# epfl-lts2/pygsp

Measured on AMD Instinct MI355X. Metric: filtered-vertices/sec (N·Nsig·K/s) + achieved HBM GB/s vs roofline, 1M-vertex K=30, higher is better.
Workload: dtype f64

## Files before the change

include/gspx_ext.h:

```cpp
#ifndef GSPX_EXT_H
#define GSPX_EXT_H

#include "gspx.h"

#ifdef __cplusplus
extern "C" {
#endif

int gspx_newton_filter_dev(gspx_graph* g, double lmax, int K, const double* nodes,
                           const double* dcoef, int64_t Nsig, const void* x_dev, void* y_dev,
                           double* kernel_ms);
int gspx_newton_filter(gspx_graph* g, double lmax, int K, const double* nodes, const double* dcoef,
                       int64_t Nsig, const void* x_host, void* y_host, double* kernel_ms);

int gspx_poly_program_dev(gspx_graph* g, double lmax, int S, const double* scale, const double* beta, const double* gamma,
                          int old_is_x, int64_t Nsig, const void* x_dev, void* y_dev, double* kernel_ms);
int gspx_poly_program(gspx_graph* g, double lmax, int S, const double* scale, const double* beta, const double* gamma,
                      int old_is_x, int64_t Nsig, const void* x_host, void* y_host, double* kernel_ms);

int gspx_graph_download_internal(gspx_graph* g, int32_t* rowptr, int32_t* col);

int gspx_graph_set_gather_tiles(gspx_graph* g, int block_rows, int nb, const int32_t* s1ptr,
                                const int32_t* s1rows, const uint16_t* lidx, int64_t* stats);

int gspx_laplacian_apply_dev(gspx_graph* g, int64_t Nsig, const void* x_dev, void* y_dev,
                             double* kernel_ms);
int gspx_dirichlet_energy_dev(gspx_graph* g, int64_t Nsig, const void* x_dev, double* gram_host,
                              double* kernel_ms);
int gspx_panel_gram_dev(gspx_ctx* ctx, int64_t N, const double* A, int64_t lda, int na, const double* B, int64_t ldb,
                        int nb, double* C_host, double* kernel_ms);
int gspx_panel_combine_dev(gspx_ctx* ctx, int64_t N, const double* X, int64_t ldx, int p, const double* Q_host, int q,
                           double* Y, int64_t ldy, double* kernel_ms);
int gspx_panel_gram_to_dev(gspx_ctx* ctx, int64_t N, const double* A, int64_t lda, int na, const double* B, int64_t ldb,
                           int nb, const double* rowscale, double alpha, double* C, int64_t ldc, double* kernel_ms);
int gspx_spectral_apply_dev(gspx_ctx* ctx, int64_t N, const double* U, int64_t ldu, int n, const double* S, int64_t lds,
                            int w, int mode, int nf, const double* H, double* Y, int64_t ldy, double* kernel_ms);
int gspx_panel_residual_norms_dev(gspx_ctx* ctx, int64_t N, const double* X, const double* LX, int64_t ld, int p,
                                  const double* theta_host, double* out_host, double* kernel_ms);
int gspx_panel_copy_dev(gspx_ctx* ctx, int64_t N, const double* X, int64_t ldx, int w, double* Y, int64_t ldy,
                        double* kernel_ms);
int gspx_lanczos_krylov_dev(gspx_graph* g, int order, int64_t Nsig, const void* x_dev, int64_t ldx, double breakdown,
                            void* V_dev, double* alpha_host, double* beta_host, double* proj_host, int32_t* steps_host,
                            double* phase_ms, double* kernel_ms);
int gspx_lanczos_combine_dev(gspx_graph* g, int order, int64_t Nsig, const void* V_dev, int Nf,
                             const double* weights_host, void* y_dev, int64_t ldy, double* kernel_ms);
int gspx_tikhonov_cg_dev(gspx_graph* g, double tau, const void* mask_dev, int64_t Nsig,
                         const void* y_dev, void* x_dev, double rtol, double atol, int64_t maxiter,
                         int32_t* iterations, double* kernel_ms);
int gspx_dirichlet_cg_dev(gspx_graph* g, const void* mask_dev, int64_t Nsig, const void* y_dev, void* x_dev,
                          double rtol, double atol, int64_t maxiter, int32_t* iterations, double* kernel_ms);
int gspx_tikhonov_simplex_dev(gspx_graph* g, double tau, double step, const int32_t* labels_dev, int n_classes,
                              double rtol, double atol, double dtol, double xtol, int64_t maxit, void* x_dev,
                              int64_t* niter, int32_t* crit, double* objective_host, double* kernel_ms);
int gspx_prox_tv_dev(gspx_graph* g, double gamma, double step, int64_t Nsig, const void* x_dev, void* z_dev,
                     double rtol, double atol, double dtol, double xtol, int64_t maxit, int64_t* niter, int32_t* crit,
                     double* objective_host, double* kernel_ms);
int gspx_graph_n_edges(gspx_graph* g, int64_t* n_edges);
int gspx_graph_download_edges(gspx_graph* g, int32_t* sources, int32_t* targets, void* weights,
                              void* d_source, void* d_target);
int gspx_graph_set_edge_list(gspx_graph* g, int64_t n_edges, const int32_t* sources, const int32_t* targets,
                             const double* weights, int directed);

int gspx_grad_dev(gspx_graph* g, int64_t Nsig, const void* x_dev, void* y_dev, double* kernel_ms);
int gspx_div_dev(gspx_graph* g, int64_t Nsig, const void* y_dev, void* z_dev, double* kernel_ms);

typedef struct gspx_knn gspx_knn;
int gspx_knn_build(gspx_ctx* ctx, int64_t N, int d, const double* coords, int k, double sigma,
                   int metric, int symmetrize, gspx_knn** out);
int gspx_knn_destroy(gspx_knn* h);
int gspx_knn_info(gspx_knn* h, int64_t* nnz, double* sigma, double* build_ms);
int gspx_knn_search_stats(gspx_knn* h, double out[4]);
int gspx_knn_download_w(gspx_knn* h, int32_t* indptr, int32_t* indices, double* data);
int gspx_knn_download_neighbors(gspx_knn* h, int32_t* nn, double* dist);

int gspx_radius_build(gspx_ctx* ctx, int64_t N, int d, const double* coords, double epsilon,
                      double sigma, int metric, gspx_knn** out);

int gspx_sbm_build(gspx_ctx* ctx, int64_t N, int k, const int32_t* order, const int64_t* bounds,
                   const double* M, uint64_t seed, gspx_knn** out);
int gspx_sbm_build_ex(gspx_ctx* ctx, int64_t N, int k, const int32_t* order, const int64_t* bounds,
                      const double* M, uint64_t seed, int flags, gspx_knn** out);

int gspx_linegraph_size(gspx_graph* g, int64_t* n_vertices, int64_t* nnz);
int gspx_linegraph_build(gspx_graph* g, gspx_knn** out, double* kernel_ms);

int gspx_schur_cg_dev(gspx_graph* g, double shift, const void* mask_dev, int64_t Nsig, const void* f_dev, void* x_dev,
                      void* alpha_dev, double rtol, double atol, int64_t maxiter, int32_t* iterations,
                      double* kernel_ms);
int gspx_kron_build(gspx_graph* g, double shift, const int32_t* ind_host, int64_t nk, double rtol, int64_t maxiter,
                    double* lnew_dev, gspx_knn** w_out, int32_t* iterations, double* kernel_ms);

int gspx_curve_keys(gspx_ctx* ctx, int64_t N, int d, const double* coords, int curve, uint64_t* keys);

int gspx_curve_order(gspx_ctx* ctx, int64_t N, int d, const double* coords, int curve, int32_t* perm);

int gspx_graph_setup(gspx_ctx* ctx, int64_t N, int64_t nnz, const int32_t* indptr, const int32_t* indices,
                     const void* data, int data_dtype, int lap_type, int compute_dtype, const double* coords,
                     int d, int order_mode, const int32_t* perm_in, int64_t report[12], gspx_graph** out);
int gspx_graph_setup_from_knn(gspx_knn* h, int lap_type, int compute_dtype, const double* coords, int d,
                              int order_mode, const int32_t* perm_in, int64_t report[12], gspx_graph** out);
int gspx_graph_lmax_bounds(gspx_graph* g, double out[4]);
int gspx_graph_download_perm(gspx_graph* g, int32_t* perm);

int gspx_graph_components_dev(gspx_graph* g, int32_t* labels_dev, int64_t* n_components, int* rounds,
                              double* kernel_ms);
int gspx_graph_components(gspx_graph* g, int32_t* labels_host, int64_t* n_components, int* rounds, double* kernel_ms);
int gspx_components_round_cap(int64_t N, int* cap);

int gspx_layout_spring_dev(gspx_graph* g, int dim, double k, const void* fixed_dev, int64_t iterations, double t0,
                           double dt, void* pos_dev, double* kernel_ms);
int gspx_layout_splits(gspx_graph* g, int64_t* splits);

#define GSPX_ERR_NOCONV 7
int gspx_sym_eig_dev(gspx_ctx* ctx, int n, const double* A, int64_t lda, double* V, int64_t ldv, double* e_host,
                     double tol, int max_sweeps, double* info, int64_t* skipped_per_sweep);
int gspx_sym_eig_schedule_describe(int n_blocks, int* pairs_out, int* n_rounds);
int gspx_panel_scale_cols_dev(gspx_ctx* ctx, int64_t N, double* X, int64_t ldx, int w, const double* s_host);

int gspx_identity_panel_dev(gspx_ctx* ctx, int dtype, int64_t N, int64_t j0, int64_t w, void* out_dev);
int gspx_cheby_sqnorms_dev(gspx_graph* g, double lmax, int Nf, int M, const double* coeffs, int64_t Nsig,
                           const void* x_dev, double* out, double* kernel_ms);
int gspx_cheby_moments_dev(gspx_graph* g, double lmax, int M, int64_t Nsig, const void* x_dev,
                           double* out, double* kernel_ms);

int gspx_device_pci_bus_id(int device, char* out, int capacity);

int gspx_planes_pack_dev(gspx_ctx* ctx, int dtype, int64_t N, int64_t S, int64_t F, const void* src_dev,
                         void* dst_dev, int to_planes);

int gspx_plan_describe(gspx_ctx* ctx, int Nf, int M, const double* coeffs, double* plan);
int gspx_host_pipeline_describe(int mode, int64_t host_batch, int64_t host_edge, int64_t host_threads, int dtype,
                                int64_t N, int64_t Nsig, int planes_total, int64_t* widths, int capacity,
                                int* n_batches, int* threads);

int gspx_last_host_timing(gspx_ctx* ctx, double out[9]);
int gspx_last_step_kinds(gspx_ctx* ctx, int64_t out[2]);
int gspx_last_host_timeline(gspx_ctx* ctx, double* out, int capacity, int* batches);

int gspx_bench_copy(gspx_ctx* ctx, int64_t bytes, int iters, double* gbps);

int gspx_bench_read(gspx_ctx* ctx, int64_t bytes, int passes, double* gbps);

int gspx_ctx_tune_placement(gspx_graph* g, double lmax, int M, const double* coeffs, int64_t Nsig, const void* x_dev,
                            void* y_dev, int candidates, int64_t stride_mb, double* out);

int gspx_bench_streams(gspx_ctx* ctx, int64_t bytes_per_stream, int n_read, int n_write, int nt, int workgroups_per_cu,
                       int iters, double* gbps);

int gspx_bench_step_mix(gspx_graph* g, double lmax, int M, const double* coeffs, int64_t Nsig, const void* x_dev,
                        void* y_dev, int mode);

int gspx_bench_gather(gspx_ctx* ctx, int64_t panel_rows, int row_bytes, int64_t n_gathers, int in_flight,
                      int blocks, double p_intra, int workgroups_per_cu, int iters, double* ms, double* gbps);

int gspx_comm_info(gspx_comm* comm, int64_t out[3]);

#ifdef __cplusplus
}
#endif
#endif
```

pygsp_amd/_capi.py:

```python
import ctypes
import os

import numpy as np

_HERE = os.path.dirname(os.path.abspath(__file__))
LIB_PATH = os.environ.get("GSPX_LIB_PATH") or os.path.join(_HERE, "_lib", "libgspx.so")

F32, F64 = 0, 1
LAP_COMBINATORIAL, LAP_NORMALIZED = 0, 1
ANALYSIS, SYNTHESIS = 0, 1

OK, ERR_INVALID, ERR_COEFF, ERR_HIP, ERR_NODEVICE, ERR_OOM, ERR_INTERNAL, ERR_NOCONV = 0, 1, 2, 3, 4, 5, 6, 7

_lib = None


class GspxError(RuntimeError):
    """HIP / runtime failure inside libgspx."""


def dtype_code(dt):
    dt = np.dtype(dt)
    if dt == np.float32:
        return F32
    if dt == np.float64:
        return F64
    raise ValueError("libgspx computes in float32 or float64, got {}".format(dt))


def np_dtype(code):
    return np.float32 if code == F32 else np.float64


_c = ctypes
_P = _c.c_void_p
SIGNATURES = {
    "gspx_last_error": (_c.c_char_p, []),
    "gspx_version": (_c.c_char_p, []),
    "gspx_device_count": (_c.c_int, [_c.POINTER(_c.c_int)]),
    "gspx_ctx_create": (_c.c_int, [_c.c_int, _c.POINTER(_P)]),
    "gspx_ctx_destroy": (_c.c_int, [_P]),
    "gspx_ctx_sync": (_c.c_int, [_P]),
    "gspx_ctx_set_option": (_c.c_int, [_P, _c.c_char_p, _c.c_int64]),
    "gspx_ctx_get_option": (_c.c_int, [_P, _c.c_char_p, _c.POINTER(_c.c_int64)]),
    "gspx_buf_alloc": (_c.c_int, [_P, _c.c_int64, _c.POINTER(_P)]),
    "gspx_buf_free": (_c.c_int, [_P]),
    "gspx_buf_upload": (_c.c_int, [_P, _P, _c.c_int64]),
    "gspx_buf_download": (_c.c_int, [_P, _P, _c.c_int64]),
    "gspx_buf_ptr": (_c.c_int, [_P, _c.POINTER(_P)]),
    "gspx_buf_bytes": (_c.c_int, [_P, _c.POINTER(_c.c_int64)]),
    "gspx_graph_create_from_w": (_c.c_int, [_P, _c.c_int64, _c.c_int64, _P, _P, _P, _c.c_int,
                                            _c.c_int, _c.c_int, _P, _c.POINTER(_P)]),
    "gspx_graph_create_from_l": (_c.c_int, [_P, _c.c_int64, _c.c_int64, _P, _P, _P, _c.c_int,
                                            _c.c_int, _P, _c.POINTER(_P)]),
    "gspx_graph_destroy": (_c.c_int, [_P]),
    "gspx_graph_n": (_c.c_int, [_P, _c.POINTER(_c.c_int64)]),
    "gspx_graph_nnz_l": (_c.c_int, [_P, _c.POINTER(_c.c_int64)]),
    "gspx_graph_nnz_internal": (_c.c_int, [_P, _c.POINTER(_c.c_int64)]),
    "gspx_graph_download_l": (_c.c_int, [_P, _P, _P, _P]),
    "gspx_graph_download_dw": (_c.c_int, [_P, _P]),
    "gspx_graph_build_ms": (_c.c_int, [_P, _c.POINTER(_c.c_double)]),
    "gspx_cheby_filter_dev": (_c.c_int, [_P, _c.c_double, _c.c_int, _c.c_int, _P, _c.c_int64, _P,
                                         _P, _c.c_int, _c.POINTER(_c.c_double)]),
    "gspx_cheby_filter": (_c.c_int, [_P, _c.c_double, _c.c_int, _c.c_int, _P, _c.c_int64, _P, _P,
                                     _c.c_int, _c.POINTER(_c.c_double)]),
    "gspx_newton_filter_dev": (_c.c_int, [_P, _c.c_double, _c.c_int, _P, _P, _c.c_int64, _P, _P,
                                          _c.POINTER(_c.c_double)]),
    "gspx_newton_filter": (_c.c_int, [_P, _c.c_double, _c.c_int, _P, _P, _c.c_int64, _P, _P,
                                      _c.POINTER(_c.c_double)]),
    "gspx_graph_download_internal": (_c.c_int, [_P, _P, _P]),
    "gspx_laplacian_apply_dev": (_c.c_int, [_P, _c.c_int64, _P, _P, _P]),
    "gspx_dirichlet_energy_dev": (_c.c_int, [_P, _c.c_int64, _P, _P, _P]),
    "gspx_panel_gram_dev": (_c.c_int, [_P, _c.c_int64, _P, _c.c_int64, _c.c_int, _P, _c.c_int64, _c.c_int, _P, _P]),
    "gspx_panel_combine_dev": (_c.c_int, [_P, _c.c_int64, _P, _c.c_int64, _c.c_int, _P, _c.c_int, _P, _c.c_int64, _P]),
    "gspx_panel_gram_to_dev": (_c.c_int, [_P, _c.c_int64, _P, _c.c_int64, _c.c_int, _P, _c.c_int64, _c.c_int, _P,
                                          _c.c_double, _P, _c.c_int64, _P]),
    "gspx_spectral_apply_dev": (_c.c_int, [_P, _c.c_int64, _P, _c.c_int64, _c.c_int, _P, _c.c_int64, _c.c_int, _c.c_int,
                                           _c.c_int, _P, _P, _c.c_int64, _P]),
    "gspx_panel_residual_norms_dev": (_c.c_int, [_P, _c.c_int64, _P, _P, _c.c_int64, _c.c_int, _P, _P, _P]),
    "gspx_panel_copy_dev": (_c.c_int, [_P, _c.c_int64, _P, _c.c_int64, _c.c_int, _P, _c.c_int64, _P]),
    "gspx_sym_eig_dev": (_c.c_int, [_P, _c.c_int, _P, _c.c_int64, _P, _c.c_int64, _P, _c.c_double, _c.c_int, _P, _P]),
    "gspx_sym_eig_schedule_describe": (_c.c_int, [_c.c_int, _P, _c.POINTER(_c.c_int)]),
    "gspx_panel_scale_cols_dev": (_c.c_int, [_P, _c.c_int64, _P, _c.c_int64, _c.c_int, _P]),
    "gspx_lanczos_krylov_dev": (_c.c_int, [_P, _c.c_int, _c.c_int64, _P, _c.c_int64, _c.c_double, _P, _P, _P, _P, _P,
                                           _P, _P]),
    "gspx_lanczos_combine_dev": (_c.c_int, [_P, _c.c_int, _c.c_int64, _P, _c.c_int, _P, _P, _c.c_int64, _P]),
    "gspx_tikhonov_cg_dev": (_c.c_int, [_P, _c.c_double, _P, _c.c_int64, _P, _P, _c.c_double,
                                         _c.c_double, _c.c_int64, _P, _P]),
    "gspx_dirichlet_cg_dev": (_c.c_int, [_P, _P, _c.c_int64, _P, _P, _c.c_double, _c.c_double, _c.c_int64, _P, _P]),
    "gspx_tikhonov_simplex_dev": (_c.c_int, [_P, _c.c_double, _c.c_double, _P, _c.c_int, _c.c_double, _c.c_double,
                                              _c.c_double, _c.c_double, _c.c_int64, _P, _c.POINTER(_c.c_int64),
                                              _c.POINTER(_c.c_int32), _P, _c.POINTER(_c.c_double)]),
    "gspx_prox_tv_dev": (_c.c_int, [_P, _c.c_double, _c.c_double, _c.c_int64, _P, _P, _c.c_double, _c.c_double,
                                     _c.c_double, _c.c_double, _c.c_int64, _c.POINTER(_c.c_int64),
                                     _c.POINTER(_c.c_int32), _P, _c.POINTER(_c.c_double)]),
    "gspx_graph_n_edges": (_c.c_int, [_P, _P]),
    "gspx_graph_download_edges": (_c.c_int, [_P, _P, _P, _P, _P, _P]),
    "gspx_graph_set_edge_list": (_c.c_int, [_P, _c.c_int64, _P, _P, _P, _c.c_int]),
    "gspx_grad_dev": (_c.c_int, [_P, _c.c_int64, _P, _P, _P]),
    "gspx_div_dev": (_c.c_int, [_P, _c.c_int64, _P, _P, _P]),
    "gspx_knn_build": (_c.c_int, [_P, _c.c_int64, _c.c_int, _P, _c.c_int, _c.c_double, _c.c_int, _c.c_int, _P]),
    "gspx_knn_destroy": (_c.c_int, [_P]),
    "gspx_knn_info": (_c.c_int, [_P, _P, _P, _P]),
    "gspx_knn_download_w": (_c.c_int, [_P, _P, _P, _P]),
    "gspx_knn_search_stats": (_c.c_int, [_P, _P]),
    "gspx_knn_download_neighbors": (_c.c_int, [_P, _P, _P]),
    "gspx_graph_set_gather_tiles": (_c.c_int, [_P, _c.c_int, _c.c_int, _P, _P, _P, _P]),
    "gspx_curve_keys": (_c.c_int, [_P, _c.c_int64, _c.c_int, _P, _c.c_int, _P]),
    "gspx_graph_build_gather_tiles": (_c.c_int, [_P, _P]),
    "gspx_curve_order": (_c.c_int, [_P, _c.c_int64, _c.c_int, _P, _c.c_int, _P]),
    "gspx_graph_setup": (_c.c_int, [_P, _c.c_int64, _c.c_int64, _P, _P, _P, _c.c_int, _c.c_int, _c.c_int, _P, _c.c_int,
                                    _c.c_int, _P, _P, _c.POINTER(_P)]),
    "gspx_graph_setup_from_knn": (_c.c_int, [_P, _c.c_int, _c.c_int, _P, _c.c_int, _c.c_int, _P, _P, _c.POINTER(_P)]),
    "gspx_graph_download_perm": (_c.c_int, [_P, _P]),
    "gspx_graph_lmax_bounds": (_c.c_int, [_P, _P]),
    "gspx_graph_components_dev": (_c.c_int, [_P, _P, _c.POINTER(_c.c_int64), _c.POINTER(_c.c_int),
                                             _c.POINTER(_c.c_double)]),
    "gspx_graph_components": (_c.c_int, [_P, _P, _c.POINTER(_c.c_int64), _c.POINTER(_c.c_int),
                                         _c.POINTER(_c.c_double)]),
    "gspx_components_round_cap": (_c.c_int, [_c.c_int64, _c.POINTER(_c.c_int)]),
    "gspx_layout_spring_dev": (_c.c_int, [_P, _c.c_int, _c.c_double, _P, _c.c_int64, _c.c_double, _c.c_double, _P,
                                          _c.POINTER(_c.c_double)]),
    "gspx_layout_splits": (_c.c_int, [_P, _c.POINTER(_c.c_int64)]),
    "gspx_sbm_build": (_c.c_int, [_P, _c.c_int64, _c.c_int, _P, _P, _P, _c.c_uint64, _P]),
    "gspx_sbm_build_ex": (_c.c_int, [_P, _c.c_int64, _c.c_int, _P, _P, _P, _c.c_uint64, _c.c_int, _P]),
    "gspx_linegraph_size": (_c.c_int, [_P, _c.POINTER(_c.c_int64), _c.POINTER(_c.c_int64)]),
    "gspx_linegraph_build": (_c.c_int, [_P, _c.POINTER(_P), _c.POINTER(_c.c_double)]),
    "gspx_schur_cg_dev": (_c.c_int, [_P, _c.c_double, _P, _c.c_int64, _P, _P, _P, _c.c_double, _c.c_double, _c.c_int64,
                                     _P, _P]),
    "gspx_kron_build": (_c.c_int, [_P, _c.c_double, _P, _c.c_int64, _c.c_double, _c.c_int64, _P, _c.POINTER(_P), _P,
                                   _c.POINTER(_c.c_double)]),
    "gspx_radius_build": (_c.c_int, [_P, _c.c_int64, _c.c_int, _P, _c.c_double, _c.c_double, _c.c_int, _P]),
    "gspx_last_timing": (_c.c_int, [_P, _c.POINTER(_c.c_double)]),
    "gspx_last_host_timing": (_c.c_int, [_P, _c.POINTER(_c.c_double)]),
    "gspx_last_step_kinds": (_c.c_int, [_P, _c.POINTER(_c.c_int64)]),
    "gspx_last_host_timeline": (_c.c_int, [_P, _P, _c.c_int, _P]),
    "gspx_host_pipeline_describe": (_c.c_int, [_c.c_int, _c.c_int64, _c.c_int64, _c.c_int64, _c.c_int, _c.c_int64,
                                               _c.c_int64, _c.c_int, _P, _c.c_int, _P, _P]),
    "gspx_plan_describe": (_c.c_int, [_P, _c.c_int, _c.c_int, _P, _P]),
    "gspx_lanczos_lmax": (_c.c_int, [_P, _c.c_int, _c.c_double, _c.POINTER(_c.c_double),
                                     _c.POINTER(_c.c_int), _c.POINTER(_c.c_int)]),
    "gspx_bench_read": (_c.c_int, [_P, _c.c_int64, _c.c_int, _c.POINTER(_c.c_double)]),
    "gspx_gather": (_c.c_int, [_P, _c.c_int, _P, _P]),
    "gspx_identity_panel_dev": (_c.c_int, [_P, _c.c_int, _c.c_int64, _c.c_int64, _c.c_int64, _P]),
    "gspx_cheby_sqnorms_dev": (_c.c_int, [_P, _c.c_double, _c.c_int, _c.c_int, _P, _c.c_int64, _P, _P,
                                          _c.POINTER(_c.c_double)]),
    "gspx_cheby_moments_dev": (_c.c_int, [_P, _c.c_double, _c.c_int, _c.c_int64, _P, _P, _c.POINTER(_c.c_double)]),
    "gspx_planes_pack_dev": (_c.c_int, [_P, _c.c_int, _c.c_int64, _c.c_int64, _c.c_int64, _P, _P, _c.c_int]),
    "gspx_device_pci_bus_id": (_c.c_int, [_c.c_int, _c.c_char_p, _c.c_int]),
    "gspx_comm_available": (_c.c_int, []),
    "gspx_comm_unique_id": (_c.c_int, [_P]),
    "gspx_comm_create": (_c.c_int, [_P, _c.c_int, _c.c_int, _P, _c.POINTER(_P)]),
    "gspx_comm_destroy": (_c.c_int, [_P]),
    "gspx_comm_info": (_c.c_int, [_P, _P]),
    "gspx_comm_gather": (_c.c_int, [_P, _P, _P, _c.c_int, _P, _c.POINTER(_c.c_double)]),
    "gspx_bench_gather": (_c.c_int, [_P, _c.c_int64, _c.c_int, _c.c_int64, _c.c_int, _c.c_int, _c.c_double, _c.c_int,
                                     _c.c_int, _c.POINTER(_c.c_double), _c.POINTER(_c.c_double)]),
    "gspx_bench_copy": (_c.c_int, [_P, _c.c_int64, _c.c_int, _c.POINTER(_c.c_double)]),
    "gspx_poly_program_dev": (_c.c_int, [_P, _c.c_double, _c.c_int, _P, _P, _P, _c.c_int, _c.c_int64, _P, _P,
                                       _c.POINTER(_c.c_double)]),
    "gspx_poly_program": (_c.c_int, [_P, _c.c_double, _c.c_int, _P, _P, _P, _c.c_int, _c.c_int64, _P, _P,
                                   _c.POINTER(_c.c_double)]),
    "gspx_ctx_tune_placement": (_c.c_int, [_P, _c.c_double, _c.c_int, _P, _c.c_int64, _P, _P, _c.c_int, _c.c_int64, _P]),
    "gspx_bench_streams": (_c.c_int, [_P, _c.c_int64, _c.c_int, _c.c_int, _c.c_int, _c.c_int, _c.c_int, _c.POINTER(_c.c_double)]),
    "gspx_bench_step_mix": (_c.c_int, [_P, _c.c_double, _c.c_int, _P, _c.c_int64, _P, _P, _c.c_int]),
}


def load():
    global _lib
    if _lib is not None:
        return _lib
    if not os.path.exists(LIB_PATH):
        raise GspxError(
            "libgspx.so not found at {} - build it with `python -c 'import __graft_entry__ as g; "
            "g.build()'` or `make -C pygsp_amd/csrc`. pygsp_amd has no CPU fallback.".format(LIB_PATH))
    lib = ctypes.CDLL(LIB_PATH)
    for name, (res, args) in SIGNATURES.items():
        fn = getattr(lib, name)
        fn.restype = res
        fn.argtypes = args
    _lib = lib
    return lib


def last_error():
    msg = load().gspx_last_error()
    return msg.decode("utf-8", "replace") if msg else ""


def check(rc):
    if rc == OK:
        return
    msg = last_error()
    if rc == ERR_INVALID:
        raise ValueError(msg)
    if rc == ERR_NOCONV:
        raise ValueError(msg)
    if rc == ERR_COEFF:
        raise TypeError(msg)
    if rc == ERR_NODEVICE:
        raise GspxError("no MI355X/HIP device: " + msg)
    if rc == ERR_OOM:
        raise GspxError("out of device memory: " + msg)
    raise GspxError(msg)


def ptr(arr):
    if arr is None:
        return None
    assert arr.flags["C_CONTIGUOUS"]
    return arr.ctypes.data_as(ctypes.c_void_p)


def device_count():
    n = ctypes.c_int(0)
    rc = load().gspx_device_count(ctypes.byref(n))
    if rc != OK:
        return 0
    return n.value
```

pygsp_amd/csrc/gspx_ctx.hip.h:

```cpp
#pragma once

struct Options {
  int64_t kernel = 0;
  int64_t vec = 0;
  int64_t rows_per_wave = 0;
  int64_t narrow_g_log2 = -1;
  int64_t waves_per_block = 4;
  int64_t calib_mix = 0;
  int64_t graph_launch = 2;
  int64_t tile_gather = 1;
  int64_t tile_workgroups = 0;
  int64_t knn_f32 = 1;
  int64_t tile_pad = 1;
  int64_t tile_min_row = 16;
  int64_t staged_copy = 1;
  int64_t staged_copy_min_mb = 32;
  int64_t copy_threads = 0;
  int64_t tile_regroup = 1;
  int64_t tile_acc_builds = 1;
  int64_t tile_lg = 0;
  int64_t edge_vertex_walk = 1;
  int64_t fuse_input = 1;
  int64_t tile_nt = -1;
  int64_t synthesis = 0;
  int64_t alternate_sweep = 1;
  int64_t xcd_remap = 1;
  int64_t combine = 0;
  int64_t ws_limit_mb = 65536;
  int64_t max_batch = 0;
  int64_t gather_rccl = 1;
  int64_t lds_pad_kb = 0;
  int64_t host_pipeline = 1;
  int64_t host_batch = 0;
  int64_t host_edge = 0;
  int64_t host_threads = 0;
  int64_t streamed_alloc = 1;
  int64_t layout_splits = 0;
};

struct gspx_ctx {
  int device = 0;
  int cu_count = 256;
  hipStream_t stream = nullptr;
  Options opt;
  DevMem ws_t;
  DevMem ws_r;
  DevMem ws_w;
  DevMem io_x, io_y;
  DevMem ws_spec;
  DevMem ws_sq, ws_sqp;
  HostPipe* pipe = nullptr;
  CopyStage* copy = nullptr;
  bool counted = false;
  std::mutex comms_mu;
  std::vector<struct gspx_comm*> comms;
  hipEvent_t ev[4] = {nullptr, nullptr, nullptr, nullptr};
  std::vector<hipEvent_t> ev_pool;
  double timing[5] = {0, 0, 0, 0, 0};
  int64_t step_kinds[2] = {0, 0};
  bool capturing = false;
  std::vector<unsigned char> seen_key;
  std::vector<unsigned char> graph_key;
  hipGraphExec_t graph_exec = nullptr;
  int64_t graph_kinds[2] = {0, 0};
};

static std::atomic<int> g_live_ctx[64];

static void replay_reset(gspx_ctx* ctx) {
  if (!ctx) return;
  ctx->seen_key.clear();
  ctx->graph_key.clear();
  if (ctx->graph_exec) {
    (void)hipGraphExecDestroy(ctx->graph_exec);
    ctx->graph_exec = nullptr;
  }
}

static int finish_timed(gspx_ctx* ctx, double* kernel_ms) {
  HIPCHK(hipGetLastError());
  HIPCHK(hipStreamSynchronize(ctx->stream));
  float f = 0;
  HIPCHK(hipEventElapsedTime(&f, ctx->ev[0], ctx->ev[1]));
  if (kernel_ms) *kernel_ms = f;
  return GSPX_OK;
}

struct gspx_buf {
  gspx_ctx* ctx = nullptr;
  DevMem mem;
  int64_t bytes = 0;
};

static std::atomic<uint64_t> g_generation{1};

struct gspx_graph {
  gspx_ctx* ctx = nullptr;
  const uint64_t generation = g_generation.fetch_add(1);
  int64_t N = 0;
  int dtype = GSPX_F64;
  bool from_w = false;
  int64_t nnz_l = 0;
  DevMem lptr, lcol, lval, dw;
  int64_t nnz_int = 0;
  DevMem rptr, rcol, rval, fval, coff;
  unsigned coff_ldb = 0;
  DevMem perm, iperm;
  bool has_perm = false;
  double fval_lmax = -1.0;
  double build_ms = 0.0;
  bool has_bounds = false;
  double bounds[4] = {0, 0, 0, 0};
  DevMem gt_hdr, gt_s1rows, gt_lidx;
  DevMem gt_s1nat;
  int gt_ns1 = 0;
  int gt_rows = 0, gt_nb = 0, gt_slow = 0;
  size_t gt_lds = 0;
  int gt_entmax = 0;
  int lap_type = GSPX_LAP_COMBINATORIAL;
  bool edges_built = false;
  bool edges_custom = false;
  int64_t n_edges = 0;
  DevMem e_off, e_toff, e_src, e_dst, e_tedge, e_cs, e_ct, e_w;
};

static size_t elt_size(int dtype) { return dtype == GSPX_F32 ? 4 : 8; }

static hipEvent_t pool_event(gspx_ctx* ctx, size_t& i_ref) {
  size_t i = i_ref - 1;
  if (i >= 1024) {
    i = 1020 + (i & 3);
    i_ref = i + 1;
  }
  while (ctx->ev_pool.size() <= i) {
    hipEvent_t e = nullptr;
    if (hipEventCreate(&e) != hipSuccess) return nullptr;
    ctx->ev_pool.push_back(e);
  }
  return ctx->ev_pool[i];
}

extern "C" int gspx_device_count(int* n) {
  if (!n) return set_err(GSPX_ERR_INVALID, "gspx_device_count: null output");
  int c = 0;
  hipError_t e = hipGetDeviceCount(&c);
  if (e != hipSuccess) {
    *n = 0;
    (void)hipGetLastError();
    return set_err(GSPX_ERR_NODEVICE, "hipGetDeviceCount failed: %s", hipGetErrorString(e));
  }
  *n = c;
  return GSPX_OK;
}

extern "C" int gspx_device_pci_bus_id(int device, char* out, int capacity) {
  if (!out || capacity < 16) return set_err(GSPX_ERR_INVALID, "gspx_device_pci_bus_id: need a buffer of >= 16 chars");
  out[0] = 0;
  int c = 0;
  if (hipGetDeviceCount(&c) != hipSuccess) {
    (void)hipGetLastError();
    return set_err(GSPX_ERR_NODEVICE, "no HIP device visible (libgspx has no CPU fallback)");
  }
  if (device < 0 || device >= c) return set_err(GSPX_ERR_INVALID, "device %d of %d", device, c);
  HIPCHK(hipDeviceGetPCIBusId(out, capacity, device));
  return GSPX_OK;
}

extern "C" int gspx_ctx_create(int device, gspx_ctx** out) {
  if (!out) return set_err(GSPX_ERR_INVALID, "gspx_ctx_create: null output");
  *out = nullptr;
  int c = 0;
  if (hipGetDeviceCount(&c) != hipSuccess || c <= 0) {
    (void)hipGetLastError();
    return set_err(GSPX_ERR_NODEVICE, "no HIP device visible (libgspx has no CPU fallback)");
  }
  if (device < 0 || device >= c)
    return set_err(GSPX_ERR_INVALID, "device %d out of range (%d visible)", device, c);
  HIPCHK(hipSetDevice(device));
  gspx_ctx* ctx = new gspx_ctx();
  ctx->device = device;
  {
    const char* env = getenv("GSPX_STREAMED_ALLOC");
    const int others = g_live_ctx[device & 63].fetch_add(1);
    ctx->counted = true;
    if (env && (env[0] == '0' || env[0] == '1')) ctx->opt.streamed_alloc = env[0] == '1';
    else ctx->opt.streamed_alloc = others == 0 ? 1 : 0;
    ctx->ws_t.streamed = ctx->ws_r.streamed = ctx->opt.streamed_alloc != 0;
  }
  if (hipDeviceGetAttribute(&ctx->cu_count, hipDeviceAttributeMultiprocessorCount, device) !=
          hipSuccess ||
      ctx->cu_count < 1)
    ctx->cu_count = 256;
  hipError_t e = hipStreamCreateWithFlags(&ctx->stream, hipStreamNonBlocking);
  if (e != hipSuccess) {
    delete ctx;
    return set_err(GSPX_ERR_HIP, "hipStreamCreate failed: %s", hipGetErrorString(e));
  }
  for (int i = 0; i < 4; ++i) {
    e = hipEventCreate(&ctx->ev[i]);
    if (e != hipSuccess) {
      delete ctx;
      return set_err(GSPX_ERR_HIP, "hipEventCreate failed: %s", hipGetErrorString(e));
    }
  }
  *out = ctx;
  return GSPX_OK;
}

static void comm_invalidate_all(gspx_ctx* ctx);

extern "C" int gspx_ctx_destroy(gspx_ctx* ctx) {
  replay_reset(ctx);
  if (!ctx) return GSPX_OK;
  if (ctx->counted) g_live_ctx[ctx->device & 63].fetch_sub(1);
  comm_invalidate_all(ctx);
  if (ctx->graph_exec) {
    (void)hipGraphExecDestroy(ctx->graph_exec);
    ctx->graph_exec = nullptr;
  }
  (void)hipSetDevice(ctx->device);
  if (ctx->stream) (void)hipStreamSynchronize(ctx->stream);
  for (int i = 0; i < 4; ++i)
    if (ctx->ev[i]) (void)hipEventDestroy(ctx->ev[i]);
  for (hipEvent_t e : ctx->ev_pool) (void)hipEventDestroy(e);
  ctx->ws_t.release();
  ctx->ws_r.release();
  ctx->ws_w.release();
  ctx->io_x.release();
  ctx->io_y.release();
  ctx->ws_spec.release();
  ctx->ws_sq.release();
  ctx->ws_sqp.release();
  if (ctx->pipe) {
    ctx->pipe->destroy();
    delete ctx->pipe;
    ctx->pipe = nullptr;
  }
  if (ctx->copy) {
    ctx->copy->destroy();
    delete ctx->copy;
    ctx->copy = nullptr;
  }
  if (ctx->stream) (void)hipStreamDestroy(ctx->stream);
  delete ctx;
  return GSPX_OK;
}

extern "C" int gspx_ctx_sync(gspx_ctx* ctx) {
  if (!ctx) return set_err(GSPX_ERR_INVALID, "null ctx");
  HIPCHK(hipSetDevice(ctx->device));
  HIPCHK(hipStreamSynchronize(ctx->stream));
  return GSPX_OK;
}

struct OptionDef {
  const char* key;
  int64_t Options::*slot;
  bool (*ok)(int64_t);
  const char* refusal;
};
static const OptionDef OPTION_TABLE[] = {
    {"kernel", &Options::kernel, [](int64_t v) { return v == 0 || v == 1 || v == 2 || v == 5; },
     "kernel must be 0 (auto), 1 (panel), 2 (narrow) or 5 (LDS-staged)"},
    {"vec", &Options::vec, [](int64_t v) { return v == 0 || v == 1 || v == 2 || v == 4; }, "vec must be 0, 1, 2 or 4"},
    {"rows_per_wave", &Options::rows_per_wave, [](int64_t v) { return v >= 0 && v <= 1024; },
     "rows_per_wave must be in [0, 1024] (0 = auto)"},
    {"narrow_g_log2", &Options::narrow_g_log2, [](int64_t v) { return v >= -1 && v <= 6; },
     "narrow_g_log2 must be in [-1, 6] (-1 = auto)"},
    {"waves_per_block", &Options::waves_per_block, [](int64_t v) { return v == 4 || v == 8 || v == 16; },
     "waves_per_block must be 4, 8 or 16"},
    {"alternate_sweep", &Options::alternate_sweep, nullptr, nullptr},
    {"synthesis", &Options::synthesis, nullptr, nullptr},
    {"tile_gather", &Options::tile_gather, nullptr, nullptr},
    {"graph_launch", &Options::graph_launch, nullptr, nullptr},
    {"tile_workgroups", &Options::tile_workgroups, nullptr, nullptr},
    {"tile_lg", &Options::tile_lg, nullptr, nullptr},
    {"tile_regroup", &Options::tile_regroup, nullptr, nullptr},
    {"tile_acc_builds", &Options::tile_acc_builds, nullptr, nullptr},
    {"staged_copy", &Options::staged_copy, nullptr, nullptr},
    {"staged_copy_min_mb", &Options::staged_copy_min_mb, nullptr, nullptr},
    {"copy_threads", &Options::copy_threads, nullptr, nullptr},
    {"tile_min_row", &Options::tile_min_row, nullptr, nullptr},
    {"tile_pad", &Options::tile_pad, nullptr, nullptr},
    {"knn_f32", &Options::knn_f32, nullptr, nullptr},
    {"tile_nt", &Options::tile_nt, nullptr, nullptr},
    {"fuse_input", &Options::fuse_input, nullptr, nullptr},
    {"edge_vertex_walk", &Options::edge_vertex_walk, nullptr, nullptr},
    {"xcd_remap", &Options::xcd_remap, nullptr, nullptr},
    {"combine", &Options::combine, nullptr, nullptr},
    {"ws_limit_mb", &Options::ws_limit_mb, nullptr, nullptr},
    {"max_batch", &Options::max_batch, nullptr, nullptr},
    {"gather_rccl", &Options::gather_rccl, nullptr, nullptr},
    {"lds_pad_kb", &Options::lds_pad_kb, nullptr, nullptr},
    {"host_pipeline", &Options::host_pipeline, nullptr, nullptr},
    {"host_batch", &Options::host_batch, nullptr, nullptr},
    {"host_edge", &Options::host_edge, nullptr, nullptr},
    {"host_threads", &Options::host_threads, nullptr, nullptr},
    {"streamed_alloc", &Options::streamed_alloc, nullptr, nullptr},
    {"layout_splits", &Options::layout_splits, [](int64_t v) { return v >= 0 && v <= 65535; },
     "layout_splits must be in [0, 65535] (0 = automatic)"},
};

static const OptionDef* find_option(const char* key) {
  if (key)
    for (const OptionDef& d : OPTION_TABLE)
      if (!strcmp(key, d.key)) return &d;
  set_err(GSPX_ERR_INVALID, "unknown option '%s'", key ? key : "(null)");
  return nullptr;
}

extern "C" int gspx_ctx_set_option(gspx_ctx* ctx, const char* key, int64_t value) {
  replay_reset(ctx);
  if (!ctx) return set_err(GSPX_ERR_INVALID, "null ctx");
  const OptionDef* d = find_option(key);
  if (!d) return GSPX_ERR_INVALID;
  if (d->ok && !d->ok(value)) return set_err(GSPX_ERR_INVALID, "%s", d->refusal);
  ctx->opt.*d->slot = value;
  if (d->slot == &Options::streamed_alloc) {
    const bool on = value != 0;
    (void)hipSetDevice(ctx->device);
    for (DevMem* m : {&ctx->ws_t, &ctx->ws_r}) {
      if (!on && m->va_size) {
        (void)hipStreamSynchronize(ctx->stream);
        m->release();
      }
      m->streamed = on;
    }
  }
  return GSPX_OK;
}

extern "C" int gspx_ctx_get_option(gspx_ctx* ctx, const char* key, int64_t* value) {
  if (!ctx || !value) return set_err(GSPX_ERR_INVALID, "null argument");
  if (key && !strcmp(key, "retired_va_mb")) {
    *value = (int64_t)(g_retired_va_bytes.load() >> 20);
    return GSPX_OK;
  }
  const OptionDef* d = find_option(key);
  if (!d) return GSPX_ERR_INVALID;
  *value = ctx->opt.*d->slot;
  return GSPX_OK;
}

extern "C" int gspx_buf_alloc(gspx_ctx* ctx, int64_t bytes, gspx_buf** out) {
  if (!ctx || !out || bytes < 0) return set_err(GSPX_ERR_INVALID, "gspx_buf_alloc: bad argument");
  *out = nullptr;
  HIPCHK(hipSetDevice(ctx->device));
  gspx_buf* b = new gspx_buf();
  b->ctx = ctx;
  b->bytes = bytes;
  int rc = b->mem.alloc((size_t)bytes);
  if (rc != GSPX_OK) {
    delete b;
    return rc;
  }
  *out = b;
  return GSPX_OK;
}

extern "C" int gspx_buf_free(gspx_buf* b) {
  if (!b) return GSPX_OK;
  (void)hipSetDevice(b->ctx->device);
  (void)hipStreamSynchronize(b->ctx->stream);
  delete b;
  return GSPX_OK;
}

static int staged_copy(gspx_ctx* ctx, unsigned char* dev, unsigned char* host, size_t bytes, bool to_device) {
  if (!ctx->copy) ctx->copy = new CopyStage();
  CopyStage& cs = *ctx->copy;
  CHK(cs.init());
  constexpr int NS = CopyStage::NS;
  const size_t chunk = CopyStage::CHUNK;
  const int nchunks = (int)((bytes + chunk - 1) / chunk);
  const int P = (int)std::max<int64_t>(1, std::min<int64_t>(ctx->opt.copy_threads > 0 ? ctx->opt.copy_threads : 8,
                                                             (int64_t)std::thread::hardware_concurrency()));
  if (!to_device) {
    const uintptr_t lo = ((uintptr_t)host + ((size_t)2 << 20) - 1) & ~(((uintptr_t)2 << 20) - 1);
    const uintptr_t hi = ((uintptr_t)host + bytes) & ~(((uintptr_t)2 << 20) - 1);
    if (hi > lo) (void)madvise((void*)lo, hi - lo, MADV_HUGEPAGE);
  }
  std::atomic<int> released{to_device ? std::min(NS, nchunks) : 0};
  std::vector<std::atomic<int>> done((size_t)nchunks);
  for (auto& d : done) d.store(0);
  std::atomic<bool> failed{false};
  auto worker = [&](int t) {
    for (int c = 0; c < nchunks; ++c) {
      while (released.load(std::memory_order_acquire) <= c) {
        if (failed.load()) return;
        std::this_thread::yield();
      }
      if (failed.load(std::memory_order_acquire)) return;
      const size_t off = (size_t)c * chunk, len = std::min(chunk, bytes - off);
      const size_t per = ((len + P - 1) / P + 63) & ~(size_t)63;
      const size_t lo = std::min(len, per * (size_t)t), hi = std::min(len, lo + per);
      if (hi > lo) {
        unsigned char* pinned = (unsigned char*)cs.pin[c % NS].p;
        if (to_device) memcpy(pinned + lo, host + off + lo, hi - lo);
        else memcpy(host + off + lo, pinned + lo, hi - lo);
      }
      done[(size_t)c].fetch_add(1, std::memory_order_release);
    }
  };
  std::vector<std::thread> pool;
  try {
    pool.reserve((size_t)P);
    for (int t = 0; t < P; ++t) pool.emplace_back(worker, t);
  } catch (...) {
    failed.store(true, std::memory_order_release);
    released.store(nchunks, std::memory_order_release);
    for (auto& th : pool)
      if (th.joinable()) th.join();
    return set_err(GSPX_ERR_HIP, "staged copy: could not start %d host threads", P);
  }
  auto wait_done = [&](int c) {
    while (done[(size_t)c].load(std::memory_order_acquire) < P) std::this_thread::yield();
  };
  hipError_t err = hipSuccess;
  for (int c = 0; c < nchunks && err == hipSuccess; ++c) {
    const size_t off = (size_t)c * chunk, len = std::min(chunk, bytes - off);
    void* pinned = cs.pin[c % NS].p;
    if (to_device) {
      wait_done(c);
      err = hipMemcpyAsync(dev + off, pinned, len, hipMemcpyHostToDevice, cs.st);
      if (err == hipSuccess) err = hipStreamSynchronize(cs.st);
      released.store(std::min(nchunks, c + NS + 1), std::memory_order_release);
    } else {
      if (c >= NS) wait_done(c - NS);
      err = hipMemcpyAsync(pinned, dev + off, len, hipMemcpyDeviceToHost, cs.st);
      if (err == hipSuccess) err = hipStreamSynchronize(cs.st);
      released.store(c + 1, std::memory_order_release);
    }
  }
  if (err != hipSuccess) {
    failed.store(true, std::memory_order_release);
    released.store(nchunks, std::memory_order_release);
  }
  for (auto& th : pool) th.join();
  if (err != hipSuccess) return set_err(GSPX_ERR_HIP, "staged copy: %s", hipGetErrorString(err));
  return GSPX_OK;
}

extern "C" int gspx_buf_upload(gspx_buf* b, const void* host, int64_t bytes) {
  if (!b || (!host && bytes > 0) || bytes < 0 || bytes > b->bytes)
    return set_err(GSPX_ERR_INVALID, "gspx_buf_upload: bad argument");
  HIPCHK(hipSetDevice(b->ctx->device));
  if (bytes == 0) return GSPX_OK;
  if (b->ctx->opt.staged_copy >= 2 && (size_t)bytes >= ((size_t)b->ctx->opt.staged_copy_min_mb << 20)) {
    HIPCHK(hipStreamSynchronize(b->ctx->stream));
    if (staged_copy(b->ctx, (unsigned char*)b->mem.p, (unsigned char*)const_cast<void*>(host), (size_t)bytes, true) == GSPX_OK)
      return GSPX_OK;
    (void)hipGetLastError();
  }
  HIPCHK(hipMemcpyAsync(b->mem.p, host, (size_t)bytes, hipMemcpyHostToDevice, b->ctx->stream));
  HIPCHK(hipStreamSynchronize(b->ctx->stream));
  return GSPX_OK;
}

extern "C" int gspx_buf_download(gspx_buf* b, void* host, int64_t bytes) {
  if (!b || (!host && bytes > 0) || bytes < 0 || bytes > b->bytes)
    return set_err(GSPX_ERR_INVALID, "gspx_buf_download: bad argument");
  HIPCHK(hipSetDevice(b->ctx->device));
  if (bytes == 0) return GSPX_OK;
  if (b->ctx->opt.staged_copy && (size_t)bytes >= ((size_t)b->ctx->opt.staged_copy_min_mb << 20)) {
    HIPCHK(hipStreamSynchronize(b->ctx->stream));
    if (staged_copy(b->ctx, (unsigned char*)b->mem.p, (unsigned char*)host, (size_t)bytes, false) == GSPX_OK) return GSPX_OK;
    (void)hipGetLastError();
  }
  HIPCHK(hipMemcpyAsync(host, b->mem.p, (size_t)bytes, hipMemcpyDeviceToHost, b->ctx->stream));
  HIPCHK(hipStreamSynchronize(b->ctx->stream));
  return GSPX_OK;
}

extern "C" int gspx_buf_ptr(gspx_buf* b, void** p) {
  if (!b || !p) return set_err(GSPX_ERR_INVALID, "gspx_buf_ptr: null argument");
  *p = b->mem.p;
  return GSPX_OK;
}

extern "C" int gspx_buf_bytes(gspx_buf* b, int64_t* bytes) {
  if (!b || !bytes) return set_err(GSPX_ERR_INVALID, "gspx_buf_bytes: null argument");
  *bytes = b->bytes;
  return GSPX_OK;
}

extern "C" int gspx_last_host_timing(gspx_ctx* ctx, double out[9]) {
  if (!ctx || !out) return set_err(GSPX_ERR_INVALID, "null argument");
  for (int i = 0; i < 9; ++i) out[i] = ctx->pipe ? ctx->pipe->timing[i] : 0.0;
  return GSPX_OK;
}

extern "C" int gspx_last_host_timeline(gspx_ctx* ctx, double* out, int capacity, int* batches) {
  if (!ctx || !batches) return set_err(GSPX_ERR_INVALID, "null argument");
  const std::vector<double> empty;
  const std::vector<double>& t = ctx->pipe ? ctx->pipe->timeline : empty;
  *batches = (int)(t.size() / 6);
  if (out)
    for (int i = 0; i < capacity && i < (int)t.size(); ++i) out[i] = t[(size_t)i];
  return GSPX_OK;
}

extern "C" int gspx_last_timing(gspx_ctx* ctx, double out[5]) {
  if (!ctx || !out) return set_err(GSPX_ERR_INVALID, "null argument");
  for (int i = 0; i < 5; ++i) out[i] = ctx->timing[i];
  return GSPX_OK;
}

extern "C" int gspx_last_step_kinds(gspx_ctx* ctx, int64_t out[2]) {
  if (!ctx || !out) return set_err(GSPX_ERR_INVALID, "null argument");
  out[0] = ctx->step_kinds[0];
  out[1] = ctx->step_kinds[1];
  return GSPX_OK;
}
```

pygsp_amd/csrc/gspx_hostpipe.hip.h:

```cpp
#pragma once

#include <sys/mman.h>

#include <condition_variable>
#include <thread>


static inline void copy_rows(unsigned char* dst, size_t dpitch, const unsigned char* src, size_t spitch, size_t rb,
                             int64_t r0, int64_t r1) {
  dst += (size_t)r0 * dpitch;
  src += (size_t)r0 * spitch;
  switch (rb) {
#define GSPX_CR(B)                                                        \
  case B:                                                                 \
    for (int64_t r = r0; r < r1; ++r, dst += dpitch, src += spitch) memcpy(dst, src, B); \
    return;
    GSPX_CR(32)
    GSPX_CR(64)
    GSPX_CR(128)
    GSPX_CR(256)
#undef GSPX_CR
    default:
      for (int64_t r = r0; r < r1; ++r, dst += dpitch, src += spitch) memcpy(dst, src, rb);
  }
}

#define GSPX_HOSTPIPE_UNAVAILABLE (-1)

template <typename T, typename Run>
static int filter_host_pipelined(gspx_graph* g, int64_t Nsig, int in_planes, int out_planes, const T* x, T* y,
                                 const std::vector<int64_t>& widths, int nthreads, double* kernel_ms, const Run& run) {
  gspx_ctx* ctx = g->ctx;
  HostPipe& hp = *ctx->pipe;
  if (hp.init() != GSPX_OK) {
    (void)hipGetLastError();
    return GSPX_HOSTPIPE_UNAVAILABLE;
  }
  const int64_t N = g->N;
  const int nb = (int)widths.size();
  std::vector<int64_t> col0((size_t)nb, 0);
  for (int b = 1; b < nb; ++b) col0[(size_t)b] = col0[(size_t)b - 1] + widths[(size_t)b - 1];
  const int64_t w = *std::max_element(widths.begin(), widths.end());
  {
    const uintptr_t xa = (uintptr_t)x, xb = xa + (size_t)in_planes * N * Nsig * sizeof(T);
    const uintptr_t ya = (uintptr_t)y, yb = ya + (size_t)out_planes * N * Nsig * sizeof(T);
    if (xa < yb && ya < xb) return GSPX_HOSTPIPE_UNAVAILABLE;
  }
  {
    const size_t bytes = (size_t)out_planes * N * Nsig * sizeof(T);
    const uintptr_t lo = ((uintptr_t)y + ((size_t)2 << 20) - 1) & ~(((uintptr_t)2 << 20) - 1);
    const uintptr_t hi = ((uintptr_t)y + bytes) & ~(((uintptr_t)2 << 20) - 1);
    if (hi > lo) (void)madvise((void*)lo, hi - lo, MADV_HUGEPAGE);
  }
  const size_t in_cap = (size_t)in_planes * N * w * sizeof(T), out_cap = (size_t)out_planes * N * w * sizeof(T);
  constexpr int NIN = HostPipe::NIN;
  for (int s = 0; s < NIN; ++s) {
    if (hp.pin_in[s].ensure(in_cap) != GSPX_OK || hp.dx[s].ensure(in_cap) != GSPX_OK ||
        (s < 2 && (hp.pin_out[s].ensure(out_cap) != GSPX_OK || hp.dy[s].ensure(out_cap) != GSPX_OK))) {
      (void)hipGetLastError();
      return GSPX_HOSTPIPE_UNAVAILABLE;
    }
  }
  const int P = std::max(1, nthreads), Q = std::max(1, nthreads);
  const auto wall0 = std::chrono::steady_clock::now();

  std::mutex mu;
  std::condition_variable cv;
  int issued = 0, computed = 0, shipped = 0, unpacked = 0;
  std::vector<int> pack_arrived((size_t)nb, 0), unpack_arrived((size_t)nb, 0);
  int err = GSPX_OK;
  std::string err_msg;
  auto fail = [&](int rc) {
    std::lock_guard<std::mutex> lock(mu);
    if (err == GSPX_OK) {
      err = rc;
      err_msg = g_err;
    }
    cv.notify_all();
  };
  auto wait_for = [&](auto pred) {
    std::unique_lock<std::mutex> lock(mu);
    cv.wait(lock, [&] { return err != GSPX_OK || pred(); });
    return err == GSPX_OK;
  };
  auto hipfail = [&](hipError_t e, const char* what) {
    if (e == hipSuccess) return false;
    fail(set_err(GSPX_ERR_HIP, "%s failed in the host pipeline: %s", what, hipGetErrorString(e)));
    return true;
  };
  std::vector<double> pack_ms((size_t)P, 0.0), unpack_ms((size_t)Q, 0.0);
  std::vector<double> line((size_t)nb * 6, 0.0);
  auto stamp = [&](int b, int what) {
    line[(size_t)b * 6 + what] = std::chrono::duration<double, std::milli>(std::chrono::steady_clock::now() - wall0).count();
  };
  double h2d_ms = 0, d2h_ms = 0;
  auto width_of = [&](int b) { return widths[(size_t)b]; };

  auto pack_worker = [&](int p) {
    const int64_t r0 = N * p / P, r1 = N * (p + 1) / P;
    for (int b = 0; b < nb; ++b) {
      const int s = b % NIN;
      if (!wait_for([&] { return computed >= b - (NIN - 1); })) return;
      const auto t0 = std::chrono::steady_clock::now();
      const int64_t wl = width_of(b);
      for (int pl = 0; pl < in_planes; ++pl)
        copy_rows((unsigned char*)hp.pin_in[s].p + (size_t)pl * N * wl * sizeof(T), (size_t)wl * sizeof(T),
                  (const unsigned char*)(x + (size_t)pl * N * Nsig + (size_t)col0[(size_t)b]), (size_t)Nsig * sizeof(T),
                  (size_t)wl * sizeof(T), r0, r1);
      pack_ms[(size_t)p] += std::chrono::duration<double, std::milli>(std::chrono::steady_clock::now() - t0).count();
      bool last;
      {
        std::lock_guard<std::mutex> lock(mu);
        last = ++pack_arrived[(size_t)b] == P;
      }
      if (last) {
        stamp(b, 0);
        if (hipfail(hipSetDevice(ctx->device), "hipSetDevice")) return;
        if (b >= NIN) {
          float t = 0;
          if (hipEventElapsedTime(&t, hp.t_in[s][0], hp.t_in[s][1]) == hipSuccess) h2d_ms += t;
        }
        if (hipfail(hipEventRecord(hp.t_in[s][0], hp.stream_in), "hipEventRecord")) return;
        if (hipfail(hipMemcpyAsync(hp.dx[s].p, hp.pin_in[s].p, (size_t)in_planes * N * wl * sizeof(T),
                                   hipMemcpyHostToDevice, hp.stream_in), "hipMemcpyAsync (H2D)")) return;
        if (hipfail(hipEventRecord(hp.t_in[s][1], hp.stream_in), "hipEventRecord")) return;
        if (hipfail(hipEventRecord(hp.h2d_ev[s], hp.stream_in), "hipEventRecord")) return;
        stamp(b, 1);
        std::lock_guard<std::mutex> lock(mu);
        issued = b + 1;
        cv.notify_all();
      }
    }
  };
  auto shipper = [&]() {
    if (hipfail(hipSetDevice(ctx->device), "hipSetDevice")) return;
    for (int b = 0; b < nb; ++b) {
      const int s = b & 1;
      if (!wait_for([&] { return computed >= b + 1 && unpacked >= b - 1; })) return;
      const int64_t wl = width_of(b);
      if (hipfail(hipEventRecord(hp.t_out[0], hp.stream_out), "hipEventRecord")) return;
      if (hipfail(hipMemcpyAsync(hp.pin_out[s].p, hp.dy[s].p, (size_t)out_planes * N * wl * sizeof(T),
                                 hipMemcpyDeviceToHost, hp.stream_out), "hipMemcpyAsync (D2H)")) return;
      if (hipfail(hipEventRecord(hp.t_out[1], hp.stream_out), "hipEventRecord")) return;
      if (hipfail(hipStreamSynchronize(hp.stream_out), "hipStreamSynchronize")) return;
      float t = 0;
      if (hipEventElapsedTime(&t, hp.t_out[0], hp.t_out[1]) == hipSuccess) d2h_ms += t;
      stamp(b, 4);
      std::lock_guard<std::mutex> lock(mu);
      shipped = b + 1;
      cv.notify_all();
    }
  };
  auto unpack_worker = [&](int q) {
    const int64_t r0 = N * q / Q, r1 = N * (q + 1) / Q;
    {
      for (int pl = 0; pl < out_planes; ++pl) {
        volatile unsigned char* base = (volatile unsigned char*)(y + (size_t)pl * N * Nsig);
        const size_t lo = (size_t)r0 * Nsig * sizeof(T), hi = (size_t)r1 * Nsig * sizeof(T);
        for (size_t off = lo; off < hi; off += 4096) base[off] = 0;
        if (hi > lo) base[hi - 1] = 0;
      }
    }
    for (int b = 0; b < nb; ++b) {
      const int s = b & 1;
      if (!wait_for([&] { return shipped >= b + 1; })) return;
      const auto t0 = std::chrono::steady_clock::now();
      const int64_t wl = width_of(b);
      for (int pl = 0; pl < out_planes; ++pl)
        copy_rows((unsigned char*)(y + (size_t)pl * N * Nsig + (size_t)col0[(size_t)b]), (size_t)Nsig * sizeof(T),
                  (const unsigned char*)hp.pin_out[s].p + (size_t)pl * N * wl * sizeof(T), (size_t)wl * sizeof(T),
                  (size_t)wl * sizeof(T), r0, r1);
      unpack_ms[(size_t)q] += std::chrono::duration<double, std::milli>(std::chrono::steady_clock::now() - t0).count();
      std::lock_guard<std::mutex> lock(mu);
      if (++unpack_arrived[(size_t)b] == Q) {
        stamp(b, 5);
        unpacked = b + 1;
        cv.notify_all();
      }
    }
  };

  std::vector<std::thread> threads;
  threads.reserve((size_t)P + Q + 1);
  try {
    for (int p = 0; p < P; ++p) threads.emplace_back(pack_worker, p);
    threads.emplace_back(shipper);
    for (int q = 0; q < Q; ++q) threads.emplace_back(unpack_worker, q);
  } catch (...) {
    fail(set_err(GSPX_ERR_HIP, "could not start the host pipeline threads"));
  }

  double k_ms = 0, tm[5] = {0, 0, 0, 0, 0};
  int64_t kinds[2] = {0, 0};
  for (int b = 0; b < nb; ++b) {
    const int s = b % NIN, so = b & 1;
    if (!wait_for([&] { return issued >= b + 1 && shipped >= b - 1; })) break;
    if (hipfail(hipStreamWaitEvent(ctx->stream, hp.h2d_ev[s], 0), "hipStreamWaitEvent")) break;
    stamp(b, 2);
    const int rc = run((const T*)hp.dx[s].p, (T*)hp.dy[so].p, width_of(b));
    if (rc != GSPX_OK) {
      fail(rc);
      break;
    }
    stamp(b, 3);
    k_ms += ctx->timing[0];
    for (int i = 0; i < 5; ++i) tm[i] += ctx->timing[i];
    for (int i = 0; i < 2; ++i) kinds[i] += ctx->step_kinds[i];
    std::lock_guard<std::mutex> lock(mu);
    computed = b + 1;
    cv.notify_all();
  }
  for (auto& t : threads) t.join();
  (void)hipSetDevice(ctx->device);
  if (err != GSPX_OK) {
    (void)hipStreamSynchronize(hp.stream_in);
    (void)hipStreamSynchronize(hp.stream_out);
    (void)hipStreamSynchronize(ctx->stream);
    g_err = err_msg;
    return err;
  }
  for (int b = std::max(0, nb - NIN); b < nb; ++b) {
    float t = 0;
    if (hipEventElapsedTime(&t, hp.t_in[b % NIN][0], hp.t_in[b % NIN][1]) == hipSuccess) h2d_ms += t;
  }
  (void)hipGetLastError();
  for (int i = 0; i < 5; ++i) ctx->timing[i] = tm[i];
  for (int i = 0; i < 2; ++i) ctx->step_kinds[i] = kinds[i];
  hp.timing[0] = std::chrono::duration<double, std::milli>(std::chrono::steady_clock::now() - wall0).count();
  hp.timing[1] = *std::max_element(pack_ms.begin(), pack_ms.end());
  hp.timing[2] = h2d_ms;
  hp.timing[3] = k_ms;
  hp.timing[4] = d2h_ms;
  hp.timing[5] = *std::max_element(unpack_ms.begin(), unpack_ms.end());
  hp.timing[6] = nb;
  hp.timing[7] = (double)w;
  hp.timing[8] = P;
  hp.timeline = line;
  if (kernel_ms) *kernel_ms = k_ms;
  return GSPX_OK;
}

static void host_pipeline_shape(const Options& opt, size_t elt, int64_t N, int64_t Nsig, int planes_total,
                                std::vector<int64_t>* widths, int* threads_out) {
  widths->clear();
  if (!opt.host_pipeline) return;
  const size_t total = (size_t)N * (size_t)Nsig * elt * (size_t)planes_total;
  if (opt.host_pipeline == 1 && total < ((size_t)48 << 20)) return;
  const int64_t unit = (int64_t)(64 / elt);
  int64_t w = opt.host_batch > 0 ? opt.host_batch : (int64_t)(128 / elt);
  if (opt.host_batch <= 0 && Nsig < 4 * w) w = std::max<int64_t>(unit, (Nsig / 4) / unit * unit);
  w = std::min<int64_t>(w, Nsig);
  int64_t edge = opt.host_edge > 0 ? std::min<int64_t>(opt.host_edge, w) : (opt.host_batch > 0 ? w : std::max(unit, w / 2 / unit * unit));
  if (Nsig <= w || (opt.host_pipeline == 1 && Nsig < 2 * w)) {
    if (opt.host_pipeline != 2 || Nsig < 2) return;
    w = edge = (Nsig + 1) / 2;
  }
  if (2 * edge >= Nsig) edge = w;
  if (edge < w) {
    widths->push_back(edge);
    for (int64_t c = edge; c < Nsig - edge; c += w) widths->push_back(std::min<int64_t>(w, Nsig - edge - c));
    widths->push_back(edge);
  } else {
    for (int64_t c = 0; c < Nsig; c += w) widths->push_back(std::min<int64_t>(w, Nsig - c));
  }
  if (opt.host_batch <= 0 && widths->size() >= 2 && (size_t)widths->back() * elt < 32) {
    const int64_t tail = widths->back();
    widths->pop_back();
    widths->back() += tail;
  }
  int t = (int)opt.host_threads;
  if (t <= 0) {
    const unsigned hc = std::thread::hardware_concurrency();
    t = (int)std::min<unsigned>(16, std::max<unsigned>(1, hc / 4));
  }
  *threads_out = std::min(t, 64);
}

extern "C" int gspx_host_pipeline_describe(int mode, int64_t host_batch, int64_t host_edge, int64_t host_threads,
                                           int dtype, int64_t N, int64_t Nsig, int planes_total, int64_t* widths,
                                           int capacity, int* n_batches, int* threads) {
  if (!n_batches || N < 0 || Nsig < 0 || planes_total < 1 || (dtype != GSPX_F32 && dtype != GSPX_F64))
    return set_err(GSPX_ERR_INVALID, "bad argument");
  Options opt;
  opt.host_pipeline = mode;
  opt.host_batch = host_batch;
  opt.host_edge = host_edge;
  opt.host_threads = host_threads;
  std::vector<int64_t> w;
  int t = 1;
  host_pipeline_shape(opt, elt_size(dtype), N, Nsig, planes_total, &w, &t);
  if (w.size() < 2) w.clear();
  *n_batches = (int)w.size();
  if (threads) *threads = t;
  if (widths)
    for (int i = 0; i < capacity && i < (int)w.size(); ++i) widths[i] = w[(size_t)i];
  return GSPX_OK;
}
```

pygsp_amd/csrc/gspx_poly.hip.h:

```cpp
#pragma once

struct PlanStep {
  double scale = 1.0, gamma = -1.0;
  int flush = 0;
  int final = 0;
  std::vector<double> w;
};

static void make_plan_fused(int nf, int M, const std::vector<double>& cp, bool acc_existing,
                            bool final_to_y, std::vector<PlanStep>& plan) {
  const int K = M - 1;
  plan.assign((size_t)K, PlanStep());
  int covered = -1;
  bool first = !acc_existing;
  for (int k = 1; k <= K; ++k) {
    PlanStep& st = plan[(size_t)k - 1];
    st.scale = (k == 1) ? 0.5 : 1.0;
    st.gamma = (k == 1) ? 0.0 : -1.0;
    st.w.assign((size_t)nf * 3, 0.0);
    const bool must = (k == K) || (k >= 2 && (k - 2) > covered);
    if (!must) continue;
    st.flush = first ? 1 : 2;
    first = false;
    st.final = (k == K && final_to_y) ? 1 : 0;
// ... 29 lines not shown
  if (Nf < 1 || !coeffs || !plan_out) return set_err(GSPX_ERR_INVALID, "bad argument");
  Options opt;
  if (ctx) opt = ctx->opt;
  std::vector<double> cp;
  halve_c0(Nf, M, coeffs, cp);
  std::vector<PlanStep> plan;
  const bool deferred = opt.combine == 2 || (opt.combine == 0 && Nf >= 2);
  if (deferred)
    make_plan_deferred(Nf, M, plan);
  else
    make_plan_fused(Nf, M, cp, false, true, plan);
  const size_t stride = 4 + 3 * (size_t)Nf;
  for (size_t k = 0; k < plan.size(); ++k) {
    double* o = plan_out + k * stride;
    o[0] = plan[k].scale;
    o[1] = plan[k].gamma;
    o[2] = plan[k].flush;
    o[3] = plan[k].final;
    for (size_t j = 0; j < 3 * (size_t)Nf; ++j) o[4 + j] = plan[k].w[j];
  }
  return GSPX_OK;
}

struct Shape {
  int kernel;
  int vec;
  int wlog2;
  int glog2;
  int gridy;
};

static Shape choose_shape(const Options& opt, size_t elt, int64_t ld, int veccap) {
  Shape s{};
  const int maxvec = std::min((int)(16 / elt), veccap);
  int vec = 1;
  for (int v = maxvec; v >= 1; v /= 2)
    if (ld % v == 0) { vec = v; break; }
  while (vec > 1 && ld / vec < 16) vec /= 2;
  if (opt.vec != 0 && opt.vec <= maxvec && ld % opt.vec == 0) vec = (int)opt.vec;
  int kernel = (ld <= 4) ? 2 : 1;
  if (opt.kernel == 2 && ld <= 64) kernel = 2;
  if (opt.kernel == 1 && ld > 4) kernel = 1;
  if (opt.kernel == 5 && ld > 4) kernel = 5;
  if (opt.kernel == 0 && kernel == 1 && (elt == 4 || ld <= 32)) kernel = 5;
  s.kernel = kernel;
  if (kernel == 1 || kernel == 5) {
    s.vec = vec;
    const int64_t lanes = ld / vec;
    s.wlog2 = lanes <= 16 ? 4 : (lanes <= 32 ? 5 : 6);
    s.gridy = (int)((lanes + 63) / 64);
    s.glog2 = 0;
  } else {
    s.vec = 1;
    int wl = 0;
    while ((1 << wl) < ld) ++wl;
    s.wlog2 = wl;
    const int64_t gl = opt.narrow_g_log2 >= 0 ? opt.narrow_g_log2 : std::max(0, 2 - wl);
    s.glog2 = (int)std::min<int64_t>(gl, 6 - wl);
    s.gridy = 1;
  }
  return s;
}

template <typename T, int VEC, int MODE>
static void launch_panel_w(const StepArgs<T>& a, int wlog2, dim3 grid, hipStream_t st) {
#define GSPX_LP(WL)                                                                     \
  hipLaunchKernelGGL((k_step_panel<T, VEC, WL, MODE>), grid, dim3(64 * a.wpb), 0, st, a.rowptr, \
                     a.col, a.val, a.cur, a.wts, a.perm, a)
  switch (wlog2) {
    case 4: GSPX_LP(4); break;
    case 5: GSPX_LP(5); break;
    default: GSPX_LP(6); break;
  }
#undef GSPX_LP
}

template <typename T, int MODE>
static void launch_panel(const StepArgs<T>& a, const Shape& s, dim3 grid, hipStream_t st) {
  if constexpr (sizeof(T) == 4) {
    if (s.vec == 4) return launch_panel_w<T, 4, MODE>(a, s.wlog2, grid, st);
  }
  if (s.vec == 2) return launch_panel_w<T, 2, MODE>(a, s.wlog2, grid, st);
  return launch_panel_w<T, 1, MODE>(a, s.wlog2, grid, st);
}

template <typename T, int VEC, int MODE>
static void launch_lds_w(const StepArgs<T>& a, const unsigned* coff, int wlog2, dim3 grid,
                         hipStream_t st) {
#define GSPX_LL(WL)                                                                          \
  hipLaunchKernelGGL((k_step_lds<T, VEC, WL, MODE>), grid, dim3(256), (size_t)a.lds_pad, st, a.rowptr, coff, \
                     a.val, a.cur, a.wts, a.perm, a)
  switch (wlog2) {
    case 4: GSPX_LL(4); break;
    case 5: GSPX_LL(5); break;
    default: GSPX_LL(6); break;
  }
#undef GSPX_LL
}

template <typename T, int MODE>
static void launch_lds(const StepArgs<T>& a, const unsigned* coff, const Shape& s, dim3 grid,
                       hipStream_t st) {
  if constexpr (sizeof(T) == 4) {
    if (s.vec == 4) return launch_lds_w<T, 4, MODE>(a, coff, s.wlog2, grid, st);
  }
  if (s.vec == 2) return launch_lds_w<T, 2, MODE>(a, coff, s.wlog2, grid, st);
  return launch_lds_w<T, 1, MODE>(a, coff, s.wlog2, grid, st);
}

template <typename T>
static void launch_step(gspx_ctx* ctx, StepArgs<T> a, const Shape& s, const Options& opt, hipStream_t st,
                        const unsigned* coff) {
  ++ctx->step_kinds[1];
  int rpw = (int)opt.rows_per_wave;
  if (rpw <= 0)
    rpw = (s.kernel == 5) ? (sizeof(T) == 4 ? 16 : 8) : (s.kernel == 2 ? 1 : 4);
  if (s.kernel == 1 || s.kernel == 5) {
    const int R = 64 >> s.wlog2;
    rpw = ((rpw + R - 1) / R) * R;
    if (s.kernel == 5 && rpw > 32) rpw = 32;
  }
  a.rows_per_wave = rpw;
  int rows_per_chunk;
  a.lds_pad = (int)std::min<int64_t>(std::max<int64_t>(opt.lds_pad_kb, 0), 40) * 1024;
  a.wpb = (s.kernel == 1) ? (int)opt.waves_per_block : 4;
  if (s.kernel == 1 || s.kernel == 5)
    rows_per_chunk = a.wpb * rpw;
  else
    rows_per_chunk = rpw * (4 << (6 - s.wlog2 - s.glog2));
  a.nchunks = (a.N + rows_per_chunk - 1) / rows_per_chunk;
  int gx = a.nchunks;
  a.cpx = 0;
  if (opt.xcd_remap) {
    a.cpx = (a.nchunks + 7) / 8;
    gx = a.cpx * 8;
  }
  dim3 grid((unsigned)gx, (unsigned)s.gridy, 1);
  const int mode = a.flush ? 1 : ((a.beta != T(0) || a.nin > 0 || a.final) ? 2 : 0);
  if (s.kernel == 5) {
    if (mode == 1) launch_lds<T, 1>(a, coff, s, grid, st);
    else if (mode == 2) launch_lds<T, 2>(a, coff, s, grid, st);
    else launch_lds<T, 0>(a, coff, s, grid, st);
  } else if (s.kernel == 1) {
    if (mode == 1) launch_panel<T, 1>(a, s, grid, st);
    else if (mode == 2) launch_panel<T, 2>(a, s, grid, st);
    else launch_panel<T, 0>(a, s, grid, st);
  } else {
    if (a.flush)
      hipLaunchKernelGGL((k_step_narrow<T, true>), grid, dim3(256), 0, st, a, s.wlog2, s.glog2);
    else
      hipLaunchKernelGGL((k_step_narrow<T, false>), grid, dim3(256), 0, st, a, s.wlog2, s.glog2);
  }
}

template <typename T>
static void launch_permute_in(const T* x, unsigned ldx, T* out, unsigned ld, int N,
                              const int* perm, int vec, hipStream_t st) {
  const size_t total = (size_t)N * (ld / vec);
  const unsigned nb = (unsigned)std::min<size_t>((total + 255) / 256, 65536);
  if (nb == 0) return;
  if constexpr (sizeof(T) == 4) {
    if (vec == 4) {
      hipLaunchKernelGGL((k_permute_in<T, 4>), dim3(nb), dim3(256), 0, st, x, ldx, out, ld, N, perm);
      return;
    }
  }
  if (vec == 2)
    hipLaunchKernelGGL((k_permute_in<T, 2>), dim3(nb), dim3(256), 0, st, x, ldx, out, ld, N, perm);
  else
    hipLaunchKernelGGL((k_permute_in<T, 1>), dim3(nb), dim3(256), 0, st, x, ldx, out, ld, N, perm);
}

template <typename T, int VEC>
static void launch_combine_v(const T* slots, int nslots, size_t slot_stride, const T* cf, int M,
                             int nf, int N, unsigned ld, T* y, unsigned ldy, size_t plane_y,
                             const int* perm, hipStream_t st, unsigned pitch) {
  const size_t total = (size_t)N * (ld / VEC);
  const unsigned nb = (unsigned)std::min<size_t>((total + 255) / 256, 16384);
  if (nb == 0) return;
  constexpr int NFB = 8;
  for (int f0 = 0; f0 < nf; f0 += NFB) {
    const int here = std::min(NFB, nf - f0);
    hipLaunchKernelGGL((k_combine<T, VEC, NFB>), dim3(nb), dim3(256), 0, st, slots, nslots,
                       slot_stride, cf, M, f0, here, N, ld, y, ldy, plane_y, perm, 0, pitch);
  }
}

template <typename T>
static void launch_combine(const T* slots, int nslots, size_t slot_stride, const T* cf, int M,
                           int nf, int N, unsigned ld, T* y, unsigned ldy, size_t plane_y,
                           const int* perm, int vec, hipStream_t st, unsigned pitch = 0) {
  if (!pitch) pitch = ld;
  if constexpr (sizeof(T) == 4) {
    if (vec == 4)
      return launch_combine_v<T, 4>(slots, nslots, slot_stride, cf, M, nf, N, ld, y, ldy, plane_y,
                                    perm, st, pitch);
  }
  if (vec == 2)
    return launch_combine_v<T, 2>(slots, nslots, slot_stride, cf, M, nf, N, ld, y, ldy, plane_y,
                                  perm, st, pitch);
  return launch_combine_v<T, 1>(slots, nslots, slot_stride, cf, M, nf, N, ld, y, ldy, plane_y,
                                perm, st, pitch);
}

struct SqNorms {
  const double* cf;
  int ldc, nf;
  double* out;
  size_t ldo;
  double* part;
};
static const int SQ_PASS = 128;
static int sqnorm_cwl(unsigned w) {
  int l = 0;
  while (l < 6 && (1u << l) < w) ++l;
  return l;
}
static int sqnorm_gx(const gspx_ctx* ctx, int N, unsigned w) {
  const int cwl = sqnorm_cwl(w);
  const int64_t tiles = ((int64_t)N + (64 >> cwl) - 1) / (64 >> cwl);
  const int64_t gy = ((int64_t)w + (1 << cwl) - 1) >> cwl;
  return (int)std::max<int64_t>(1, std::min<int64_t>(tiles, (4 * (int64_t)ctx->cu_count + gy - 1) / gy));
}
static size_t sqnorm_parts(const gspx_ctx* ctx, int N, unsigned w) {
  return (size_t)sqnorm_gx(ctx, N, w) * SQ_PASS * w;
}

template <typename T>
static int launch_combine_sqnorm(gspx_ctx* ctx, const T* slots, int nslots, size_t slot_stride, unsigned pitch, int N,
                                 unsigned w, const SqNorms& sq, hipStream_t st) {
  const size_t lds = (size_t)nslots * 64 * sizeof(double);
  const int cwl = sqnorm_cwl(w);
  const dim3 grid((unsigned)sqnorm_gx(ctx, N, w), (w + (1u << cwl) - 1) >> cwl);
  for (int f0 = 0; f0 < sq.nf; f0 += SQ_PASS) {
    const int here = std::min(SQ_PASS, sq.nf - f0);
    const int fb = here <= 8 ? 2 : here <= 32 ? 8 : 32;
    typedef void (*kern_t)(const T*, int, size_t, u32, int, int, int, const double*, int, double*);
    const kern_t kern = fb == 2 ? k_combine_sqnorm<T, 2> : fb == 8 ? k_combine_sqnorm<T, 8> : k_combine_sqnorm<T, 32>;
    if (lds > ((size_t)64 << 10))
      HIPCHK(hipFuncSetAttribute((const void*)kern, hipFuncAttributeMaxDynamicSharedMemorySize, (int)lds));
    hipLaunchKernelGGL(kern, grid, dim3(256), lds, st, slots, nslots, slot_stride, (u32)pitch, N, (int)w, cwl,
                       sq.cf + f0, sq.ldc, sq.part);
    const int64_t n = (int64_t)here * w;
    hipLaunchKernelGGL(k_sqnorm_reduce, dim3((unsigned)((n + 255) / 256)), dim3(256), 0, st, sq.part, (int)grid.x,
                       4 * fb, here, (int)w, sq.out + (size_t)f0 * sq.ldo, sq.ldo);
  }
  return GSPX_OK;
}

struct SlotDots {
  double* out;
  size_t ldo;
  double* part;
};
static const int DOTS_CS[2] = {16, 8};
template <typename T> static int dots_vec(unsigned w, unsigned pitch) {
  return sizeof(T) == 4 && w % 2 == 0 && pitch % 2 == 0 ? 2 : 1;
}
static int dots_chunks(int S, int vec) { return (S - 1 + DOTS_CS[vec - 1] - 1) / DOTS_CS[vec - 1]; }
static int dots_gx(const gspx_ctx* ctx, int N, unsigned w, int S, int vec) {
  const int cwl = sqnorm_cwl(w / vec);
  const int64_t rows = 4 * (int64_t)(64 >> cwl);
  const int64_t tiles = ((int64_t)N + rows - 1) / rows;
  const int64_t others = (((int64_t)(w / vec) + (1 << cwl) - 1) >> cwl) * dots_chunks(S, vec);
  const int64_t fit = ((int64_t)64 << 20) / ((int64_t)(2 * S - 1) * w * (int64_t)sizeof(double));
  const int64_t want = (8 * (int64_t)ctx->cu_count + others - 1) / others;
  return (int)std::max<int64_t>(1, std::min(std::min(tiles, want), fit));
}
static size_t dots_parts(const gspx_ctx* ctx, int N, unsigned w, int S) {
  const int gx = std::max(dots_gx(ctx, N, w, S, 1), w % 2 == 0 ? dots_gx(ctx, N, w, S, 2) : 0);
  return (size_t)gx * (size_t)(2 * S - 1) * w;
}

template <typename T>
static int launch_slot_dots(gspx_ctx* ctx, const T* slots, int S, size_t slot_stride, unsigned pitch, int N, unsigned w,
                            const SlotDots& sd, hipStream_t st) {
  const int vec = dots_vec<T>(w, pitch);
  const int cwl = sqnorm_cwl(w / vec);
  const int gx = dots_gx(ctx, N, w, S, vec);
  const dim3 grid((unsigned)gx, (unsigned)dots_chunks(S, vec), (w / vec + (1u << cwl) - 1) >> cwl);
  typedef void (*kern_t)(const T*, int, size_t, u32, int, int, int, double*);
  kern_t kern = k_slot_dots<T, 1, 16>;
  if constexpr (sizeof(T) == 4) {
    if (vec == 2) kern = k_slot_dots<T, 2, 8>;
  }
  hipLaunchKernelGGL(kern, grid, dim3(256), 0, st, slots, S, slot_stride, (u32)pitch, N, (int)w, cwl, sd.part);
  const int64_t n = (int64_t)(2 * S - 1) * w;
  hipLaunchKernelGGL(k_dots_reduce, dim3((unsigned)((n + 63) / 64)), dim3(256), 0, st, sd.part, gx, n, (int)w, sd.out,
                     sd.ldo);
  return GSPX_OK;
}

template <typename T> static bool tile_geometry(const gspx_graph* g, const Options& opt, unsigned ld) {
  constexpr int TVEC = 16 / (int)sizeof(T);
  const size_t U = (size_t)g->N * ld;
  return opt.tile_gather && g->gt_rows == GSPX_TILE_BR && (size_t)ld * sizeof(T) >= (size_t)opt.tile_min_row &&
         (ld % TVEC) == 0 && U * sizeof(T) < ((size_t)1 << 31) && (size_t)g->nnz_int * sizeof(T) < ((size_t)1 << 31);
}
template <typename T>
static bool tile_usable(const gspx_graph* g, const Options& opt, unsigned ld, const T* y, unsigned ldy) {
  constexpr int TVEC = 16 / (int)sizeof(T);
  return tile_geometry<T>(g, opt, ld) && (ldy % TVEC) == 0 && (((uintptr_t)y / sizeof(T)) % TVEC) == 0;
}
template <typename T>
static int launch_step_tile(gspx_graph* g, const Options& opt, TileArgs<T> t, unsigned ld, hipStream_t st,
                            const T* vals = nullptr) {
  const size_t rowb = (size_t)ld * sizeof(T);
  int lg = rowb <= 16 ? 1 : rowb <= 32 ? 2 : rowb <= 64 ? 4 : rowb <= 128 ? 8 : 16;
  if (opt.tile_lg == 8 || opt.tile_lg == 4 || opt.tile_lg == 2) lg = rowb <= 128 ? std::max(lg, (int)opt.tile_lg) : 16;
  const bool narrow = lg < 16;
  const int ncol = narrow ? 1 : (int)((rowb + 255) / 256);
  const int flavour = t.old_rows ? 1 : t.nin > 0 ? 2 : 0;
  typedef void (*kern_t)(const TileArgs<T>);
  static const kern_t wide[3][3] = {
      {k_step_tile<T, 0>, k_step_tile<T, 1>, k_step_tile<T, 2>},
      {k_step_tile<T, 0, 16, true>, k_step_tile<T, 1, 16, true>, k_step_tile<T, 2, 16, true>},
      {k_step_tile<T, 0, 16, false, true>, k_step_tile<T, 1, 16, false, true>, k_step_tile<T, 2, 16, false, true>}};
  static const kern_t slim[3][4] = {
      {k_step_tile<T, 1, 1, false, false, 64>, k_step_tile<T, 1, 2, false, false, 128>,
       k_step_tile<T, 1, 4, false, false, 256>, k_step_tile<T, 1, 8>},
      {k_step_tile<T, 1, 1, true, false, 64>, k_step_tile<T, 1, 2, true, false, 128>,
       k_step_tile<T, 1, 4, true, false, 256>, k_step_tile<T, 1, 8, true>},
      {k_step_tile<T, 1, 1, false, true, 64>, k_step_tile<T, 1, 2, false, true, 128>,
       k_step_tile<T, 1, 4, false, true, 256>, k_step_tile<T, 1, 8, false, true>}};
  kern_t kern = narrow ? slim[flavour][lg == 1 ? 0 : lg == 2 ? 1 : lg == 4 ? 2 : 3] : wide[flavour][ncol <= 2 ? ncol : 0];
  unsigned threads = narrow ? 64u * (unsigned)lg : 512u;
  const bool noacc = opt.tile_acc_builds && t.flush == 0 && !narrow && flavour == 0;
  if (noacc) {
    static const kern_t freek[3] = {k_step_tile<T, 0, 16, false, false, 512, 16, 0, false>,
                                    k_step_tile<T, 1, 16, false, false, 512, 16, 0, false>,
                                    k_step_tile<T, 2, 16, false, false, 512, 16, 0, false>};
    kern = freek[ncol <= 2 ? ncol : 0];
  }
  bool mix = false;
  if (opt.calib_mix && !narrow && flavour == 0) {
    static const kern_t mixk[2][3] = {
        {k_step_tile<T, 0, 16, false, false, 512, 16, 1>, k_step_tile<T, 1, 16, false, false, 512, 16, 1>,
         k_step_tile<T, 2, 16, false, false, 512, 16, 1>},
        {k_step_tile<T, 0, 16, false, false, 512, 16, 2>, k_step_tile<T, 1, 16, false, false, 512, 16, 2>,
         k_step_tile<T, 2, 16, false, false, 512, 16, 2>}};
    static const kern_t mixfree[2][3] = {
        {k_step_tile<T, 0, 16, false, false, 512, 16, 1, false>, k_step_tile<T, 1, 16, false, false, 512, 16, 1, false>,
         k_step_tile<T, 2, 16, false, false, 512, 16, 1, false>},
        {k_step_tile<T, 0, 16, false, false, 512, 16, 2, false>, k_step_tile<T, 1, 16, false, false, 512, 16, 2, false>,
         k_step_tile<T, 2, 16, false, false, 512, 16, 2, false>}};
    kern = (noacc ? mixfree : mixk)[opt.calib_mix == 2 ? 1 : 0][ncol <= 2 ? ncol : 0];
    mix = true;
  }
  const int pieces = (int)(rowb / 16);
  if (opt.tile_regroup && ncol == 1 && flavour != 1 && pieces < lg && !mix) {
#define GSPX_CL(LG_, CL_, NT_) \
  (flavour == 2 ? (kern_t)k_step_tile<T, 1, LG_, false, true, NT_, CL_> : (kern_t)k_step_tile<T, 1, LG_, false, false, NT_, CL_>)
    kern_t k2 = nullptr;
    unsigned nt2 = 0;
    if (lg == 4 && pieces == 3) k2 = GSPX_CL(4, 3, 192), nt2 = 192;
    else if (lg == 8 && pieces == 5) k2 = GSPX_CL(8, 5, 320), nt2 = 320;
    else if (lg == 16 && pieces == 10) k2 = GSPX_CL(16, 10, 320), nt2 = 320;
#undef GSPX_CL
    if (k2) kern = k2, threads = nt2;
  }
  size_t lds = g->gt_lds;
  if (lg < 8)
    lds = std::min(lds, (size_t)GSPX_TILE_MAXN1 * 16 * lg + (((size_t)g->gt_entmax * sizeof(T) + 15) & ~(size_t)15) +
                            (((size_t)g->gt_entmax + 15) & ~(size_t)15) + 64);
  if (lg < 8) lds = (lds + 2047) & ~(size_t)2047;
  int per_cu = 2;
  {
    struct Known { size_t attr = 0; std::map<size_t, int> fit; };
    static std::map<std::pair<const void*, int>, Known> known;
    static std::mutex lds_mu;
    std::lock_guard<std::mutex> lock(lds_mu);
    Known& k = known[std::make_pair((const void*)kern, g->ctx->device)];
    if (k.attr < lds) {
      HIPCHK(hipFuncSetAttribute((const void*)kern, hipFuncAttributeMaxDynamicSharedMemorySize, (int)lds));
      k.attr = lds;
    }
    if (lg < 8) {
      auto it = k.fit.find(lds);
      if (it == k.fit.end()) {
        int fit = 2;
        HIPCHK(hipOccupancyMaxActiveBlocksPerMultiprocessor(&fit, (const void*)kern, (int)threads, lds));
        it = k.fit.emplace(lds, std::max(2, std::min(fit, 16))).first;
      }
      per_cu = it->second;
    }
  }
  t.rowptr = g->rptr.as<int>();
  t.col = g->rcol.as<int>();
  t.val = vals ? vals : g->fval.as<T>();
  t.hdr = g->gt_hdr.as<int>();
  if (!t.s1rows) t.s1rows = g->gt_s1rows.as<int>();
  t.lidx = g->gt_lidx.as<unsigned char>();
  t.N = (int)g->N;
  t.ld = ld;
  t.panel_bytes = (unsigned)((size_t)g->N * ld * sizeof(T));
  t.val_bytes = (unsigned)((size_t)g->nnz_int * sizeof(T));
  t.lidx_bytes = (unsigned)((size_t)g->nnz_int);
  t.nb = g->gt_nb;
  t.ncol = ncol;
  t.per_xcd = (t.nb + 7) / 8;
  t.lds_bytes = (int)lds;
  unsigned nwg = (unsigned)std::max<int64_t>(8, ((int64_t)per_cu * g->ctx->cu_count) / 8 * 8);
  if (opt.tile_workgroups > 0)
    nwg = (unsigned)std::max<int64_t>(8, std::min<int64_t>(opt.tile_workgroups, 1 << 20) / 8 * 8);
  nwg = std::min(nwg, 8u * (unsigned)std::max(t.per_xcd, 1));
  t.nt = opt.tile_nt >= 0 ? (int)opt.tile_nt : ((size_t)g->N * ld * sizeof(T) >= ((size_t)192 << 20) ? 5 : 0);
  ++g->ctx->step_kinds[0];
  hipLaunchKernelGGL(kern, dim3(nwg), dim3(threads), lds, st, t);
  return GSPX_OK;
}

template <typename T>
static int prepare_coff(gspx_graph* g, const Shape& shape, unsigned ld, hipStream_t st) {
  if (shape.kernel == 5 && g->coff_ldb != ld * (unsigned)sizeof(T)) {
    CHK(g->coff.ensure(((size_t)g->nnz_int + 64) * sizeof(unsigned)));
    const int nb = std::max(1, (int)((g->N + 255) / 256));
    hipLaunchKernelGGL((k_coff<T>), dim3(nb), dim3(256), 0, st, g->rptr.as<int>(), g->rcol.as<int>(), (int)g->N,
                       ld * (unsigned)sizeof(T), g->coff.as<unsigned>());
    g->coff_ldb = ld * (unsigned)sizeof(T);
  }
  return GSPX_OK;
}

template <typename T> static int vec_cap(int v, unsigned ld, const T* p) {
  while (v > 1 && ((ld % v) != 0 || (((uintptr_t)p / sizeof(T)) % v) != 0)) v /= 2;
  return v;
}

struct WorkPanels {
  bool tile_direct, padded;
  unsigned ldw;
};
template <typename T>
static WorkPanels work_panels(const gspx_graph* g, const Options& opt, bool tiles, size_t planes, unsigned ld,
                              const T* y, unsigned ldy) {
  constexpr unsigned TVEC = 16 / (unsigned)sizeof(T);
  const unsigned ldp = (ld + TVEC - 1) / TVEC * TVEC;
  auto window = [&](unsigned w) { return planes * (size_t)g->N * w * sizeof(T) < ((size_t)1 << 31); };
  const bool pad_pays = opt.tile_pad == 2 || ld >= 2 ||
                        (size_t)g->nnz_int * (sizeof(T) + 4) >= ((size_t)20 << 20);
  WorkPanels p;
  p.tile_direct = tiles && tile_usable<T>(g, opt, ld, y, ldy) && window(ld);
  p.padded = !p.tile_direct && tiles && opt.tile_pad && pad_pays && tile_geometry<T>(g, opt, ldp) && window(ldp);
  p.ldw = p.padded ? ldp : ld;
  return p;
}

template <typename T>
static StepArgs<T> step_base(const gspx_graph* g, unsigned ld, T* y, unsigned ldy) {
  StepArgs<T> a{};
  a.rowptr = g->rptr.as<int>();
  a.col = g->rcol.as<int>();
  a.val = g->fval.as<T>();
  a.N = (int)g->N;
  a.ld = ld;
  a.curbytes = (u32)((size_t)g->N * ld * sizeof(T));
  a.y = y;
  a.ldy = ldy;
  a.perm = g->has_perm ? g->perm.as<int>() : nullptr;
  return a;
}

static int batch_events(gspx_ctx* ctx, size_t& ev_idx, hipEvent_t ev[4]) {
  for (int i = 0; i < 4; ++i) ev[i] = pool_event(ctx, ++ev_idx);
  if (!ev[0] || !ev[1] || !ev[2] || !ev[3]) return set_err(GSPX_ERR_HIP, "hipEventCreate failed");
  HIPCHK(hipEventRecord(ev[0], ctx->stream));
  return GSPX_OK;
}

static int batch_width(const gspx_graph* g, size_t elt, size_t panels, int64_t Nsig, int64_t* width) {
  const Options& opt = g->ctx->opt;
  const size_t rowb = (size_t)g->N * elt;
  int64_t max_ld = (int64_t)((((size_t)1 << 31) - 65536) / rowb);
  if (max_ld < 1)
    return set_err(GSPX_ERR_INVALID, "graph too large: one signal column exceeds 2 GiB");
  const size_t budget = (size_t)std::max<int64_t>(opt.ws_limit_mb, 1) << 20;
  max_ld = std::min<int64_t>(max_ld, std::max<int64_t>(1, (int64_t)(budget / (rowb * panels))));
  if (opt.max_batch > 0) max_ld = std::min<int64_t>(max_ld, opt.max_batch);
  if (max_ld < Nsig && max_ld >= 4) max_ld &= ~(int64_t)3;
  *width = max_ld;
  return GSPX_OK;
}

template <typename Batch>
static int run_batches(gspx_graph* g, int64_t Nsig, int64_t width, int steps, const Batch& batch) {
  gspx_ctx* ctx = g->ctx;
  size_t ev_idx = 0;
  HIPCHK(hipEventRecord(ctx->ev[0], ctx->stream));
  for (int64_t c0 = 0; c0 < Nsig; c0 += width)
    CHK(batch(c0, (unsigned)std::min<int64_t>(width, Nsig - c0), ev_idx));
  HIPCHK(hipEventRecord(ctx->ev[1], ctx->stream));
  HIPCHK(hipStreamSynchronize(ctx->stream));
  float ms = 0;
  HIPCHK(hipEventElapsedTime(&ms, ctx->ev[0], ctx->ev[1]));
  ctx->timing[0] = ms;
  double phase[3] = {0, 0, 0};
  for (size_t i = 0; i + 3 < ev_idx; i += 4)
    for (size_t j = 0; j < 3; ++j) {
      float t = 0;
      HIPCHK(hipEventElapsedTime(&t, ctx->ev_pool[i + j], ctx->ev_pool[i + j + 1]));
      phase[j] += t;
    }
  ctx->timing[1] = phase[1];
  ctx->timing[2] = (double)(ev_idx / 4) * steps;
  ctx->timing[3] = phase[0];
  ctx->timing[4] = phase[2];
  return GSPX_OK;
}

template <typename T>
static int run_batch(gspx_graph* g, int nf, int M, const std::vector<double>& cp, const T* x,
                     unsigned ldx, T* y, unsigned ldy, unsigned ld, bool deferred,
                     bool acc_existing, bool final_to_y, size_t& ev_idx, const SqNorms* sq = nullptr,
                     const SlotDots* sd = nullptr) {
  gspx_ctx* ctx = g->ctx;
  const Options& opt = ctx->opt;
  hipStream_t st = ctx->stream;
  const int N = (int)g->N;
  const int K = M - 1;
  const WorkPanels wp = work_panels<T>(g, opt, deferred || nf == 1, 1, ld, y, ldy);
  const bool tile_direct = wp.tile_direct, padded = wp.padded;
  const unsigned ldw = wp.ldw;
  const size_t U = (size_t)N * ldw;
  const Shape shape = choose_shape(opt, sizeof(T), ld, vec_cap(4, ldy, y));
  const int* perm = g->has_perm ? g->perm.as<int>() : nullptr;

  std::vector<PlanStep> plan;
  if (deferred)
    make_plan_deferred(nf, M, plan);
  else
    make_plan_fused(nf, M, cp, acc_existing, final_to_y, plan);

  std::vector<T> hw;
  if (deferred) {
    hw.resize((size_t)nf * M);
    for (size_t i = 0; i < hw.size(); ++i) hw[i] = (T)cp[i];
  } else {
    hw.resize((size_t)K * nf * 3);
    for (int k = 0; k < K; ++k)
      for (int j = 0; j < nf * 3; ++j) hw[(size_t)k * nf * 3 + j] = (T)plan[(size_t)k].w[(size_t)j];
  }
  const bool cap = ctx->capturing;
  if (!cap) {
    CHK(ctx->ws_w.ensure(hw.size() * sizeof(T) + 64));
    HIPCHK(hipMemcpyAsync(ctx->ws_w.p, hw.data(), hw.size() * sizeof(T), hipMemcpyHostToDevice, st));
    HIPCHK(hipStreamSynchronize(st));
  }

  const size_t nslots = deferred ? (size_t)M : 2;
  const size_t SU = U;
  CHK(ctx->ws_t.ensure(nslots * SU * sizeof(T) + 256));
  if (!deferred) CHK(ctx->ws_r.ensure((size_t)nf * U * sizeof(T) + 256));
  T* slots = ctx->ws_t.as<T>();
  T* racc = ctx->ws_r.as<T>();

  hipEvent_t ev[4] = {};
  if (!cap) CHK(batch_events(ctx, ev_idx, ev));
  const bool tile_ok = tile_direct || padded;
  const unsigned char* xb = (const unsigned char*)x;
  const unsigned char* yb = (const unsigned char*)y;
  const size_t xbytes = (size_t)N * ldx * sizeof(T), ybytes = (size_t)nf * N * ldy * sizeof(T);
  const bool fuse_in = tile_direct && !deferred && opt.fuse_input && g->gt_slow == 0 && ldx == ld &&
                       ((uintptr_t)x % 16) == 0 && (xb + xbytes <= yb || yb + ybytes <= xb) &&
                       (!g->has_perm || (g->gt_ns1 > 0 && (!cap || g->gt_s1nat.p)));
  if (fuse_in) {
    CHK(ensure_s1nat(g, st));
  } else if (padded) {
    const unsigned nb = (unsigned)std::min<size_t>((U + 255) / 256, 65536);
    hipLaunchKernelGGL((k_permute_in_pad<T>), dim3(nb), dim3(256), 0, st, x, ldx, slots, ldw, ld, N, perm);
  } else {
    launch_permute_in<T>(x, ldx, slots, ld, N, perm, vec_cap(shape.vec, ldx, x), st);
  }
  if (!cap) HIPCHK(hipEventRecord(ev[1], st));

  CHK(prepare_coff<T>(g, shape, ld, st));
  StepArgs<T> a = step_base<T>(g, ld, y, ldy);
  a.nf = nf;
  a.racc = racc;
  for (int k = 1; k <= K; ++k) {
    const PlanStep& ps = plan[(size_t)k - 1];
    if (tile_ok) {
      TileArgs<T> t{};
      if (deferred) {
        t.cur = slots + (size_t)(k - 1) * SU;
        t.old = (k >= 2 && ps.gamma != 0.0) ? slots + (size_t)(k - 2) * SU : t.cur;
        t.out = slots + (size_t)k * SU;
      } else {
        t.cur = slots + (size_t)((k - 1) & 1) * SU;
        t.old = ps.gamma == 0.0 ? t.cur : slots + (size_t)(k & 1) * SU;
        t.out = slots + (size_t)(k & 1) * SU;
        if (fuse_in && k == 1) {
          t.cur = x;
          t.old = x;
          t.s1rows = g->has_perm ? g->gt_s1nat.as<int>() : nullptr;
        } else if (fuse_in && k == 2) {
          t.old = x;
          t.old_rows = perm;
        }
      }
      t.racc = racc;
      t.y = y;
      t.ldy = ldy;
      t.perm = perm;
      t.scale = (T)ps.scale;
      t.gamma = (T)ps.gamma;
      t.beta = T(0);
      t.flush = ps.flush;
      t.final = padded ? 0 : ps.final;
      t.reverse = (opt.alternate_sweep && (k & 1)) ? 1 : 0;
      if (ps.flush) {
        t.wn = (T)ps.w[0];
        t.wc = (T)ps.w[1];
        t.wo = (T)ps.w[2];
      }
      CHK(launch_step_tile<T>(g, opt, t, ldw, st));
      continue;
    }
    if (deferred) {
      a.cur = slots + (size_t)(k - 1) * SU;
      a.old = k >= 2 ? slots + (size_t)(k - 2) * SU : slots;
      a.out = slots + (size_t)k * SU;
    } else {
      a.cur = slots + (size_t)((k - 1) & 1) * SU;
      a.old = slots + (size_t)(k & 1) * SU;
      a.out = slots + (size_t)(k & 1) * SU;
    }
    if (ps.gamma == 0.0) a.old = a.cur;
    a.scale = (T)ps.scale;
    a.gamma = (T)ps.gamma;
    a.flush = ps.flush;
    a.final = ps.final;
    a.reverse = (opt.alternate_sweep && (k & 1)) ? 1 : 0;
    a.wts = ctx->ws_w.as<T>() + (size_t)(k - 1) * nf * 3;
    launch_step<T>(ctx, a, shape, opt, st, g->coff.as<unsigned>());
  }
  if (!cap) HIPCHK(hipEventRecord(ev[2], st));
  if (deferred && sq) {
    CHK(launch_combine_sqnorm<T>(ctx, slots, M, SU, ldw, N, ld, *sq, st));
  } else if (deferred && sd) {
    CHK(launch_slot_dots<T>(ctx, slots, M, SU, ldw, N, ld, *sd, st));
  } else if (deferred) {
    launch_combine<T>(slots, M, SU, ctx->ws_w.as<T>(), M, nf, N, ld, y, ldy, (size_t)N * ldy, perm,
                      padded ? 1 : vec_cap(shape.vec, ldy, y), st, ldw);
  } else if (padded && final_to_y) {
    const unsigned nb = (unsigned)std::min<size_t>(((size_t)N * ld + 255) / 256, 65536);
    hipLaunchKernelGGL((k_permute_out_pad<T>), dim3(nb), dim3(256), 0, st, racc, ldw, y, ldy, ld, N, perm);
  }
  if (!cap) {
    HIPCHK(hipEventRecord(ev[3], st));
    HIPCHK(hipGetLastError());
  }
  return GSPX_OK;
}

template <typename T>
static int run_synthesis_batch(gspx_graph* g, int nf, int M, const std::vector<double>& cp,
                               const T* x, size_t plane_x, unsigned ldx, T* y, unsigned ldy,
                               unsigned ld, size_t& ev_idx) {
  gspx_ctx* ctx = g->ctx;
  Options opt = ctx->opt;
  hipStream_t st = ctx->stream;
  const int N = (int)g->N;
  const int K = M - 1;
  const WorkPanels wp = work_panels<T>(g, opt, true, (size_t)nf, ld, y, ldy);
  const bool padded = wp.padded;
  const unsigned ldw = wp.ldw;
  const size_t U = (size_t)N * ldw;
  const Shape shape = choose_shape(opt, sizeof(T), ld, vec_cap(4, ldy, y));
  const int* perm = g->has_perm ? g->perm.as<int>() : nullptr;

  std::vector<T> hw((size_t)M * nf);
  for (int k = 0; k < M; ++k)
    for (int f = 0; f < nf; ++f) hw[(size_t)k * nf + f] = (T)cp[(size_t)f * M + k];
  CHK(ctx->ws_w.ensure(hw.size() * sizeof(T) + 64));
  HIPCHK(hipMemcpyAsync(ctx->ws_w.p, hw.data(), hw.size() * sizeof(T), hipMemcpyHostToDevice, st));
  HIPCHK(hipStreamSynchronize(st));
  CHK(ctx->ws_r.ensure((size_t)nf * U * sizeof(T) + 256));
  CHK(ctx->ws_t.ensure(2 * U * sizeof(T) + 256));
  T* S = ctx->ws_r.as<T>();
  T* B[2] = {ctx->ws_t.as<T>(), ctx->ws_t.as<T>() + U};

  hipEvent_t ev[4];
  CHK(batch_events(ctx, ev_idx, ev));
  for (int f = 0; f < nf; ++f) {
    const T* xf = x + (size_t)f * plane_x;
    if (padded) {
      const unsigned nbp = (unsigned)std::min<size_t>((U + 255) / 256, 65536);
      hipLaunchKernelGGL((k_permute_in_pad<T>), dim3(nbp), dim3(256), 0, st, xf, ldx, S + (size_t)f * U, ldw, ld, N, perm);
      continue;
    }
    launch_permute_in<T>(xf, ldx, S + (size_t)f * U, ld, N, perm, vec_cap(shape.vec, ldx, xf), st);
  }
  HIPCHK(hipEventRecord(ev[1], st));

  CHK(prepare_coff<T>(g, shape, ld, st));
  StepArgs<T> a = step_base<T>(g, ld, y, ldy);
  a.nf = 1;
  a.nin = nf;
  a.racc = S;
  const bool tile_ok = wp.tile_direct || padded;
  for (int k = K; k >= 0; --k) {
    if (tile_ok) {
      TileArgs<T> t{};
      const bool has_b2 = (k + 2 <= K);
      t.cur = (k == K) ? S : B[(k + 1) & 1];
      t.old = (k < K && has_b2) ? B[k & 1] : t.cur;
      t.out = B[k & 1];
      t.racc = B[0];
      t.y = y;
      t.ldy = ldy;
      t.perm = perm;
      t.scale = (k == K) ? T(0) : (k == 0 ? T(0.5) : T(1));
      t.gamma = (k < K && has_b2) ? T(-1) : T(0);
      t.beta = T(0);
      t.inp = S;
      t.wts = ctx->ws_w.as<T>() + (size_t)k * nf;
      t.nin = nf;
      t.flush = 0;
      t.final = (k == 0 && !padded) ? 1 : 0;
      t.reverse = (opt.alternate_sweep && (k & 1)) ? 1 : 0;
      CHK(launch_step_tile<T>(g, opt, t, ldw, st));
      continue;
    }
    a.wts = ctx->ws_w.as<T>() + (size_t)k * nf;
    a.final = (k == 0) ? 1 : 0;
    a.flush = 0;
    if (k == K) {
      a.cur = S;
      a.old = S;
      a.out = B[k & 1];
      a.scale = T(0);
      a.gamma = T(0);
    } else {
      a.cur = B[(k + 1) & 1];
      a.out = B[k & 1];
      const bool has_b2 = (k + 2 <= K);
      a.old = has_b2 ? B[k & 1] : a.cur;
      a.gamma = has_b2 ? T(-1) : T(0);
      a.scale = (k == 0) ? T(0.5) : T(1);
    }
    a.reverse = (opt.alternate_sweep && (k & 1)) ? 1 : 0;
    launch_step<T>(ctx, a, shape, opt, st, g->coff.as<unsigned>());
  }
  HIPCHK(hipEventRecord(ev[2], st));
  if (padded) {
    const unsigned nbp = (unsigned)std::min<size_t>(((size_t)N * ld + 255) / 256, 65536);
    hipLaunchKernelGGL((k_permute_out_pad<T>), dim3(nbp), dim3(256), 0, st, B[0], ldw, y, ldy, ld, N, perm);
  }
  HIPCHK(hipEventRecord(ev[3], st));
  HIPCHK(hipGetLastError());
  return GSPX_OK;
}

template <typename T>
static int run_program_batch(gspx_graph* g, int S, const double* sc, const double* be, const double* ga, bool old_is_x,
                             const T* x, unsigned ldx, T* y, unsigned ldy, unsigned ld, size_t& ev_idx) {
  gspx_ctx* ctx = g->ctx;
  Options opt = ctx->opt;
  hipStream_t st = ctx->stream;
  const int N = (int)g->N;
  const size_t U = (size_t)N * ld;
  const Shape shape = choose_shape(opt, sizeof(T), ld, vec_cap(4, ldy, y));
  const int* perm = g->has_perm ? g->perm.as<int>() : nullptr;

  const T hw[3] = {T(1), T(0), T(0)};
  CHK(ctx->ws_w.ensure(sizeof(hw) + 64));
  HIPCHK(hipMemcpyAsync(ctx->ws_w.p, hw, sizeof(hw), hipMemcpyHostToDevice, st));
  HIPCHK(hipStreamSynchronize(st));
  CHK(ctx->ws_t.ensure((old_is_x ? 3 : 2) * U * sizeof(T) + 256));
  T* X = ctx->ws_t.as<T>();
  T* H[2] = {X + U, old_is_x ? X + 2 * U : X};

  hipEvent_t ev[4];
  CHK(batch_events(ctx, ev_idx, ev));
  launch_permute_in<T>(x, ldx, X, ld, N, perm, vec_cap(shape.vec, ldx, x), st);
  HIPCHK(hipEventRecord(ev[1], st));

  CHK(prepare_coff<T>(g, shape, ld, st));
  StepArgs<T> a = step_base<T>(g, ld, y, ldy);
  a.nf = 1;
  a.racc = H[0];
  a.wts = ctx->ws_w.as<T>();
  const bool tile_ok = tile_usable<T>(g, opt, ld, y, ldy);
  for (int s = 0; s < S; ++s) {
    const bool last = s == S - 1;
    const T* cur = (s == 0) ? X : H[(s - 1) & 1];
    T* out = H[s & 1];
    const T* old = old_is_x ? X : (const T*)out;
    const double gam = (!old_is_x && s == 0) ? 0.0 : ga[s];
    if (tile_ok) {
      TileArgs<T> t{};
      t.cur = cur;
      t.old = gam == 0.0 ? cur : old;
      t.out = out;
      t.racc = H[0];
      t.y = y;
      t.ldy = ldy;
      t.perm = perm;
      t.scale = (T)sc[s];
      t.beta = (T)be[s];
      t.gamma = (T)gam;
      t.flush = 0;
      t.final = last ? 1 : 0;
      t.reverse = (opt.alternate_sweep && (s & 1)) ? 1 : 0;
      CHK(launch_step_tile<T>(g, opt, t, ld, st));
      continue;
    }
    a.cur = cur;
    a.old = gam == 0.0 ? cur : old;
    a.out = out;
    a.scale = (T)sc[s];
    a.beta = (T)be[s];
    a.gamma = (T)gam;
    a.flush = last ? 1 : 0;
    a.final = last ? 1 : 0;
    a.reverse = (opt.alternate_sweep && (s & 1)) ? 1 : 0;
    launch_step<T>(ctx, a, shape, opt, st, g->coff.as<unsigned>());
  }
  HIPCHK(hipEventRecord(ev[2], st));
  HIPCHK(hipEventRecord(ev[3], st));
  HIPCHK(hipGetLastError());
  return GSPX_OK;
}

template <typename T>
static int filter_dev_t(gspx_graph* g, double lmax, int Nf, int M, const double* coeffs,
                        int64_t Nsig, const T* x, T* y, int mode) {
  gspx_ctx* ctx = g->ctx;
  const Options& opt = ctx->opt;
  const int64_t N = g->N;
  for (int i = 0; i < 5; ++i) ctx->timing[i] = 0;
  ctx->step_kinds[0] = ctx->step_kinds[1] = 0;
  if (N == 0 || Nsig == 0) return GSPX_OK;
  CHK(ensure_factor<T>(g, lmax));
  std::vector<double> cp;
  halve_c0(Nf, M, coeffs, cp);

  const int K = M - 1;
  const bool analysis = mode == GSPX_ANALYSIS;
  bool deferred = analysis && (opt.combine == 2 || (opt.combine == 0 && Nf >= 2));
  const size_t budget = (size_t)std::max<int64_t>(opt.ws_limit_mb, 1) << 20;
  if (deferred && (size_t)N * sizeof(T) * M * (size_t)std::min<int64_t>(Nsig, 4) > budget) deferred = false;
  int64_t max_ld = 0;
  CHK(batch_width(g, sizeof(T), deferred ? (size_t)M : (size_t)(2 + Nf), Nsig, &max_ld));

  std::vector<unsigned char> key;
  const bool graph_mode =
      analysis && Nsig <= max_ld &&
      (opt.graph_launch == 1 || (opt.graph_launch == 2 && (size_t)N * Nsig * sizeof(T) <= ((size_t)32 << 20)));
  if (graph_mode) {
    auto put = [&](const void* p, size_t n) {
      const unsigned char* b = (const unsigned char*)p;
      key.insert(key.end(), b, b + n);
    };
    put(&g->generation, sizeof(g->generation));
    const void* ptrs[] = {x, y, ctx->ws_t.p, ctx->ws_r.p, ctx->ws_w.p, g->coff.p, g->gt_hdr.p, g->gt_s1nat.p,
                          g->fval.p, g->perm.p};
    put(ptrs, sizeof(ptrs));
    put(&lmax, sizeof(lmax));
    put(&g->fval_lmax, sizeof(g->fval_lmax));
    put(&Nf, sizeof(Nf));
    put(&M, sizeof(M));
    put(&Nsig, sizeof(Nsig));
    put(cp.data(), cp.size() * sizeof(double));
    put(&opt, sizeof(opt));
    put(&g->gt_rows, sizeof(g->gt_rows));
    put(&g->gt_slow, sizeof(g->gt_slow));
    if (ctx->graph_exec && !key.empty() && ctx->graph_key == key) {
      HIPCHK(hipEventRecord(ctx->ev[0], ctx->stream));
      HIPCHK(hipGraphLaunch(ctx->graph_exec, ctx->stream));
      HIPCHK(hipEventRecord(ctx->ev[1], ctx->stream));
      HIPCHK(hipStreamSynchronize(ctx->stream));
      float gms = 0;
      HIPCHK(hipEventElapsedTime(&gms, ctx->ev[0], ctx->ev[1]));
      ctx->timing[0] = gms;
      ctx->timing[1] = gms;
      ctx->timing[2] = (double)K;
      ctx->step_kinds[0] = ctx->graph_kinds[0];
      ctx->step_kinds[1] = ctx->graph_kinds[1];
      return GSPX_OK;
    }
    if (!key.empty() && ctx->seen_key == key) {
      if (ctx->graph_exec) {
        (void)hipGraphExecDestroy(ctx->graph_exec);
        ctx->graph_exec = nullptr;
      }
      hipGraph_t graph = nullptr;
      size_t dummy = 0;
      HIPCHK(hipStreamBeginCapture(ctx->stream, hipStreamCaptureModeThreadLocal));
      ctx->capturing = true;
      const int rc = run_batch<T>(g, Nf, M, cp, x, (unsigned)Nsig, y, (unsigned)Nsig, (unsigned)Nsig,
                                  deferred, false, true, dummy);
      ctx->capturing = false;
      const hipError_t ce = hipStreamEndCapture(ctx->stream, &graph);
      if (rc != GSPX_OK || ce != hipSuccess || !graph) {
        if (graph) (void)hipGraphDestroy(graph);
        (void)hipGetLastError();
        ctx->seen_key.clear();
      } else {
        const hipError_t ie = hipGraphInstantiate(&ctx->graph_exec, graph, nullptr, nullptr, 0);
        (void)hipGraphDestroy(graph);
        if (ie == hipSuccess) {
          ctx->graph_key = key;
          ctx->graph_kinds[0] = ctx->step_kinds[0];
          ctx->graph_kinds[1] = ctx->step_kinds[1];
          return filter_dev_t<T>(g, lmax, Nf, M, coeffs, Nsig, x, y, mode);
        }
        ctx->graph_exec = nullptr;
        (void)hipGetLastError();
      }
    }
  }
  if (ctx->graph_exec && ctx->graph_key != key) replay_reset(ctx);
  ctx->seen_key = key;

  const size_t plane_x = (size_t)N * Nsig;
  return run_batches(g, Nsig, max_ld, K, [&](int64_t c0, unsigned ld, size_t& ev_idx) -> int {
    if (analysis)
      return run_batch<T>(g, Nf, M, cp, x + c0, (unsigned)Nsig, y + c0, (unsigned)Nsig, ld, deferred, false, true,
                          ev_idx);
    if (opt.synthesis != 1)
      return run_synthesis_batch<T>(g, Nf, M, cp, x + c0, plane_x, (unsigned)Nsig, y + c0, (unsigned)Nsig, ld, ev_idx);
    for (int f = 0; f < Nf; ++f) {
      std::vector<double> cf(cp.begin() + (size_t)f * M, cp.begin() + (size_t)(f + 1) * M);
      CHK(run_batch<T>(g, 1, M, cf, x + (size_t)f * plane_x + c0, (unsigned)Nsig, y + c0, (unsigned)Nsig, ld, false,
                       f > 0, f == Nf - 1, ev_idx));
    }
    return GSPX_OK;
  });
}

template <typename T>
static int program_dev_t(gspx_graph* g, double lmax, int S, const double* sc, const double* be, const double* ga,
                         bool old_is_x, int64_t Nsig, const T* x, T* y) {
  gspx_ctx* ctx = g->ctx;
  replay_reset(ctx);
  for (int i = 0; i < 5; ++i) ctx->timing[i] = 0;
  ctx->step_kinds[0] = ctx->step_kinds[1] = 0;
  if (g->N == 0 || Nsig == 0) return GSPX_OK;
  CHK(ensure_factor<T>(g, lmax));
  int64_t max_ld = 0;
  CHK(batch_width(g, sizeof(T), 3, Nsig, &max_ld));
  CHK(run_batches(g, Nsig, max_ld, S, [&](int64_t c0, unsigned ld, size_t& ev_idx) {
    return run_program_batch<T>(g, S, sc, be, ga, old_is_x, x + c0, (unsigned)Nsig, y + c0, (unsigned)Nsig, ld, ev_idx);
  }));
  ctx->timing[4] = 0;
  return GSPX_OK;
}

static void horner_program(int K, const double* nodes, const double* dc, std::vector<double>& sc,
                           std::vector<double>& be, std::vector<double>& ga) {
  sc.assign((size_t)K, 0.0);
  be.assign((size_t)K, 0.0);
  ga.assign((size_t)K, 0.0);
  for (int s = 0; s < K; ++s) {
    const int j = K - 1 - s;
    if (s == 0) {
      sc[0] = 0.5 * dc[K];
      be[0] = 0.0;
      ga[0] = dc[j] - dc[K] * nodes[j];
    } else {
      sc[(size_t)s] = 0.5;
      be[(size_t)s] = -nodes[j];
      ga[(size_t)s] = dc[j];
    }
  }
}

template <typename Run>
static int device_call(gspx_graph* g, int64_t Nsig, const void* x, void* y, double* kernel_ms, const Run& run) {
  HIPCHK(hipSetDevice(g->ctx->device));
  const int rc = g->dtype == GSPX_F32 ? run((const float*)x, (float*)y, Nsig) : run((const double*)x, (double*)y, Nsig);
  if (rc == GSPX_OK && kernel_ms) *kernel_ms = g->ctx->timing[0];
  return rc;
}

static int check_program_args(gspx_graph* g, double lmax, int S, const double* scale, const double* beta,
                              const double* gamma, int64_t Nsig, const void* x, void* y) {
  if (!g) return set_err(GSPX_ERR_INVALID, "null graph");
  if (S < 1) return set_err(GSPX_ERR_COEFF, "The coefficients have an invalid shape");
  if (!scale || !beta || !gamma) return set_err(GSPX_ERR_INVALID, "null program");
  if (Nsig < 0) return set_err(GSPX_ERR_INVALID, "negative number of signals");
  if (!(lmax > 0.0) || !std::isfinite(lmax))
    return set_err(GSPX_ERR_INVALID, "lmax must be positive and finite (got %g)", lmax);
  if (Nsig > 0 && g->N > 0 && (!x || !y)) return set_err(GSPX_ERR_INVALID, "null signal pointer");
  for (int i = 0; i < S; ++i)
    if (!std::isfinite(scale[i]) || !std::isfinite(beta[i]) || !std::isfinite(gamma[i]))
      return set_err(GSPX_ERR_INVALID, "non-finite program coefficient");
  if (Nsig >= ((int64_t)1 << 31) / 16) return set_err(GSPX_ERR_INVALID, "too many signals");
  return GSPX_OK;
}

extern "C" int gspx_poly_program_dev(gspx_graph* g, double lmax, int S, const double* scale, const double* beta,
                                     const double* gamma, int old_is_x, int64_t Nsig, const void* x_dev, void* y_dev,
                                     double* kernel_ms) {
  if (g) replay_reset(g->ctx);
  CHK(check_program_args(g, lmax, S, scale, beta, gamma, Nsig, x_dev, y_dev));
  return device_call(g, Nsig, x_dev, y_dev, kernel_ms, [&](auto x, auto y, int64_t n) {
    return program_dev_t(g, lmax, S, scale, beta, gamma, old_is_x != 0, n, x, y);
  });
}

static int check_newton_args(gspx_graph* g, double lmax, int K, const double* nodes, const double* dcoef,
                             int64_t Nsig, const void* x, void* y) {
  if (!g) return set_err(GSPX_ERR_INVALID, "null graph");
  if (K < 1) return set_err(GSPX_ERR_COEFF, "The coefficients have an invalid shape");
  if (!nodes || !dcoef) return set_err(GSPX_ERR_INVALID, "null nodes / coefficients");
  if (Nsig < 0) return set_err(GSPX_ERR_INVALID, "negative number of signals");
  if (!(lmax > 0.0) || !std::isfinite(lmax))
    return set_err(GSPX_ERR_INVALID, "lmax must be positive and finite (got %g)", lmax);
  if (Nsig > 0 && g->N > 0 && (!x || !y))
    return set_err(GSPX_ERR_INVALID, "null signal pointer");
  for (int i = 0; i < K; ++i)
    if (!std::isfinite(nodes[i])) return set_err(GSPX_ERR_INVALID, "non-finite node");
  for (int i = 0; i <= K; ++i)
    if (!std::isfinite(dcoef[i])) return set_err(GSPX_ERR_INVALID, "non-finite coefficient");
  if (Nsig >= ((int64_t)1 << 31) / 16) return set_err(GSPX_ERR_INVALID, "too many signals");
  return GSPX_OK;
}

extern "C" int gspx_newton_filter_dev(gspx_graph* g, double lmax, int K, const double* nodes,
                                      const double* dcoef, int64_t Nsig, const void* x_dev,
                                      void* y_dev, double* kernel_ms) {
  if (g) replay_reset(g->ctx);
  CHK(check_newton_args(g, lmax, K, nodes, dcoef, Nsig, x_dev, y_dev));
  std::vector<double> sc, be, ga;
  horner_program(K, nodes, dcoef, sc, be, ga);
  return device_call(g, Nsig, x_dev, y_dev, kernel_ms, [&](auto x, auto y, int64_t n) {
    return program_dev_t(g, lmax, K, sc.data(), be.data(), ga.data(), true, n, x, y);
  });
}

template <typename Prepare, typename Run>
static int host_call(gspx_graph* g, int64_t Nsig, int in_planes, int out_planes, const void* x_host, void* y_host,
                     double* kernel_ms, const Prepare& prepare, const Run& run) {
  gspx_ctx* ctx = g->ctx;
  HIPCHK(hipSetDevice(ctx->device));
  if (g->N == 0 || Nsig <= 0) {
    if (kernel_ms) *kernel_ms = 0;
    return GSPX_OK;
  }
  CHK(prepare());
  const size_t e = elt_size(g->dtype);
  std::vector<int64_t> widths;
  int threads = 1;
  host_pipeline_shape(ctx->opt, e, g->N, Nsig, in_planes + out_planes, &widths, &threads);
  if (widths.size() >= 2) {
    if (!ctx->pipe) ctx->pipe = new HostPipe();
    replay_reset(ctx);
    const int rc = g->dtype == GSPX_F32
                       ? filter_host_pipelined<float>(g, Nsig, in_planes, out_planes, (const float*)x_host,
                                                      (float*)y_host, widths, threads, kernel_ms, run)
                       : filter_host_pipelined<double>(g, Nsig, in_planes, out_planes, (const double*)x_host,
                                                       (double*)y_host, widths, threads, kernel_ms, run);
    if (rc != GSPX_HOSTPIPE_UNAVAILABLE) return rc;
  }
  if (ctx->pipe) {
    ctx->pipe->timing[6] = 0;
    ctx->pipe->timeline.clear();
  }
  const size_t n_in = (size_t)in_planes * g->N * Nsig * e, n_out = (size_t)out_planes * g->N * Nsig * e;
  CHK(ctx->io_x.ensure(n_in));
  CHK(ctx->io_y.ensure(n_out));
  HIPCHK(hipMemcpyAsync(ctx->io_x.p, x_host, n_in, hipMemcpyHostToDevice, ctx->stream));
  HIPCHK(hipStreamSynchronize(ctx->stream));
  CHK(device_call(g, Nsig, ctx->io_x.p, ctx->io_y.p, kernel_ms, run));
  HIPCHK(hipMemcpyAsync(y_host, ctx->io_y.p, n_out, hipMemcpyDeviceToHost, ctx->stream));
  HIPCHK(hipStreamSynchronize(ctx->stream));
  return GSPX_OK;
}

extern "C" int gspx_newton_filter(gspx_graph* g, double lmax, int K, const double* nodes,
                                  const double* dcoef, int64_t Nsig, const void* x_host,
                                  void* y_host, double* kernel_ms) {
  if (!g) return set_err(GSPX_ERR_INVALID, "null graph");
  if (Nsig > 0 && g->N > 0 && (!x_host || !y_host))
    return set_err(GSPX_ERR_INVALID, "null signal pointer");
  if (K < 1) return set_err(GSPX_ERR_COEFF, "The coefficients have an invalid shape");
  std::vector<double> sc, be, ga;
  auto prepare = [&]() -> int {
    CHK(check_newton_args(g, lmax, K, nodes, dcoef, Nsig, x_host, y_host));
    horner_program(K, nodes, dcoef, sc, be, ga);
    return GSPX_OK;
  };
  return host_call(g, Nsig, 1, 1, x_host, y_host, kernel_ms, prepare, [&](auto x, auto y, int64_t n) {
    return program_dev_t(g, lmax, K, sc.data(), be.data(), ga.data(), true, n, x, y);
  });
}

static int check_filter_args(gspx_graph* g, double lmax, int Nf, int M, const double* coeffs,
                             int64_t Nsig, const void* x, void* y, int mode) {
  if (!g) return set_err(GSPX_ERR_INVALID, "null graph");
  if (M < 2) return set_err(GSPX_ERR_COEFF, "The coefficients have an invalid shape");
  if (Nf < 1) return set_err(GSPX_ERR_INVALID, "Nf must be >= 1");
  if (!coeffs) return set_err(GSPX_ERR_INVALID, "null coefficients");
  if (Nsig < 0) return set_err(GSPX_ERR_INVALID, "negative number of signals");
  if (mode != GSPX_ANALYSIS && mode != GSPX_SYNTHESIS)
    return set_err(GSPX_ERR_INVALID, "unknown mode %d", mode);
  if (!(lmax > 0.0) || !std::isfinite(lmax))
    return set_err(GSPX_ERR_INVALID, "lmax must be positive and finite (got %g)", lmax);
  if (Nsig > 0 && g->N > 0 && (!x || !y)) return set_err(GSPX_ERR_INVALID, "null signal pointer");
  for (int64_t i = 0; i < (int64_t)Nf * M; ++i)
    if (!std::isfinite(coeffs[i])) return set_err(GSPX_ERR_INVALID, "non-finite coefficient");
  if (Nsig >= ((int64_t)1 << 31) / 16) return set_err(GSPX_ERR_INVALID, "too many signals");
  return GSPX_OK;
}

extern "C" int gspx_cheby_filter_dev(gspx_graph* g, double lmax, int Nf, int M,
                                     const double* coeffs, int64_t Nsig, const void* x_dev,
                                     void* y_dev, int mode, double* kernel_ms) {
  CHK(check_filter_args(g, lmax, Nf, M, coeffs, Nsig, x_dev, y_dev, mode));
  return device_call(g, Nsig, x_dev, y_dev, kernel_ms, [&](auto x, auto y, int64_t n) {
    return filter_dev_t(g, lmax, Nf, M, coeffs, n, x, y, mode);
  });
}

extern "C" int gspx_cheby_filter(gspx_graph* g, double lmax, int Nf, int M, const double* coeffs,
                                 int64_t Nsig, const void* x_host, void* y_host, int mode,
                                 double* kernel_ms) {
  CHK(check_filter_args(g, lmax, Nf, M, coeffs, Nsig, x_host, y_host, mode));
  const bool analysis = mode == GSPX_ANALYSIS;
  return host_call(g, Nsig, analysis ? 1 : Nf, analysis ? Nf : 1, x_host, y_host, kernel_ms,
                   [] { return (int)GSPX_OK; }, [&](auto x, auto y, int64_t n) {
                     return filter_dev_t(g, lmax, Nf, M, coeffs, n, x, y, mode);
                   });
}

template <typename T>
static int sqnorms_dev_t(gspx_graph* g, double lmax, int Nf, int M, const double* coeffs, int64_t Nsig, const T* x,
                         double* out) {
  gspx_ctx* ctx = g->ctx;
  const int64_t N = g->N;
  for (int i = 0; i < 5; ++i) ctx->timing[i] = 0;
  ctx->step_kinds[0] = ctx->step_kinds[1] = 0;
  if (Nsig == 0) return GSPX_OK;
  if (N == 0) {
    std::fill(out, out + (size_t)Nf * Nsig, 0.0);
    return GSPX_OK;
  }
  int64_t width = 0;
  CHK(batch_width(g, sizeof(T), (size_t)M, Nsig, &width));
  std::vector<double> cp;
  halve_c0(Nf, M, coeffs, cp);
  const int ldc = (Nf + SQ_PASS - 1) / SQ_PASS * SQ_PASS;
  std::vector<double> hc((size_t)M * ldc, 0.0);
  for (int f = 0; f < Nf; ++f)
    for (int k = 0; k < M; ++k) hc[(size_t)k * ldc + f] = cp[(size_t)f * M + k];
  const size_t cbytes = (hc.size() * sizeof(double) + 255) / 256 * 256, obytes = (size_t)Nf * Nsig * sizeof(double);
  const int64_t first = std::min<int64_t>(width, Nsig), last = Nsig - (Nsig - 1) / width * width;
  const size_t parts = std::max(sqnorm_parts(ctx, (int)N, (unsigned)first), sqnorm_parts(ctx, (int)N, (unsigned)last));
  CHK(ctx->ws_sq.ensure(cbytes + obytes + 256));
  CHK(ctx->ws_sqp.ensure(parts * sizeof(double) + 256));
  hipStream_t st = ctx->stream;
  HIPCHK(hipMemcpyAsync(ctx->ws_sq.p, hc.data(), hc.size() * sizeof(double), hipMemcpyHostToDevice, st));
  HIPCHK(hipStreamSynchronize(st));
  CHK(ensure_factor<T>(g, lmax));
  double* outd = (double*)((char*)ctx->ws_sq.p + cbytes);
  const SqNorms sq{ctx->ws_sq.as<double>(), ldc, Nf, outd, (size_t)Nsig, ctx->ws_sqp.as<double>()};
  CHK(run_batches(g, Nsig, width, M - 1, [&](int64_t c0, unsigned ld, size_t& ev_idx) -> int {
    SqNorms b = sq;
    b.out = outd + c0;
    return run_batch<T>(g, Nf, M, cp, x + c0, (unsigned)Nsig, (T*)nullptr, ld, ld, true, false, false, ev_idx, &b);
  }));
  HIPCHK(hipMemcpyAsync(out, outd, obytes, hipMemcpyDeviceToHost, st));
  HIPCHK(hipStreamSynchronize(st));
  return GSPX_OK;
}

extern "C" int gspx_cheby_sqnorms_dev(gspx_graph* g, double lmax, int Nf, int M, const double* coeffs, int64_t Nsig,
                                      const void* x_dev, double* out, double* kernel_ms) {
  if (g) replay_reset(g->ctx);
  CHK(check_filter_args(g, lmax, Nf, M, coeffs, Nsig, x_dev, out, GSPX_ANALYSIS));
  if (M > 256) return set_err(GSPX_ERR_INVALID, "gspx_cheby_sqnorms_dev: at most 256 coefficients per filter");
  if (Nsig > 0 && !out) return set_err(GSPX_ERR_INVALID, "gspx_cheby_sqnorms_dev: null output");
  return device_call(g, Nsig, x_dev, out, kernel_ms, [&](auto x, auto, int64_t n) {
    return sqnorms_dev_t(g, lmax, Nf, M, coeffs, n, x, out);
  });
}

template <typename T>
static int moments_dev_t(gspx_graph* g, double lmax, int M, int64_t Nsig, const T* x, double* out) {
  gspx_ctx* ctx = g->ctx;
  const int64_t N = g->N;
  for (int i = 0; i < 5; ++i) ctx->timing[i] = 0;
  ctx->step_kinds[0] = ctx->step_kinds[1] = 0;
  if (Nsig == 0) return GSPX_OK;
  if (N == 0) {
    std::fill(out, out + (size_t)M * Nsig, 0.0);
    return GSPX_OK;
  }
  const int S = M / 2 + 1, rows = 2 * S - 1;
  int64_t width = 0;
  CHK(batch_width(g, sizeof(T), (size_t)S, Nsig, &width));
  const std::vector<double> cp((size_t)S, 0.0);
  const size_t obytes = (size_t)rows * Nsig * sizeof(double);
  const int64_t first = std::min<int64_t>(width, Nsig), last = Nsig - (Nsig - 1) / width * width;
  const size_t parts =
      std::max(dots_parts(ctx, (int)N, (unsigned)first, S), dots_parts(ctx, (int)N, (unsigned)last, S));
  CHK(ctx->ws_sq.ensure(obytes + 256));
  CHK(ctx->ws_sqp.ensure(parts * sizeof(double) + 256));
  hipStream_t st = ctx->stream;
  CHK(ensure_factor<T>(g, lmax));
  double* outd = ctx->ws_sq.as<double>();
  CHK(run_batches(g, Nsig, width, S - 1, [&](int64_t c0, unsigned ld, size_t& ev_idx) -> int {
    const SlotDots b{outd + c0, (size_t)Nsig, ctx->ws_sqp.as<double>()};
    return run_batch<T>(g, 1, S, cp, x + c0, (unsigned)Nsig, (T*)nullptr, ld, ld, true, false, false, ev_idx, nullptr,
                        &b);
  }));
  std::vector<double> d((size_t)rows * Nsig);
  HIPCHK(hipMemcpyAsync(d.data(), outd, obytes, hipMemcpyDeviceToHost, st));
  HIPCHK(hipStreamSynchronize(st));
  const double *a = d.data(), *b = d.data() + (size_t)S * Nsig;
  for (int k = 0; k < M; ++k)
    for (int64_t j = 0; j < Nsig; ++j) {
      const double dot = (k & 1 ? b : a)[(size_t)(k / 2) * Nsig + j];
      out[(size_t)k * Nsig + j] = k < 2 ? dot : 2.0 * dot - (k & 1 ? b : a)[j];
    }
  return GSPX_OK;
}

extern "C" int gspx_cheby_moments_dev(gspx_graph* g, double lmax, int M, int64_t Nsig, const void* x_dev, double* out,
                                      double* kernel_ms) {
  if (!g) return set_err(GSPX_ERR_INVALID, "null graph");
  if (M < 2 || M > 2048) return set_err(GSPX_ERR_INVALID, "gspx_cheby_moments_dev: 2 to 2048 moments (got %d)", M);
  if (Nsig < 0) return set_err(GSPX_ERR_INVALID, "negative number of signals");
  if (!(lmax > 0.0) || !std::isfinite(lmax))
    return set_err(GSPX_ERR_INVALID, "lmax must be positive and finite (got %g)", lmax);
  if (Nsig > 0 && (!out || (g->N > 0 && !x_dev))) return set_err(GSPX_ERR_INVALID, "null signal pointer");
  if (Nsig >= ((int64_t)1 << 31) / 16) return set_err(GSPX_ERR_INVALID, "too many signals");
  replay_reset(g->ctx);
  return device_call(g, Nsig, x_dev, out, kernel_ms, [&](auto x, auto, int64_t n) {
    return moments_dev_t(g, lmax, M, n, x, out);
  });
}

extern "C" int gspx_poly_program(gspx_graph* g, double lmax, int S, const double* scale, const double* beta,
                                 const double* gamma, int old_is_x, int64_t Nsig, const void* x_host, void* y_host,
                                 double* kernel_ms) {
  if (!g) return set_err(GSPX_ERR_INVALID, "null graph");
  if (Nsig > 0 && g->N > 0 && (!x_host || !y_host)) return set_err(GSPX_ERR_INVALID, "null signal pointer");
  if (S < 1) return set_err(GSPX_ERR_COEFF, "The coefficients have an invalid shape");
  auto prepare = [&] { return check_program_args(g, lmax, S, scale, beta, gamma, Nsig, x_host, y_host); };
  return host_call(g, Nsig, 1, 1, x_host, y_host, kernel_ms, prepare, [&](auto x, auto y, int64_t n) {
    return program_dev_t(g, lmax, S, scale, beta, gamma, old_is_x != 0, n, x, y);
  });
}
```

pygsp_amd/csrc/gspx_tile_kernels.hip.h:

```cpp
#pragma once

#include "gspx_kernels.hip.h"

namespace gspx {

template <typename T> struct TileArgs {
  const int* rowptr;
  const int* col;
  const T* val;
  const int* hdr;
  const int* s1rows;
  const u8* lidx;
  const T* cur;
  const T* old;
  const int* old_rows;
  T* out;
  T* racc;
  T* y;
  const int* perm;
  int N;
  u32 ld, ldy;
  u32 panel_bytes, val_bytes, lidx_bytes;
  int nb, ncol, per_xcd;
  int lds_bytes;
  T scale, gamma;
  T beta;
  T wn, wc, wo;
  const T* inp;
  const T* wts;
  int nin;
  int flush;
  int final;
  int reverse;
  int nt;
};

constexpr int GSPX_TILE_BR = 64;
constexpr int GSPX_TILE_MAXN1 = 160;

template <typename T, int NCOL, int LG, bool OLDNAT, bool ACC = true> struct TileSchedule {
  static constexpr bool PF = !OLDNAT;
  static constexpr bool TILE_LAST = PF && LG == 16;
  static constexpr bool PF_ENTRIES = PF;
  static constexpr bool META_AFTER = !OLDNAT && LG == 16 && NCOL == 0;
  static constexpr bool EARLY_OLD = !ACC && PF && LG == 16 && NCOL == 2 && sizeof(T) == 4;
};

template <typename T, int NCOL, int LG = 16, bool OLDNAT = false, bool INS = false, int NT = 512, int CL = LG,
          int MIX = 0, bool ACC = true>
__global__ __launch_bounds__(NT, 4) void k_step_tile(const TileArgs<T> a) {
  static_assert(NT == 512 || (NT == 64 * LG && NCOL == 1) || (CL < LG && NCOL == 1 && NT % 64 == 0 && NT % CL == 0),
                "narrow builds: one row per group, one chunk per row");
  constexpr int BR = GSPX_TILE_BR;
  static_assert(CL <= LG && (BR % (NT / CL)) == 0, "compute groups must tile the block's rows");
  constexpr int MAXN1 = GSPX_TILE_MAXN1;
  typedef TileSchedule<T, NCOL, LG, OLDNAT, ACC> Sched;
  constexpr bool PF = Sched::PF;
  constexpr bool META_AFTER = Sched::META_AFTER;
  constexpr bool TILE_LAST = Sched::TILE_LAST;
  constexpr bool PF_ENTRIES = Sched::PF_ENTRIES;
  constexpr bool EARLY_OLD = Sched::EARLY_OLD;
  static_assert(ACC || (!OLDNAT && !INS && CL == LG), "flush-free builds: the plain flavour only");
  constexpr int VEC = 16 / (int)sizeof(T);
  typedef typename VT<T, VEC>::t V;
  typedef __attribute__((address_space(3))) void* lds_ptr;
  extern __shared__ __attribute__((aligned(16))) unsigned char gspx_smem[];

  const int tid = threadIdx.x;
  constexpr int NGD = NT / LG;
  constexpr int NG = NT / CL;
  constexpr int NE = (512 + NT - 1) / NT;
  constexpr int RPG = BR / NG;
  constexpr int ST = (MAXN1 + NGD - 1) / NGD;
  constexpr int RB = LG * 16;
  const int lane_d = tid & (LG - 1);
  const int grp_d = tid / LG;
  const int lane16 = CL == LG ? lane_d : tid % CL;
  const int grp = CL == LG ? grp_d : tid / CL;
  const int wave = tid >> 6;
  const int nwx = (int)(gridDim.x >> 3);
  const int xlo = (int)(blockIdx.x & 7) * a.per_xcd;
  int k1 = xlo + a.per_xcd;
  if (k1 > a.nb) k1 = a.nb;
  const int k0 = xlo + (int)(blockIdx.x >> 3);
  if (k0 >= k1) return;

  constexpr u32 POISON = 0x80000000u;
  const rsrc_t rcur = __builtin_amdgcn_make_buffer_rsrc((void*)a.cur, 0, a.panel_bytes, 0x00020000);
  const rsrc_t rold = __builtin_amdgcn_make_buffer_rsrc((void*)a.old, 0, a.panel_bytes, 0x00020000);
  const rsrc_t rra = __builtin_amdgcn_make_buffer_rsrc((void*)a.racc, 0, a.panel_bytes, 0x00020000);
  const rsrc_t rv = __builtin_amdgcn_make_buffer_rsrc((void*)a.val, 0, a.val_bytes, 0x00020000);
  const rsrc_t ri = __builtin_amdgcn_make_buffer_rsrc((void*)a.lidx, 0, a.lidx_bytes, 0x00020000);
  const u32 ldb = a.ld * (u32)sizeof(T);

  struct Meta { int rows[ST]; int rp[RPG + 1]; int orow[OLDNAT ? RPG : 1]; };
  const int xflip = xlo + k1 - 1;
  const bool rev = a.reverse != 0;
  auto phys = [&](int p) { return rev ? xflip - p : p; };
  auto load_hdr = [&](int p) { return *(const int4*)(a.hdr + (size_t)phys(p) * 4); };
  auto uniform = [](int4 h) {
    int4 u;
    u.x = __builtin_amdgcn_readfirstlane(h.x); u.y = __builtin_amdgcn_readfirstlane(h.y);
    u.z = __builtin_amdgcn_readfirstlane(h.z); u.w = __builtin_amdgcn_readfirstlane(h.w);
    return u;
  };
  auto load_meta = [&](int k, const int4& h) {
    Meta m;
    const int n1 = h.y;
#pragma unroll
    for (int t = 0; t < ST; ++t) {
      const int u = grp_d + NGD * t;
      m.rows[t] = a.s1rows[h.x + (u < n1 ? u : 0)];
    }
    int r = phys(k) * BR + grp * RPG;
#pragma unroll
    for (int t = 0; t < RPG + 1; ++t) m.rp[t] = a.rowptr[(r + t) <= a.N ? (r + t) : a.N];
    if constexpr (OLDNAT) {
#pragma unroll
      for (int t = 0; t < RPG; ++t) m.orow[t] = a.old_rows[(r + t) < a.N ? (r + t) : a.N - 1];
    }
    return m;
  };
  V* const tile = (V*)gspx_smem;
  auto stage = [&](const Meta& m, int n1, u32 cb) {
#pragma unroll
    for (int t = 0; t < ST; ++t) {
      if (grp_d + NGD * t < n1)
        __builtin_amdgcn_raw_ptr_buffer_load_lds(rcur, (lds_ptr)(gspx_smem + (wave * (64 / LG) + NGD * t) * RB), 16,
                                                 (u32)m.rows[t] * ldb + cb, 0, 0, 0);
    }
  };
  auto chunk_off_d = [&](int c) {
    const u32 col0 = (c * LG + lane_d) * VEC;
    return col0 < a.ld ? col0 * (u32)sizeof(T) : POISON;
  };
  auto chunk_off = [&](int c) {
    const u32 col0 = (c * LG + lane16) * VEC;
    return col0 < a.ld ? col0 * (u32)sizeof(T) : POISON;
  };

  V ov[RPG], ra[ACC ? RPG : 1];
  V ov2[EARLY_OLD ? RPG : 1];
  u32x4 ev[NE], ei = 0;
#pragma unroll
  for (int q = 0; q < NE; ++q) ev[q] = 0;
  auto prefetch_rows = [&](const Meta& m, int blk, int c, V (&dst)[RPG]) {
    const int r0 = phys(blk) * BR + grp * RPG;
    const u32 cb = chunk_off(c);
#pragma unroll
    for (int t = 0; t < RPG; ++t) {
      const u32 off = (r0 + t < a.N && cb != POISON) ? (u32)(r0 + t) * ldb + cb : POISON;
      u32 oo = a.gamma != T(0) ? off : POISON;
      if constexpr (OLDNAT) oo = (off != POISON && a.gamma != T(0)) ? (u32)m.orow[t] * ldb + cb : POISON;
      if (a.nt & 4) dst[t] = __builtin_bit_cast(V, __builtin_amdgcn_raw_buffer_load_b128(rold, oo, 0, 2));
      else dst[t] = VT<T, VEC>::bload(rold, oo);
      if constexpr (ACC) {
        const u32 ro = a.flush == 2 ? off : POISON;
        if (a.nt & 2) ra[t] = __builtin_bit_cast(V, __builtin_amdgcn_raw_buffer_load_b128(rra, ro, 0, 2));
        else ra[t] = VT<T, VEC>::bload(rra, ro);
      }
    }
  };
  auto prefetch_entries = [&](const int4& h) {
    const int nv16 = (h.w * (int)sizeof(T) + 15) >> 4, ni16 = (h.w + 15) >> 4;
    const u32 io = tid < ni16 ? (u32)h.z + tid * 16u : POISON;
#pragma unroll
    for (int q = 0; q < NE; ++q) {
      const int i = tid + q * NT;
      const u32 vo = i < nv16 ? (u32)h.z * (u32)sizeof(T) + i * 16u : POISON;
      if (a.nt & 1) ev[q] = __builtin_amdgcn_raw_buffer_load_b128(rv, vo, 0, 2);
      else ev[q] = __builtin_amdgcn_raw_buffer_load_b128(rv, vo, 0, 0);
    }
    if (a.nt & 1) ei = __builtin_amdgcn_raw_buffer_load_b128(ri, io, 0, 2);
    else ei = __builtin_amdgcn_raw_buffer_load_b128(ri, io, 0, 0);
  };

  int4 H = uniform(load_hdr(k0));
  Meta M = load_meta(k0, H);
  int k = k0, kn = k0 + nwx, knn = k0 + 2 * nwx;
  int4 Hn = uniform(load_hdr(kn < k1 ? kn : k0));
  if constexpr (!TILE_LAST) {
    if (H.y >= 0) stage(M, H.y, chunk_off_d(0));
  }
  if constexpr (EARLY_OLD) {
#pragma unroll
    for (int t = 0; t < RPG; ++t) ov[t] = 0, ov2[t] = 0;
    if (a.gamma != T(0)) prefetch_rows(M, k0, 0, ov);
  } else if constexpr (PF) {
    prefetch_rows(M, k0, 0, ov);
  }
  if constexpr (PF_ENTRIES) {
    if (H.y >= 0) prefetch_entries(H);
  }
  if constexpr (TILE_LAST) {
    __builtin_amdgcn_sched_barrier(0);
    if (H.y >= 0) stage(M, H.y, chunk_off_d(0));
    __builtin_amdgcn_sched_barrier(0);
  }

  auto pass = [&](const int c, const bool first, const bool last, V (&ovc)[RPG], V (&ovn)[RPG])
                  __attribute__((always_inline)) {
    const int n1 = H.y, rp0 = H.z, ent = H.w;
    const bool fast = n1 >= 0;
    T* const mval = (T*)(tile + (fast ? n1 : 0) * LG);
    u8* const midx = (u8*)(mval + ent);
    const int row0 = phys(k) * BR + grp * RPG;
    int rs[RPG + 1];
#pragma unroll
    for (int t = 0; t < RPG + 1; ++t) rs[t] = M.rp[t] & ~3;
    const u32 col0 = (c * LG + lane16) * VEC;
    const bool on = col0 < a.ld;
    const u32 cb = on ? col0 * (u32)sizeof(T) : POISON;
    if constexpr (!PF) prefetch_rows(M, k, c, ovc);
    V ins[INS ? RPG : 1];
#pragma unroll
    for (int t = 0; t < (INS ? RPG : 1); ++t) ins[t] = 0;
    if constexpr (INS) {
      const rsrc_t rin = __builtin_amdgcn_make_buffer_rsrc((void*)a.inp, 0, a.panel_bytes * (u32)a.nin, 0x00020000);
      for (int f = 0; f < a.nin; ++f) {
        const T w = a.wts[f];
#pragma unroll
        for (int t = 0; t < RPG; ++t) {
          const u32 off = (row0 + t < a.N) ? (u32)(row0 + t) * ldb + cb : POISON;
          ins[t] += w * VT<T, VEC>::bload(rin, off == POISON ? POISON : off + (u32)f * a.panel_bytes);
        }
      }
    }
    if constexpr (!PF_ENTRIES) {
      if (first && fast) prefetch_entries(H);
    }
    int4 Hv = Hn;
    if constexpr (!META_AFTER) {
      if (last) {
        M = load_meta(kn < k1 ? kn : k, Hn);
        Hv = load_hdr(knn < k1 ? knn : k);
      }
    }
    __builtin_amdgcn_sched_barrier(0);
    if (first && fast) {
      const int nv16 = (ent * (int)sizeof(T) + 15) >> 4, ni16 = (ent + 15) >> 4;
#pragma unroll
      for (int q = 0; q < NE; ++q)
        if (tid + q * NT < nv16) *(u32x4*)((unsigned char*)mval + (tid + q * NT) * 16) = ev[q];
      if (tid < ni16) *(u32x4*)((unsigned char*)midx + tid * 16) = ei;
      for (int i = tid + NE * NT; i < nv16; i += NT)
        *(u32x4*)((unsigned char*)mval + i * 16) =
            __builtin_amdgcn_raw_buffer_load_b128(rv, (u32)rp0 * (u32)sizeof(T) + i * 16u, 0, 0);
      for (int i = tid + NT; i < ni16; i += NT)
        *(u32x4*)((unsigned char*)midx + i * 16) =
            __builtin_amdgcn_raw_buffer_load_b128(ri, (u32)rp0 + i * 16u, 0, 0);
    }
    if constexpr (TILE_LAST && !META_AFTER) {
      constexpr int NMETA = ST + RPG + 1 + 1;
      static_assert(NMETA < 16, "vmcnt immediate");
      if (last && !INS) __builtin_amdgcn_s_waitcnt(0x0070 | NMETA);
      else __builtin_amdgcn_s_waitcnt(0x0070);
    } else {
      __builtin_amdgcn_s_waitcnt(0x0070);
    }
    if constexpr (MIX != 2) __syncthreads();
    if constexpr (META_AFTER) {
      if (last) {
        M = load_meta(kn < k1 ? kn : k, Hn);
        Hv = load_hdr(knn < k1 ? knn : k);
      }
    }
    if constexpr (EARLY_OLD) {
      if ((!last || kn < k1) && a.gamma != T(0)) prefetch_rows(M, last ? kn : k, last ? 0 : c + 1, ovn);
    }
    __builtin_amdgcn_sched_barrier(0);
    V nv[RPG], res[ACC ? RPG : 1];
#pragma unroll
    for (int t = 0; t < RPG; ++t) {
      const int s = rs[t], e = rs[t + 1];
      V acc = 0, self = 0;
      if (MIX && fast) {
        self = tile[(int)midx[s - rp0] * LG + lane16];
        acc = mval[s - rp0] * self;
      } else if (fast) {
        acc = lds_row_dot<T, V, LG, u8>(mval + (s - rp0), midx + (s - rp0), row0 + t < a.N ? e - s : 0, tile, lane16,
                                        self);
      } else if (row0 + t < a.N) {
        for (int j = s; j < e; ++j) {
          const int cc = a.col[j];
          const V xv = VT<T, VEC>::bload(rcur, cc < a.N ? (u32)cc * ldb + cb : POISON);
          if (j == s) self = xv;
          acc += a.val[j] * xv;
        }
      }
      if constexpr (ACC) {
        nv[t] = a.scale * acc + a.gamma * ovc[t] + a.beta * self;
      } else {
        nv[t] = __builtin_elementwise_fma((V)a.beta, self, __builtin_elementwise_fma((V)a.gamma, ovc[t], a.scale * acc));
      }
      if constexpr (INS) nv[t] += ins[t];
      if constexpr (ACC) {
        res[t] = a.wn * nv[t] + a.wc * self + a.wo * ovc[t];
        if (a.flush == 2) res[t] += ra[t];
      }
    }
    __builtin_amdgcn_s_waitcnt(0xC07F);
    if constexpr (MIX != 2) __builtin_amdgcn_s_barrier();
    bool more = true;
    if (last) {
      const int4 Hnn = uniform(Hv);
      H = Hn;
      Hn = Hnn;
      more = kn < k1;
    }
    __builtin_amdgcn_sched_barrier(0);
    if constexpr (!PF) {
      if (more && H.y >= 0) stage(M, H.y, chunk_off_d(last ? 0 : c + 1));
    }
#pragma unroll
    for (int t = 0; t < RPG; ++t) {
      const int row = row0 + t;
      if (row < a.N && on) {
        if (a.final && (!ACC || !a.flush)) {
          const size_t orow = a.perm ? (size_t)a.perm[row] : (size_t)row;
          *(V*)(a.y + orow * a.ldy + col0) = nv[t];
          continue;
        }
        if (a.nt & 8) __builtin_nontemporal_store(nv[t], (V*)(a.out + (size_t)row * a.ld + col0));
        else *(V*)(a.out + (size_t)row * a.ld + col0) = nv[t];
        if constexpr (ACC) {
          if (a.flush) {
            if (a.final) {
              const size_t orow = a.perm ? (size_t)a.perm[row] : (size_t)row;
              *(V*)(a.y + orow * a.ldy + col0) = res[t];
            } else {
              if (a.nt & 2) __builtin_nontemporal_store(res[t], (V*)(a.racc + (size_t)row * a.ld + col0));
              else *(V*)(a.racc + (size_t)row * a.ld + col0) = res[t];
            }
          }
        }
      }
    }
    __builtin_amdgcn_sched_barrier(0);
    if constexpr (PF) {
      if (more) {
        const int nc = last ? 0 : c + 1;
        if constexpr (!TILE_LAST) {
          if (H.y >= 0) stage(M, H.y, chunk_off_d(nc));
        }
        if constexpr (!EARLY_OLD) prefetch_rows(M, last ? kn : k, nc, ovn);
        if constexpr (PF_ENTRIES) {
          if (last && H.y >= 0) prefetch_entries(H);
        }
        if constexpr (TILE_LAST) {
          __builtin_amdgcn_sched_barrier(0);
          if (H.y >= 0) stage(M, H.y, chunk_off_d(nc));
          __builtin_amdgcn_sched_barrier(0);
        }
      }
    }
    if (last) {
      k = kn;
      kn = knn;
      knn += nwx;
    }
    return more;
  };
  if constexpr (EARLY_OLD) {
    static_assert(NCOL == 2, "an even number of passes per block");
    for (;;) {
      pass(0, true, false, ov, ov2);
      if (!pass(1, false, true, ov2, ov)) break;
    }
  } else {
    for (;;) {
      if constexpr (NCOL == 1) {
        if (!pass(0, true, true, ov, ov)) break;
      } else if constexpr (NCOL == 2) {
        pass(0, true, false, ov, ov);
        if (!pass(1, false, true, ov, ov)) break;
      } else {
        bool more = true;
        for (int c = 0; c < a.ncol; ++c) more = pass(c, c == 0, c == a.ncol - 1, ov, ov);
        if (!more) break;
      }
    }
  }
}

}

namespace gspx {

constexpr int GSPX_TILE_SORTCAP = 4096;
constexpr int GSPX_TILE_TMPCAP = 256;

__global__ __launch_bounds__(256) void k_tiles_unique(const int* __restrict__ rowptr,
                                                      const int* __restrict__ col, int N, int nb,
                                                      int* __restrict__ tmp, int* __restrict__ n1) {
  constexpr int BR = GSPX_TILE_BR;
  __shared__ unsigned keys[GSPX_TILE_SORTCAP];
  __shared__ int wsum[4];
  const int b = blockIdx.x;
  const int r0 = b * BR, r1 = min(r0 + BR, N);
  const int e0 = rowptr[r0] & ~3, e1 = rowptr[r1] & ~3;
  const int ent = e1 - e0;
  if (ent > GSPX_TILE_SORTCAP) {
    if (threadIdx.x == 0) n1[b] = GSPX_TILE_TMPCAP + 1;
    return;
  }
  int n = 1;
  while (n < ent) n <<= 1;
  for (int i = threadIdx.x; i < n; i += 256) {
    unsigned v = 0xFFFFFFFFu;
    if (i < ent) {
      const int c = col[e0 + i];
      if (c < N) v = (unsigned)c;
    }
    keys[i] = v;
  }
  __syncthreads();
  for (int k = 2; k <= n; k <<= 1)
    for (int j = k >> 1; j > 0; j >>= 1) {
      for (int i = threadIdx.x; i < n; i += 256) {
        const int l = i ^ j;
        if (l > i) {
          const unsigned a = keys[i], c = keys[l];
          const bool up = (i & k) == 0;
          if ((a > c) == up) {
            keys[i] = c;
            keys[l] = a;
          }
        }
      }
      __syncthreads();
    }
  int base = 0;
  for (int i0 = 0; i0 < n; i0 += 256) {
    const int i = i0 + threadIdx.x;
    const bool first = i < n && keys[i] != 0xFFFFFFFFu && (i == 0 || keys[i] != keys[i - 1]);
    const unsigned long long m = __ballot(first);
    const int lane = threadIdx.x & 63, wv = threadIdx.x >> 6;
    const int before = __popcll(m & ((1ull << lane) - 1));
    if (lane == 0) wsum[wv] = __popcll(m);
    __syncthreads();
    int off = base;
    for (int w = 0; w < wv; ++w) off += wsum[w];
    if (first && off + before < GSPX_TILE_TMPCAP) tmp[(size_t)b * GSPX_TILE_TMPCAP + off + before] = (int)keys[i];
    const int total = wsum[0] + wsum[1] + wsum[2] + wsum[3];
    __syncthreads();
    base += total;
  }
  if (threadIdx.x == 0) n1[b] = base;
}

__global__ __launch_bounds__(256) void k_tiles_fill(const int* __restrict__ rowptr,
                                                    const int* __restrict__ col, int N, int nb,
                                                    const int* __restrict__ tmp, const int* __restrict__ n1,
                                                    const int* __restrict__ s1lo, int esz, int lds_bytes,
                                                    int* __restrict__ s1rows, u8* __restrict__ lidx,
                                                    int* __restrict__ hdr, int* __restrict__ nslow) {
  constexpr int BR = GSPX_TILE_BR, MAXN1 = GSPX_TILE_MAXN1, ROWB = 256;
  const int b = blockIdx.x;
  const int r0 = b * BR, r1 = min(r0 + BR, N);
  const int e0 = rowptr[r0] & ~3, e1 = rowptr[r1] & ~3;
  const int ent = e1 - e0;
  const int n = n1[b];
  const long need = (long)n * ROWB + (((long)ent * esz + 15) & ~15L) + (((long)ent * 2 + 15) & ~15L) + 32;
  const bool fast = n <= MAXN1 && need <= lds_bytes;
  const int lo = s1lo[b];
  if (threadIdx.x == 0) {
    hdr[(size_t)b * 4 + 0] = lo;
    hdr[(size_t)b * 4 + 1] = fast ? n : -1;
    hdr[(size_t)b * 4 + 2] = e0;
    hdr[(size_t)b * 4 + 3] = ent;
    if (!fast) atomicAdd(nslow, 1);
  }
  const int* list = tmp + (size_t)b * GSPX_TILE_TMPCAP;
  const int keep = n <= GSPX_TILE_TMPCAP ? n : 0;
  for (int i = threadIdx.x; i < keep; i += 256) s1rows[lo + i] = list[i];
  for (int i = threadIdx.x; i < ent; i += 256) {
    const int c = col[e0 + i];
    int pos = 0;
    if (c < N && fast) {
      int a = 0, z = n;
      while (a < z) {
        const int mid = (a + z) >> 1;
        if (list[mid] < c) a = mid + 1; else z = mid;
      }
      pos = a;
    }
    lidx[e0 + i] = (u8)pos;
  }
}
__global__ void k_tiles_entmax(const int* __restrict__ hdr, int nb, int* __restrict__ out) {
  const int b = blockIdx.x * 256 + threadIdx.x;
  if (b < nb && hdr[(size_t)b * 4 + 1] >= 0) atomicMax(out, hdr[(size_t)b * 4 + 3]);
}

__global__ void k_tiles_keep(const int* __restrict__ n1, int nb, int* __restrict__ keep) {
  const int b = blockIdx.x * blockDim.x + threadIdx.x;
  if (b <= nb) keep[b] = (b < nb && n1[b] <= GSPX_TILE_TMPCAP) ? n1[b] : 0;
}

}
```

pygsp_amd/engine.py:

```python
import ctypes
import sys
import threading

import numpy as np
from scipy import sparse

from . import _capi


class Context:

    def __init__(self, device=0):
        lib = _capi.load()
        h = ctypes.c_void_p()
        _capi.check(lib.gspx_ctx_create(int(device), ctypes.byref(h)))
        self._h = h
        self.device = int(device)
        self._init_pool()

    def _init_pool(self):
        self._pool, self._pooled, self._pool_lock = {}, 0, threading.RLock()

    def close(self):
        if getattr(self, "_h", None):
            self.clear_pool()
            _capi.load().gspx_ctx_destroy(self._h)
            self._h = None

    def set_option(self, key, value):
        _capi.check(_capi.load().gspx_ctx_set_option(self._h, key.encode(), int(value)))

    def get_option(self, key):
        v = ctypes.c_int64(0)
        _capi.check(_capi.load().gspx_ctx_get_option(self._h, key.encode(), ctypes.byref(v)))
        return v.value

    def sync(self):
        _capi.check(_capi.load().gspx_ctx_sync(self._h))

    def last_timing(self):
        out = (ctypes.c_double * 5)()
        _capi.check(_capi.load().gspx_last_timing(self._h, out))
        return {"total_ms": out[0], "steps_ms": out[1], "step_launches": int(out[2]),
                "permute_ms": out[3], "combine_ms": out[4]}

    def last_step_kinds(self):
        out = (ctypes.c_int64 * 2)()
        _capi.check(_capi.load().gspx_last_step_kinds(self._h, out))
        return {"tile": int(out[0]), "plain": int(out[1])}

    def last_host_timing(self):
        out = (ctypes.c_double * 9)()
        _capi.check(_capi.load().gspx_last_host_timing(self._h, out))
        if out[6] == 0:
            return None
        return {"wall_ms": out[0], "pack_ms": out[1], "h2d_ms": out[2], "kernel_ms": out[3], "d2h_ms": out[4],
                "unpack_ms": out[5], "batches": int(out[6]), "signals_per_batch": int(out[7]),
                "host_threads_per_direction": int(out[8])}

    def last_host_timeline(self):
        n = ctypes.c_int(0)
        _capi.check(_capi.load().gspx_last_host_timeline(self._h, None, 0, ctypes.byref(n)))
        out = np.zeros((max(n.value, 0), 6))
        if n.value > 0:
            _capi.check(_capi.load().gspx_last_host_timeline(self._h, _capi.ptr(out), out.size, ctypes.byref(n)))
        return out

    def alloc(self, nbytes):
        return DeviceBuffer(self, nbytes)

    POOL_BYTES = 8 << 30

    def pooled_bytes(self):
        with self._pool_lock:
            return self._pooled

    def take(self, nbytes):
        nbytes = max(int(nbytes), 16)
        with self._pool_lock:
            stack = self._pool.get(nbytes)
            if stack:
                self._pooled -= nbytes
                return stack.pop()
        return DeviceBuffer(self, nbytes)

    def give(self, buf):
        with self._pool_lock:
            if not getattr(buf, "_h", None) or buf.ctx is not self or self._pooled + buf.nbytes > self.POOL_BYTES:
                buf.free()
                return
            self._pool.setdefault(buf.nbytes, []).append(buf)
            self._pooled += buf.nbytes

    def clear_pool(self):
        with self._pool_lock:
            stacks, self._pool, self._pooled = list(self._pool.values()), {}, 0
        for stack in stacks:
            for buf in stack:
                buf.free()

    def call(self, fn, *args):
        rc = fn(*args)
        if rc == _capi.ERR_OOM and self.pooled_bytes() > 0:
            self.clear_pool()
            rc = fn(*args)
        _capi.check(rc)

    def bench_copy(self, nbytes=1 << 30, iters=10):
        v = ctypes.c_double(0)
        _capi.check(_capi.load().gspx_bench_copy(self._h, int(nbytes), int(iters), ctypes.byref(v)))
        return v.value

    def bench_read(self, nbytes, passes=50):
        v = ctypes.c_double(0)
        _capi.check(_capi.load().gspx_bench_read(self._h, int(nbytes), int(passes), ctypes.byref(v)))
        return v.value

    def bench_streams(self, bytes_per_stream, n_read, n_write, nt=0, workgroups_per_cu=8, iters=5):
        v = ctypes.c_double(0)
        _capi.check(_capi.load().gspx_bench_streams(self._h, int(bytes_per_stream), int(n_read), int(n_write), int(nt),
                                                    int(workgroups_per_cu), int(iters), ctypes.byref(v)))
        return v.value

    def bench_gather(self, panel_rows, row_bytes, n_gathers, in_flight=8, blocks=1, p_intra=0.0, workgroups_per_cu=8,
                     iters=5):
        ms, gb = ctypes.c_double(0), ctypes.c_double(0)
        _capi.check(_capi.load().gspx_bench_gather(self._h, int(panel_rows), int(row_bytes), int(n_gathers),
                                                   int(in_flight), int(blocks), float(p_intra), int(workgroups_per_cu),
                                                   int(iters), ctypes.byref(ms), ctypes.byref(gb)))
        return ms.value, gb.value

    def upload(self, arr):
        arr = np.ascontiguousarray(arr)
        buf = DeviceBuffer(self, arr.nbytes)
        buf.upload(arr)
        return buf

    def _temporaries(self):
        return _Temporaries(self)

    def identity_panel(self, buf, N, j0, w, dtype):
        _capi.check(_capi.load().gspx_identity_panel_dev(self._h, _capi.dtype_code(dtype), int(N), int(j0), int(w),
                                                        ctypes.c_void_p(buf.ptr)))


_default_ctx = {}
_default_lock = threading.Lock()


def default_context(device=0):
    with _default_lock:
        ctx = _default_ctx.get(device)
        if ctx is None:
            ctx = Context(device)
            _default_ctx[device] = ctx
        return ctx


class DeviceBuffer:

    def __init__(self, ctx, nbytes):
        h = ctypes.c_void_p()
        ctx.call(_capi.load().gspx_buf_alloc, ctx._h, int(nbytes), ctypes.byref(h))
        self._h = h
        self.ctx = ctx
        self.nbytes = int(nbytes)

    def free(self):
        if getattr(self, "_h", None):
            if getattr(self.ctx, "_h", None):
                _capi.load().gspx_buf_free(self._h)
            self._h = None

    def __del__(self):
        if sys.is_finalizing():
            return
        try:
            self.free()
        except Exception:
            pass

    @property
    def ptr(self):
        p = ctypes.c_void_p()
        _capi.check(_capi.load().gspx_buf_ptr(self._h, ctypes.byref(p)))
        return p.value

    def upload(self, arr):
        arr = np.ascontiguousarray(arr)
        _capi.check(_capi.load().gspx_buf_upload(self._h, _capi.ptr(arr), arr.nbytes))

    def download(self, shape, dtype):
        out = np.empty(shape, dtype=dtype)
        _capi.check(_capi.load().gspx_buf_download(self._h, _capi.ptr(out), out.nbytes))
        return out


class _Temporaries:

    def __init__(self, ctx):
        self.ctx, self._bufs = ctx, []

    def add(self, buf):
        self._bufs.append(buf)
        return buf

    def upload(self, arr):
        return self.add(self.ctx.upload(arr))

    def alloc(self, nbytes):
        return self.add(self.ctx.alloc(max(int(nbytes), 16)))

    def keep(self, buf):
        self._bufs.remove(buf)
        return buf

    def __enter__(self):
        return self

    def __exit__(self, *exc):
        for buf in self._bufs:
            buf.free()


class DeviceArray:

    __array_priority__ = 100

    def __init__(self, buf, cube, dtype):
        self._buf, self.ctx = buf, buf.ctx
        self.cube = tuple(int(d) for d in cube)
        self.dtype = np.dtype(dtype)
        self.shape = tuple(d for d in self.cube if d != 1)

    @classmethod
    def from_host(cls, ctx, array, dtype=np.float64):
        a = np.asanyarray(array)
        if np.iscomplexobj(a):
            raise TypeError("complex signals are not supported by the Chebyshev path")
        if a.ndim < 1 or a.ndim > 3:
            raise ValueError("At most 3 dimensions: #nodes x #signals x #features.")
        cube = a.reshape(a.shape + (1,) * (3 - a.ndim))
        planes = np.ascontiguousarray(np.moveaxis(cube, 2, 0), dtype=dtype)
        buf = ctx.take(max(planes.nbytes, 16))
        if planes.nbytes:
            buf.upload(planes)
        out = cls(buf, cube.shape, dtype)
        out.shape = tuple(a.shape)
        return out

    @classmethod
    def empty(cls, ctx, cube, dtype):
        n = int(np.prod(cube)) * np.dtype(dtype).itemsize
        return cls(ctx.take(max(n, 16)), cube, dtype)

    @property
    def ndim(self):
        return len(self.shape)

    @property
    def size(self):
        return int(np.prod(self.cube))

    @property
    def nbytes(self):
        return self.size * self.dtype.itemsize

    @property
    def ptr(self):
        if self._buf is None:
            raise ValueError("the device array has been freed")
        return self._buf.ptr

    def planes(self, signals, features):
        N, S0, F0 = self.cube
        if S0 * F0 != signals * features:
            raise ValueError("cannot view {} signals x {} features as {} x {}".format(S0, F0, signals, features))
        if (S0, F0) == (signals, features) or self.size == 0:
            return self.ptr, self
        lib, code, cur = _capi.load(), _capi.dtype_code(self.dtype), self
        if F0 != 1:
            flat = DeviceArray.empty(self.ctx, (N, S0 * F0, 1), self.dtype)
            _capi.check(lib.gspx_planes_pack_dev(self.ctx._h, code, N, S0, F0, ctypes.c_void_p(self.ptr),
                                                 ctypes.c_void_p(flat.ptr), 0))
            cur = flat
        if features != 1:
            out = DeviceArray.empty(self.ctx, (N, signals, features), self.dtype)
            _capi.check(lib.gspx_planes_pack_dev(self.ctx._h, code, N, signals, features, ctypes.c_void_p(cur.ptr),
                                                 ctypes.c_void_p(out.ptr), 1))
            cur = out
        return cur.ptr, cur

    def numpy(self):
        N, S, F = self.cube
        if self.size == 0:
            return np.zeros(self.shape)
        planes = self._buf_download((F, N, S))
        return np.asarray(np.moveaxis(planes, 0, 2), dtype=np.float64).reshape(self.shape)

    def _buf_download(self, shape):
        if self._buf is None:
            raise ValueError("the device array has been freed")
        return self._buf.download(shape, self.dtype)

    def __array__(self, dtype=None, copy=None):
        out = self.numpy()
        return out if dtype is None else out.astype(dtype, copy=False)

    def __len__(self):
        if not self.shape:
            raise TypeError("len() of unsized object")
        return self.shape[0]

    def __repr__(self):
        return "DeviceArray(shape={}, dtype={}, device={})".format(self.shape, self.dtype, self.ctx.device)

    def free(self):
        if self._buf is not None:
            buf, self._buf = self._buf, None
            if getattr(self.ctx, "_h", None):
                self.ctx.sync()
                self.ctx.give(buf)
            else:
                buf.free()

    def __del__(self):
        if sys.is_finalizing():
            return
        try:
            self.free()
        except Exception:
            pass


def gather(parts, root_out):
    n = len(parts)
    arr = (ctypes.c_void_p * max(n, 1))(*[b._h for b in parts])
    _capi.check(_capi.load().gspx_gather(None, n, arr, root_out._h))
    return root_out


COMM_ID_BYTES = 128


def comm_available():
    return bool(_capi.load().gspx_comm_available())


def comm_unique_id():
    buf = (ctypes.c_ubyte * COMM_ID_BYTES)()
    _capi.check(_capi.load().gspx_comm_unique_id(buf))
    return bytes(buf)
# ... 1026 lines not shown
```

Measured before the change: 193.8 billion.

## Add specialized tile-step kernel builds for gamma-zero, first-flush and last-step cases

Adds compile-time KIND variants of the tile step kernel, selected per step by a new family function. The gamma-zero variant skips loading the old vector, the first-flush variant skips reading the running accumulator, and the last-step variant writes only the accumulated result to y, skipping the intermediate store. It also skips uploading the host weight table when every step uses the tile path, and adds counters and APIs to report which builds ran. The cost is more kernel instantiations and more dispatch logic to keep correct.

```diff
diff --git a/include/gspx_ext.h b/include/gspx_ext.h
--- a/include/gspx_ext.h
+++ b/include/gspx_ext.h
@@ -135,6 +135,8 @@
 
 int gspx_last_host_timing(gspx_ctx* ctx, double out[9]);
 int gspx_last_step_kinds(gspx_ctx* ctx, int64_t out[2]);
+int gspx_last_tile_builds(gspx_ctx* ctx, int64_t out[5]);
+int gspx_tile_build_family(int acc_builds, int kind_builds, int chunks, int flavour, int flush, int gamma0, int last_step);
 int gspx_last_host_timeline(gspx_ctx* ctx, double* out, int capacity, int* batches);
 
 int gspx_bench_copy(gspx_ctx* ctx, int64_t bytes, int iters, double* gbps);
diff --git a/pygsp_amd/_capi.py b/pygsp_amd/_capi.py
--- a/pygsp_amd/_capi.py
+++ b/pygsp_amd/_capi.py
@@ -134,6 +134,8 @@
     "gspx_last_timing": (_c.c_int, [_P, _c.POINTER(_c.c_double)]),
     "gspx_last_host_timing": (_c.c_int, [_P, _c.POINTER(_c.c_double)]),
     "gspx_last_step_kinds": (_c.c_int, [_P, _c.POINTER(_c.c_int64)]),
+    "gspx_last_tile_builds": (_c.c_int, [_P, _c.POINTER(_c.c_int64)]),
+    "gspx_tile_build_family": (_c.c_int, [_c.c_int] * 7),
     "gspx_last_host_timeline": (_c.c_int, [_P, _P, _c.c_int, _P]),
     "gspx_host_pipeline_describe": (_c.c_int, [_c.c_int, _c.c_int64, _c.c_int64, _c.c_int64, _c.c_int, _c.c_int64,
                                                _c.c_int64, _c.c_int, _P, _c.c_int, _P, _P]),
diff --git a/pygsp_amd/csrc/gspx_ctx.hip.h b/pygsp_amd/csrc/gspx_ctx.hip.h
--- a/pygsp_amd/csrc/gspx_ctx.hip.h
+++ b/pygsp_amd/csrc/gspx_ctx.hip.h
@@ -18,6 +18,7 @@
   int64_t copy_threads = 0;
   int64_t tile_regroup = 1;
   int64_t tile_acc_builds = 1;
+  int64_t tile_kind_builds = 1;
   int64_t tile_lg = 0;
   int64_t edge_vertex_walk = 1;
   int64_t fuse_input = 1;
@@ -58,11 +59,13 @@
   std::vector<hipEvent_t> ev_pool;
   double timing[5] = {0, 0, 0, 0, 0};
   int64_t step_kinds[2] = {0, 0};
+  int64_t tile_builds[5] = {0, 0, 0, 0, 0};
   bool capturing = false;
   std::vector<unsigned char> seen_key;
   std::vector<unsigned char> graph_key;
   hipGraphExec_t graph_exec = nullptr;
   int64_t graph_kinds[2] = {0, 0};
+  int64_t graph_builds[5] = {0, 0, 0, 0, 0};
 };
 
 static std::atomic<int> g_live_ctx[64];
@@ -277,6 +280,7 @@
     {"tile_lg", &Options::tile_lg, nullptr, nullptr},
     {"tile_regroup", &Options::tile_regroup, nullptr, nullptr},
     {"tile_acc_builds", &Options::tile_acc_builds, nullptr, nullptr},
+    {"tile_kind_builds", &Options::tile_kind_builds, nullptr, nullptr},
     {"staged_copy", &Options::staged_copy, nullptr, nullptr},
     {"staged_copy_min_mb", &Options::staged_copy_min_mb, nullptr, nullptr},
     {"copy_threads", &Options::copy_threads, nullptr, nullptr},
@@ -512,3 +516,14 @@
   out[1] = ctx->step_kinds[1];
   return GSPX_OK;
 }
+
+extern "C" int gspx_last_tile_builds(gspx_ctx* ctx, int64_t out[5]) {
+  if (!ctx || !out) return set_err(GSPX_ERR_INVALID, "null argument");
+  for (int i = 0; i < 5; ++i) out[i] = ctx->tile_builds[i];
+  return GSPX_OK;
+}
+
+static void reset_step_counts(gspx_ctx* ctx) {
+  ctx->step_kinds[0] = ctx->step_kinds[1] = 0;
+  for (int i = 0; i < 5; ++i) ctx->tile_builds[i] = 0;
+}
diff --git a/pygsp_amd/csrc/gspx_hostpipe.hip.h b/pygsp_amd/csrc/gspx_hostpipe.hip.h
--- a/pygsp_amd/csrc/gspx_hostpipe.hip.h
+++ b/pygsp_amd/csrc/gspx_hostpipe.hip.h
@@ -191,7 +191,7 @@
   }
 
   double k_ms = 0, tm[5] = {0, 0, 0, 0, 0};
-  int64_t kinds[2] = {0, 0};
+  int64_t kinds[2] = {0, 0}, builds[5] = {0, 0, 0, 0, 0};
   for (int b = 0; b < nb; ++b) {
     const int s = b % NIN, so = b & 1;
     if (!wait_for([&] { return issued >= b + 1 && shipped >= b - 1; })) break;
@@ -206,6 +206,7 @@
     k_ms += ctx->timing[0];
     for (int i = 0; i < 5; ++i) tm[i] += ctx->timing[i];
     for (int i = 0; i < 2; ++i) kinds[i] += ctx->step_kinds[i];
+    for (int i = 0; i < 5; ++i) builds[i] += ctx->tile_builds[i];
     std::lock_guard<std::mutex> lock(mu);
     computed = b + 1;
     cv.notify_all();
@@ -226,6 +227,7 @@
   (void)hipGetLastError();
   for (int i = 0; i < 5; ++i) ctx->timing[i] = tm[i];
   for (int i = 0; i < 2; ++i) ctx->step_kinds[i] = kinds[i];
+  for (int i = 0; i < 5; ++i) ctx->tile_builds[i] = builds[i];
   hp.timing[0] = std::chrono::duration<double, std::milli>(std::chrono::steady_clock::now() - wall0).count();
   hp.timing[1] = *std::max_element(pack_ms.begin(), pack_ms.end());
   hp.timing[2] = h2d_ms;
diff --git a/pygsp_amd/csrc/gspx_poly.hip.h b/pygsp_amd/csrc/gspx_poly.hip.h
--- a/pygsp_amd/csrc/gspx_poly.hip.h
+++ b/pygsp_amd/csrc/gspx_poly.hip.h
@@ -355,9 +355,25 @@
   constexpr int TVEC = 16 / (int)sizeof(T);
   return tile_geometry<T>(g, opt, ld) && (ldy % TVEC) == 0 && (((uintptr_t)y / sizeof(T)) % TVEC) == 0;
 }
+static int tile_build_family(bool acc_builds, bool kind_builds, int chunks, int flavour, int flush, bool gamma0,
+                             bool last_step) {
+  if (chunks < 1 || flavour == 2) return 0;
+  if (flush == 0) {
+    if (!acc_builds || flavour != 0) return 0;
+    return kind_builds && gamma0 ? 2 : 1;
+  }
+  if (!kind_builds) return 0;
+  if (last_step) return flavour == 0 ? 4 : 0;
+  return flush == 1 && !(flavour == 1 && chunks > 2) ? 3 : 0;
+}
+extern "C" int gspx_tile_build_family(int acc_builds, int kind_builds, int chunks, int flavour, int flush, int gamma0,
+                                      int last_step) {
+  return tile_build_family(acc_builds != 0, kind_builds != 0, chunks, flavour, flush, gamma0 != 0, last_step != 0);
+}
+
 template <typename T>
 static int launch_step_tile(gspx_graph* g, const Options& opt, TileArgs<T> t, unsigned ld, hipStream_t st,
-                            const T* vals = nullptr) {
+                            const T* vals = nullptr, bool last_step = false) {
   const size_t rowb = (size_t)ld * sizeof(T);
   int lg = rowb <= 16 ? 1 : rowb <= 32 ? 2 : rowb <= 64 ? 4 : rowb <= 128 ? 8 : 16;
   if (opt.tile_lg == 8 || opt.tile_lg == 4 || opt.tile_lg == 2) lg = rowb <= 128 ? std::max(lg, (int)opt.tile_lg) : 16;
@@ -385,6 +401,25 @@
                                     k_step_tile<T, 2, 16, false, false, 512, 16, 0, false>};
     kern = freek[ncol <= 2 ? ncol : 0];
   }
+  int family = tile_build_family(opt.tile_acc_builds != 0, opt.tile_kind_builds != 0, narrow ? 0 : ncol, flavour, t.flush,
+                                 t.gamma == T(0), last_step);
+  if (family >= 2) {
+    constexpr int L = TILE_KIND_LAST, F = TILE_KIND_FIRST, Z = TILE_KIND_GAMMA0;
+    static const kern_t zerok[3] = {k_step_tile<T, 0, 16, false, false, 512, 16, 0, false, Z>,
+                                    k_step_tile<T, 1, 16, false, false, 512, 16, 0, false, Z>,
+                                    k_step_tile<T, 2, 16, false, false, 512, 16, 0, false, Z>};
+    static const kern_t firstk[2][3] = {{k_step_tile<T, 0, 16, false, false, 512, 16, 0, true, F>,
+                                         k_step_tile<T, 1, 16, false, false, 512, 16, 0, true, F>,
+                                         k_step_tile<T, 2, 16, false, false, 512, 16, 0, true, F>},
+                                        {nullptr,
+                                         k_step_tile<T, 1, 16, true, false, 512, 16, 0, true, F>,
+                                         k_step_tile<T, 2, 16, true, false, 512, 16, 0, true, F>}};
+    static const kern_t lastk[3] = {k_step_tile<T, 0, 16, false, false, 512, 16, 0, true, L>,
+                                    k_step_tile<T, 1, 16, false, false, 512, 16, 0, true, L>,
+                                    k_step_tile<T, 2, 16, false, false, 512, 16, 0, true, L>};
+    const int nc = ncol <= 2 ? ncol : 0;
+    kern = family == 2 ? zerok[nc] : family == 3 ? firstk[flavour][nc] : lastk[nc];
+  }
   bool mix = false;
   if (opt.calib_mix && !narrow && flavour == 0) {
     static const kern_t mixk[2][3] = {
@@ -398,6 +433,7 @@
         {k_step_tile<T, 0, 16, false, false, 512, 16, 2, false>, k_step_tile<T, 1, 16, false, false, 512, 16, 2, false>,
          k_step_tile<T, 2, 16, false, false, 512, 16, 2, false>}};
     kern = (noacc ? mixfree : mixk)[opt.calib_mix == 2 ? 1 : 0][ncol <= 2 ? ncol : 0];
+    family = noacc ? 1 : 0;
     mix = true;
   }
   const int pieces = (int)(rowb / 16);
@@ -410,7 +446,7 @@
     else if (lg == 8 && pieces == 5) k2 = GSPX_CL(8, 5, 320), nt2 = 320;
     else if (lg == 16 && pieces == 10) k2 = GSPX_CL(16, 10, 320), nt2 = 320;
 #undef GSPX_CL
-    if (k2) kern = k2, threads = nt2;
+    if (k2) kern = k2, threads = nt2, family = 0;
   }
   size_t lds = g->gt_lds;
   if (lg < 8)
@@ -459,6 +495,7 @@
   nwg = std::min(nwg, 8u * (unsigned)std::max(t.per_xcd, 1));
   t.nt = opt.tile_nt >= 0 ? (int)opt.tile_nt : ((size_t)g->N * ld * sizeof(T) >= ((size_t)192 << 20) ? 5 : 0);
   ++g->ctx->step_kinds[0];
+  ++g->ctx->tile_builds[family];
   hipLaunchKernelGGL(kern, dim3(nwg), dim3(threads), lds, st, t);
   return GSPX_OK;
 }
@@ -584,17 +621,19 @@
   else
     make_plan_fused(nf, M, cp, acc_existing, final_to_y, plan);
 
+  const bool tile_ok = tile_direct || padded;
+  const bool need_w = deferred || !tile_ok;
   std::vector<T> hw;
-  if (deferred) {
+  if (need_w && deferred) {
     hw.resize((size_t)nf * M);
     for (size_t i = 0; i < hw.size(); ++i) hw[i] = (T)cp[i];
-  } else {
+  } else if (need_w) {
     hw.resize((size_t)K * nf * 3);
     for (int k = 0; k < K; ++k)
       for (int j = 0; j < nf * 3; ++j) hw[(size_t)k * nf * 3 + j] = (T)plan[(size_t)k].w[(size_t)j];
   }
   const bool cap = ctx->capturing;
-  if (!cap) {
+  if (!cap && need_w) {
     CHK(ctx->ws_w.ensure(hw.size() * sizeof(T) + 64));
     HIPCHK(hipMemcpyAsync(ctx->ws_w.p, hw.data(), hw.size() * sizeof(T), hipMemcpyHostToDevice, st));
     HIPCHK(hipStreamSynchronize(st));
@@ -609,7 +648,6 @@
 
   hipEvent_t ev[4] = {};
   if (!cap) CHK(batch_events(ctx, ev_idx, ev));
-  const bool tile_ok = tile_direct || padded;
   const unsigned char* xb = (const unsigned char*)x;
   const unsigned char* yb = (const unsigned char*)y;
   const size_t xbytes = (size_t)N * ldx * sizeof(T), ybytes = (size_t)nf * N * ldy * sizeof(T);
@@ -666,7 +704,7 @@
         t.wc = (T)ps.w[1];
         t.wo = (T)ps.w[2];
       }
-      CHK(launch_step_tile<T>(g, opt, t, ldw, st));
+      CHK(launch_step_tile<T>(g, opt, t, ldw, st, nullptr, !deferred && k == K));
       continue;
     }
     if (deferred) {
@@ -883,7 +921,7 @@
   const Options& opt = ctx->opt;
   const int64_t N = g->N;
   for (int i = 0; i < 5; ++i) ctx->timing[i] = 0;
-  ctx->step_kinds[0] = ctx->step_kinds[1] = 0;
+  reset_step_counts(ctx);
   if (N == 0 || Nsig == 0) return GSPX_OK;
   CHK(ensure_factor<T>(g, lmax));
   std::vector<double> cp;
@@ -931,6 +969,7 @@
       ctx->timing[2] = (double)K;
       ctx->step_kinds[0] = ctx->graph_kinds[0];
       ctx->step_kinds[1] = ctx->graph_kinds[1];
+      for (int i = 0; i < 5; ++i) ctx->tile_builds[i] = ctx->graph_builds[i];
       return GSPX_OK;
     }
     if (!key.empty() && ctx->seen_key == key) {
@@ -957,6 +996,7 @@
           ctx->graph_key = key;
           ctx->graph_kinds[0] = ctx->step_kinds[0];
           ctx->graph_kinds[1] = ctx->step_kinds[1];
+          for (int i = 0; i < 5; ++i) ctx->graph_builds[i] = ctx->tile_builds[i];
           return filter_dev_t<T>(g, lmax, Nf, M, coeffs, Nsig, x, y, mode);
         }
         ctx->graph_exec = nullptr;
@@ -989,7 +1029,7 @@
   gspx_ctx* ctx = g->ctx;
   replay_reset(ctx);
   for (int i = 0; i < 5; ++i) ctx->timing[i] = 0;
-  ctx->step_kinds[0] = ctx->step_kinds[1] = 0;
+  reset_step_counts(ctx);
   if (g->N == 0 || Nsig == 0) return GSPX_OK;
   CHK(ensure_factor<T>(g, lmax));
   int64_t max_ld = 0;
@@ -1185,7 +1225,7 @@
   gspx_ctx* ctx = g->ctx;
   const int64_t N = g->N;
   for (int i = 0; i < 5; ++i) ctx->timing[i] = 0;
-  ctx->step_kinds[0] = ctx->step_kinds[1] = 0;
+  reset_step_counts(ctx);
   if (Nsig == 0) return GSPX_OK;
   if (N == 0) {
     std::fill(out, out + (size_t)Nf * Nsig, 0.0);
@@ -1236,7 +1276,7 @@
   gspx_ctx* ctx = g->ctx;
   const int64_t N = g->N;
   for (int i = 0; i < 5; ++i) ctx->timing[i] = 0;
-  ctx->step_kinds[0] = ctx->step_kinds[1] = 0;
+  reset_step_counts(ctx);
   if (Nsig == 0) return GSPX_OK;
   if (N == 0) {
     std::fill(out, out + (size_t)M * Nsig, 0.0);
diff --git a/pygsp_amd/csrc/gspx_tile_kernels.hip.h b/pygsp_amd/csrc/gspx_tile_kernels.hip.h
--- a/pygsp_amd/csrc/gspx_tile_kernels.hip.h
+++ b/pygsp_amd/csrc/gspx_tile_kernels.hip.h
@@ -37,6 +37,7 @@
 
 constexpr int GSPX_TILE_BR = 64;
 constexpr int GSPX_TILE_MAXN1 = 160;
+constexpr int TILE_KIND_LAST = 1, TILE_KIND_FIRST = 2, TILE_KIND_GAMMA0 = 3;
 
 template <typename T, int NCOL, int LG, bool OLDNAT, bool ACC = true> struct TileSchedule {
   static constexpr bool PF = !OLDNAT;
@@ -47,7 +48,7 @@
 };
 
 template <typename T, int NCOL, int LG = 16, bool OLDNAT = false, bool INS = false, int NT = 512, int CL = LG,
-          int MIX = 0, bool ACC = true>
+          int MIX = 0, bool ACC = true, int KIND = 0>
 __global__ __launch_bounds__(NT, 4) void k_step_tile(const TileArgs<T> a) {
   static_assert(NT == 512 || (NT == 64 * LG && NCOL == 1) || (CL < LG && NCOL == 1 && NT % 64 == 0 && NT % CL == 0),
                 "narrow builds: one row per group, one chunk per row");
@@ -59,8 +60,11 @@
   constexpr bool META_AFTER = Sched::META_AFTER;
   constexpr bool TILE_LAST = Sched::TILE_LAST;
   constexpr bool PF_ENTRIES = Sched::PF_ENTRIES;
-  constexpr bool EARLY_OLD = Sched::EARLY_OLD;
+  constexpr bool LASTK = KIND == TILE_KIND_LAST, FIRSTF = KIND == TILE_KIND_FIRST, GAMMA0 = KIND == TILE_KIND_GAMMA0;
+  constexpr bool EARLY_OLD = Sched::EARLY_OLD && !GAMMA0;
   static_assert(ACC || (!OLDNAT && !INS && CL == LG), "flush-free builds: the plain flavour only");
+  static_assert(KIND == 0 || (LG == 16 && CL == LG && NT == 512 && !INS && MIX == 0), "kind builds: wide, no synthesis");
+  static_assert((!LASTK || (ACC && !OLDNAT)) && (!FIRSTF || ACC) && (!GAMMA0 || (!ACC && !OLDNAT)), "kind builds");
   constexpr int VEC = 16 / (int)sizeof(T);
   typedef typename VT<T, VEC>::t V;
   typedef __attribute__((address_space(3))) void* lds_ptr;
@@ -93,7 +97,7 @@
   const rsrc_t ri = __builtin_amdgcn_make_buffer_rsrc((void*)a.lidx, 0, a.lidx_bytes, 0x00020000);
   const u32 ldb = a.ld * (u32)sizeof(T);
 
-  struct Meta { int rows[ST]; int rp[RPG + 1]; int orow[OLDNAT ? RPG : 1]; };
+  struct Meta { int rows[ST]; int rp[RPG + 1]; int orow[(OLDNAT || LASTK) ? RPG : 1]; };
   const int xflip = xlo + k1 - 1;
   const bool rev = a.reverse != 0;
   auto phys = [&](int p) { return rev ? xflip - p : p; };
@@ -119,6 +123,11 @@
 #pragma unroll
       for (int t = 0; t < RPG; ++t) m.orow[t] = a.old_rows[(r + t) < a.N ? (r + t) : a.N - 1];
     }
+    if constexpr (LASTK) {
+      const int* const rows_of_y = a.perm ? a.perm : a.rowptr;
+#pragma unroll
+      for (int t = 0; t < RPG; ++t) m.orow[t] = rows_of_y[(r + t) < a.N ? (r + t) : a.N - 1];
+    }
     return m;
   };
   V* const tile = (V*)gspx_smem;
@@ -150,11 +159,13 @@
 #pragma unroll
     for (int t = 0; t < RPG; ++t) {
       const u32 off = (r0 + t < a.N && cb != POISON) ? (u32)(r0 + t) * ldb + cb : POISON;
+      if constexpr (!GAMMA0) {
       u32 oo = a.gamma != T(0) ? off : POISON;
       if constexpr (OLDNAT) oo = (off != POISON && a.gamma != T(0)) ? (u32)m.orow[t] * ldb + cb : POISON;
       if (a.nt & 4) dst[t] = __builtin_bit_cast(V, __builtin_amdgcn_raw_buffer_load_b128(rold, oo, 0, 2));
       else dst[t] = VT<T, VEC>::bload(rold, oo);
-      if constexpr (ACC) {
+      }
+      if constexpr (ACC && !FIRSTF) {
         const u32 ro = a.flush == 2 ? off : POISON;
         if (a.nt & 2) ra[t] = __builtin_bit_cast(V, __builtin_amdgcn_raw_buffer_load_b128(rra, ro, 0, 2));
         else ra[t] = VT<T, VEC>::bload(rra, ro);
@@ -212,6 +223,11 @@
     const bool on = col0 < a.ld;
     const u32 cb = on ? col0 * (u32)sizeof(T) : POISON;
     if constexpr (!PF) prefetch_rows(M, k, c, ovc);
+    int yrow[LASTK ? RPG : 1];
+    if constexpr (LASTK) {
+#pragma unroll
+      for (int t = 0; t < RPG; ++t) yrow[t] = M.orow[t];
+    }
     V ins[INS ? RPG : 1];
 #pragma unroll
     for (int t = 0; t < (INS ? RPG : 1); ++t) ins[t] = 0;
@@ -251,7 +267,7 @@
             __builtin_amdgcn_raw_buffer_load_b128(ri, (u32)rp0 + i * 16u, 0, 0);
     }
     if constexpr (TILE_LAST && !META_AFTER) {
-      constexpr int NMETA = ST + RPG + 1 + 1;
+      constexpr int NMETA = ST + RPG + 1 + 1 + (LASTK ? RPG : 0);
       static_assert(NMETA < 16, "vmcnt immediate");
       if (last && !INS) __builtin_amdgcn_s_waitcnt(0x0070 | NMETA);
       else __builtin_amdgcn_s_waitcnt(0x0070);
@@ -288,13 +304,22 @@
           acc += a.val[j] * xv;
         }
       }
-      if constexpr (ACC) {
+      if constexpr (GAMMA0) {
+        nv[t] = __builtin_elementwise_fma((V)a.beta, self, __builtin_elementwise_fma((V)a.gamma, (V)0, a.scale * acc));
+      } else if constexpr (KIND != 0) {
+        nv[t] = __builtin_elementwise_fma((V)a.beta, self, __builtin_elementwise_fma((V)a.gamma, ovc[t], a.scale * acc));
+      } else if constexpr (ACC) {
         nv[t] = a.scale * acc + a.gamma * ovc[t] + a.beta * self;
       } else {
         nv[t] = __builtin_elementwise_fma((V)a.beta, self, __builtin_elementwise_fma((V)a.gamma, ovc[t], a.scale * acc));
       }
       if constexpr (INS) nv[t] += ins[t];
-      if constexpr (ACC) {
+      if constexpr (ACC && KIND != 0) {
+        res[t] = __builtin_elementwise_fma((V)a.wo, ovc[t], __builtin_elementwise_fma((V)a.wc, self, a.wn * nv[t]));
+        if constexpr (!FIRSTF) {
+          if (a.flush == 2) res[t] += ra[t];
+        }
+      } else if constexpr (ACC) {
         res[t] = a.wn * nv[t] + a.wc * self + a.wo * ovc[t];
         if (a.flush == 2) res[t] += ra[t];
       }
@@ -315,6 +340,18 @@
 #pragma unroll
     for (int t = 0; t < RPG; ++t) {
       const int row = row0 + t;
+      if constexpr (LASTK) {
+        if (row < a.N && on) {
+          if (a.final) {
+            const size_t orow = a.perm ? (size_t)yrow[t] : (size_t)row;
+            *(V*)(a.y + orow * a.ldy + col0) = res[t];
+          } else {
+            if (a.nt & 2) __builtin_nontemporal_store(res[t], (V*)(a.racc + (size_t)row * a.ld + col0));
+            else *(V*)(a.racc + (size_t)row * a.ld + col0) = res[t];
+          }
+        }
+        continue;
+      }
       if (row < a.N && on) {
         if (a.final && (!ACC || !a.flush)) {
           const size_t orow = a.perm ? (size_t)a.perm[row] : (size_t)row;
diff --git a/pygsp_amd/engine.py b/pygsp_amd/engine.py
--- a/pygsp_amd/engine.py
+++ b/pygsp_amd/engine.py
@@ -6,6 +6,14 @@
 from scipy import sparse
 
 from . import _capi
+
+TILE_BUILDS = ("general", "flush_free", "gamma0", "first_flush", "last_step")
+
+
+def tile_build_family(flush, gamma_zero, last_step, flavour=0, chunks=1, acc_builds=True, kind_builds=True):
+    f = _capi.load().gspx_tile_build_family(int(bool(acc_builds)), int(bool(kind_builds)), int(chunks),
+                                            int(flavour), int(flush), int(bool(gamma_zero)), int(bool(last_step)))
+    return TILE_BUILDS[f]
 
 
 class Context:
@@ -48,6 +56,11 @@
         out = (ctypes.c_int64 * 2)()
         _capi.check(_capi.load().gspx_last_step_kinds(self._h, out))
         return {"tile": int(out[0]), "plain": int(out[1])}
+
+    def last_tile_builds(self):
+        out = (ctypes.c_int64 * 5)()
+        _capi.check(_capi.load().gspx_last_tile_builds(self._h, out))
+        return dict(zip(TILE_BUILDS, (int(v) for v in out)))
 
     def last_host_timing(self):
         out = (ctypes.c_double * 9)()
```

Result: no change. 194.7 billion, median of 6 (+0.5%).
